# ilur98/DLMC-QUANT

Hardware: AMD Instinct MI355X
Metric: ResNet-50 W8A8 fake-quant fwd images/sec (higher is better)
Workload: dtype i8; 1 GPU; resnet50 W8A8 per-channel fake-quant forward (FSPTQ forms: W minmax_channel s8, A minmax_tensor u8), BN folded first as in FSPTQuant.py:67, fused int8 MFMA conv/linear, frozen execution plan (epilogue-fused ReLU / shortcut / next-layer codes; block end + next 1x1 as one launch; weight codes quantised once at plan build), 2 HIP streams per GPU, 224x224 relu(N(0,1)) pixels, batch 512 per GPU, scales; global_batch=512, parallelism=dp1 (batch-sharded replicas)

## Files before the change

dlmc-quant_amd/csrc/conv_chain_i8.hip:

```cpp
#include "conv_i8_common.h"

namespace dlmcq {

struct ChainArgs {
  const int8_t* x;
  const int8_t* w1;
  const float* s_w1;
  const int32_t* wsum1;
  const float* bias1;
  const float* s_in1;
  const float* zp_in1;
  int shift1;
  const float* residual;
  const int8_t* x2;
  const int8_t* w2;
  const float* s_w2;
  const int32_t* wsum2;
  const float* bias2;
  const float* s_in2;
  const float* zp_in2;
  int shift2, P, Q, H2, W2, stride2;
  FastDiv qdiv, pdiv;
  float* out;
  uint8_t* codes;
  const int8_t* w3;
  const float* s_w3;
  const int32_t* wsum3;
  const float* bias3;
  uint8_t* codes2;
  int w3_row, w3_chunk;
  int M, KD, rows_per_tile;
  int f_rowq, f_cstep, o_rowq, o_cstep;
  int lab;
  unsigned long long* trace;
};

template <int CTRL>
__device__ __forceinline__ float quad_dpp(float v) {
  return __builtin_bit_cast(float, __builtin_amdgcn_mov_dpp(__builtin_bit_cast(int, v), CTRL, 0xf, 0xf, true));
}
__device__ __forceinline__ void quad_transpose(float& x0, float& x1, float& x2, float& x3, bool b0, bool b1) {
  const float x0s = quad_dpp<0xB1>(x0), x1s = quad_dpp<0xB1>(x1), x2s = quad_dpp<0xB1>(x2), x3s = quad_dpp<0xB1>(x3);
  const float n0 = b0 ? x1s : x0, n1 = b0 ? x1 : x0s, n2 = b0 ? x3s : x2, n3 = b0 ? x3 : x2s;
  const float n0s = quad_dpp<0x4E>(n0), n1s = quad_dpp<0x4E>(n1), n2s = quad_dpp<0x4E>(n2), n3s = quad_dpp<0x4E>(n3);
  x0 = b1 ? n2s : n0;
  x2 = b1 ? n2 : n0s;
  x1 = b1 ? n3s : n1;
  x3 = b1 ? n3 : n1s;
}

constexpr int CHAIN_WGS(int c1, int kb) { return c1 + kb <= 256 ? 3 : 2; }
constexpr int CH_BIG = 0x7fff0000;

template <int C1, int KB, int C2 = 0, int FL = -1>
__global__ __launch_bounds__(256, CHAIN_WGS(C1 + C2, KB)) void conv_chain_i8_kernel(ChainArgs a, ConvEpi ep1, ConvEpi ep2) {
  constexpr bool DUALH = C2 > 0;
  const bool relu1 = FL < 0 ? ep1.relu != 0 : (FL & 1) != 0;
  const bool out1 = FL < 0 ? a.out != nullptr : (FL & 2) != 0;
  constexpr int S1 = C1 / 64;
  constexpr int S2 = C2 / 64;
  constexpr int U3 = KB / 64;
  constexpr int WCH = (S1 + S2 + U3) * 4096;
  constexpr int NPD = DUALH ? 2 : 1;
  constexpr int PAR = NPD * 4 * 256;
#ifndef DLMCQ_CHAIN_LDS_T
#define DLMCQ_CHAIN_LDS_T ((C1 == 128 && C2 == 256) ? 0 : 2)
#endif
  constexpr int TF = DLMCQ_CHAIN_LDS_T;
  constexpr bool LDST = TF != 0;
#ifdef DLMCQ_LAB
  constexpr int LABDMA = (C2 == 0 && C1 == 64) ? 16384 : 0;
#else
  constexpr int LABDMA = 0;
#endif
  __shared__ __attribute__((aligned(1024))) int8_t lds[2 * WCH + 2 * PAR + 4096 + 3 * KB * 4 + (LDST ? 4096 : 0) + LABDMA];
  int8_t* const par0 = lds + 2 * WCH;
  int8_t* const ctile = lds + 2 * WCH + 2 * PAR;
  int8_t* const par3 = ctile + 4096;
  float* const tstage = reinterpret_cast<float*>(par3 + 3 * KB * 4) + (threadIdx.x >> 6) * 256;

  const int tid = threadIdx.x, wave = tid >> 6, lane = tid & 63, l31 = lane & 31, hsel = lane >> 5;
  const int wr = wave >> 1, wc = wave & 1;
  constexpr bool LDST2 = TF == 2;
  const int q4 = LDST2 ? (lane & 7) : (l31 >> 2), b4 = l31 & 3;
  const int rsel = LDST2 ? (lane >> 3) : (4 * hsel + b4);
  const bool b0 = (lane & 1) != 0, b1 = (lane & 2) != 0;
  const int64_t row0 = (int64_t)blockIdx.x * a.rows_per_tile;
  const int rows_here = (int)((a.M - row0) < a.rows_per_tile ? (a.M - row0) : a.rows_per_tile);
  const int NC = a.KD >> 6;
#ifndef DLMCQ_CHAIN_ROT
#define DLMCQ_CHAIN_ROT 0
#endif
  const int rot = DLMCQ_CHAIN_ROT ? (int)(blockIdx.x % (unsigned)NC) : 0;
  auto cn = [&](int n) { const int m = n + rot; return m >= NC ? m - NC : m; };
#ifdef DLMCQ_LAB
  unsigned long long* const tr = (a.trace && tid == 0) ? a.trace + 64 * (size_t)blockIdx.x : nullptr;
  int trn = 0;
#define CHAIN_STAMP() do { if (tr && trn < 56) tr[trn++] = __builtin_readcyclecounter(); } while (0)
#define CHAIN_FINE(k) do { if (tr && nseq == 1) tr[56 + (k)] = __builtin_readcyclecounter(); } while (0)
#else
#define CHAIN_STAMP() do { } while (0)
#define CHAIN_FINE(k) do { } while (0)
#endif
  CHAIN_STAMP();
#ifdef DLMCQ_LAB
  if ((a.lab & 0x600) && blockIdx.x < 512) {
    const int unit = a.lab >> 16;
    const int d = (a.lab & 0x200) ? ((blockIdx.x >> 8) & 1) * unit : (int)(((blockIdx.x * 2654435761u) >> 28) * (uint32_t)unit) >> 4;
    for (int i = 0; i < d; ++i) __builtin_amdgcn_s_sleep(1);
  }
#endif

  {
    const int lrw = tid >> 2;
    const int sgw = ((tid & 3) ^ ((lrw >> 2) & 3)) * 16;
    const int8_t* xp = a.x + (row0 + (lrw < rows_here ? lrw : rows_here - 1)) * C1 + sgw;
#pragma unroll
    for (int s = 0; s < S1; ++s)
      __builtin_amdgcn_global_load_lds((gptr_t)(xp + s * 64), (lptr_t)(lds + WCH + s * 4096 + (tid >> 6) * 1024), 16, 0, 0);
    if constexpr (DUALH) {
      const uint32_t m = (uint32_t)(row0 + (lrw < rows_here ? lrw : rows_here - 1));
      const uint32_t t = fdiv(m, a.qdiv), nn = fdiv(t, a.pdiv);
      const int q = (int)(m - t * (uint32_t)a.Q), pp = (int)(t - nn * (uint32_t)a.P);
      const int8_t* xp2 = a.x2 + (((int64_t)nn * a.H2 + pp * a.stride2) * a.W2 + q * a.stride2) * C2 + sgw;
#pragma unroll
      for (int s = 0; s < S2; ++s)
        __builtin_amdgcn_global_load_lds((gptr_t)(xp2 + s * 64), (lptr_t)(lds + WCH + (S1 + s) * 4096 + (tid >> 6) * 1024), 16, 0, 0);
    }
  }
  const float sin2 = ep1.q_scale[0];
  const float zpf2 = ep1.q_zp ? ep1.q_zp[0] : 0.0f;
  const int dz2 = 128 - (int)__builtin_rintf(zpf2);
  if (tid < KB) {
    reinterpret_cast<float*>(par3)[tid] = sin2 * a.s_w3[tid];
    reinterpret_cast<int*>(par3)[KB + tid] = dz2 * a.wsum3[tid];
    reinterpret_cast<float*>(par3)[2 * KB + tid] = a.bias3 ? a.bias3[tid] : 0.0f;
  }
  asm volatile("s_waitcnt vmcnt(0) lgkmcnt(0)\n\ts_barrier" ::: "memory");
  i32x4 af[S1][2];
  i32x4 af2[DUALH ? S2 : 1][2];
  {
    const int r = wr * 32 + l31;
    const int8_t* ab = lds + WCH + r * 64;
    const uint32_t xw = a.shift1 ? 0x80808080u : 0u;
#pragma unroll
    for (int s = 0; s < S1; ++s)
#pragma unroll
      for (int ks = 0; ks < 2; ++ks) {
        const i32x4 t = *reinterpret_cast<const i32x4*>(ab + s * 4096 + (((ks * 2 + hsel) ^ ((r >> 2) & 3)) << 4));
        af[s][ks] = i32x4{(int)(t.x ^ xw), (int)(t.y ^ xw), (int)(t.z ^ xw), (int)(t.w ^ xw)};
      }
    if constexpr (DUALH) {
      const uint32_t xw2 = a.shift2 ? 0x80808080u : 0u;
#pragma unroll
      for (int s = 0; s < S2; ++s)
#pragma unroll
        for (int ks = 0; ks < 2; ++ks) {
          const i32x4 t = *reinterpret_cast<const i32x4*>(ab + (S1 + s) * 4096 + (((ks * 2 + hsel) ^ ((r >> 2) & 3)) << 4));
          af2[s][ks] = i32x4{(int)(t.x ^ xw2), (int)(t.y ^ xw2), (int)(t.z ^ xw2), (int)(t.w ^ xw2)};
        }
    }
  }
  asm volatile("s_waitcnt lgkmcnt(0)" ::: "memory");
  CHAIN_STAMP();

  const uint32_t fbytes = (uint32_t)((int64_t)a.M * a.KD * 4);
  const v4i r_res = make_rsrc(a.residual, fbytes);
  const v4i r_out = make_rsrc(a.out ? (const void*)a.out : (const void*)a.residual, a.out ? fbytes : 0u);
  const v4i r_cod = make_rsrc(a.codes ? (const void*)a.codes : (const void*)a.residual, a.codes ? fbytes / 4 : 0u);
  int fo[4];
#pragma unroll
  for (int g = 0; g < 4; ++g) {
    const int lr = wr * 32 + 8 * g + rsel;
    fo[g] = lr < rows_here ? (int)(((row0 + lr) * a.f_rowq + wc * 32 + q4 * 4) * 4) : CH_BIG;
#ifdef DLMCQ_LAB
    if (a.lab & 4) {
      const int lr2 = wr * 32 + 16 * (g >> 1) + 2 * (4 * hsel + b4) + (q4 >> 2);
      fo[g] = lr2 < rows_here ? (int)(((row0 + lr2) * a.KD + wc * 32 + 16 * (g & 1) + (q4 & 3) * 4) * 4) : CH_BIG;
    }
    if (a.lab & 8) {
      const int lr3 = wr * 32 + wc * 16 + 4 * g + (lane >> 4);
      fo[g] = lr3 < rows_here ? (int)(((row0 + lr3) * a.KD + (lane & 15) * 4) * 4) : CH_BIG;
    }
#endif
  }
  int cstep = a.f_cstep;
#ifdef DLMCQ_LAB
  if (a.lab & 64) {
    cstep = 64 * 256;
#pragma unroll
    for (int g = 0; g < 4; ++g) {
      const int lr = wr * 32 + 8 * g + rsel;
      fo[g] = lr < rows_here ? (int)(row0 * a.KD * 4 + lr * 256 + (wc * 32 + q4 * 4) * 4) : CH_BIG;
    }
  }
#endif
  constexpr bool MIXED_OK = !DUALH && !(C1 == 128 && KB == 128);
  int fo2[MIXED_OK ? 4 : 1];
  const int cstep2 = a.o_cstep;
  if constexpr (MIXED_OK) {
    const bool same = a.o_rowq == a.f_rowq;
#pragma unroll
    for (int g = 0; g < 4; ++g) {
      const int lr = wr * 32 + 8 * g + rsel;
      fo2[g] = same ? fo[g] : (lr < rows_here ? (int)(((row0 + lr) * a.o_rowq + wc * 32 + q4 * 4) * 4) : CH_BIG);
    }
  }
  auto out_off = [&](int g, int n) {
    if constexpr (MIXED_OK) return fo2[g] + n * cstep2;
    else return fo[g] + n * cstep;
  };
  int tw[4];
#pragma unroll
  for (int j = 0; j < 4; ++j) tw[j] = (4 * hsel + j) * 32 + (LDST2 ? l31 : ((l31 & 3) | ((l31 & ~3) ^ ((4 * hsel + j) * 4))));
  const int trd = LDST2 ? rsel * 32 + 4 * q4 : (4 * hsel + b4) * 32 + ((4 * q4) ^ ((4 * hsel + b4) * 4));
  const int nst = (out1 ? 4 : 0) + (a.codes ? 1 : 0);

  const int lrow = lane >> 2, pslot = lane & 3;
  const int drow = wave * 16 + lrow;
  const int dseg = (pslot ^ ((drow >> 2) & 3)) * 16;
  const int8_t* w1p = a.w1 + (int64_t)drow * C1 + dseg;
  const int d3 = drow & 31;
  const int prow3 = (drow & 32) + 16 * ((d3 >> 2) & 1) + 4 * (d3 >> 3) + (d3 & 3);
  const int8_t* w3p = a.w3 + (int64_t)prow3 * a.w3_row + dseg;
  const int cvo = drow < rows_here ? (int)((row0 + drow) * a.KD + dseg) : CH_BIG;
  const void* const pars[4] = {a.s_w1, a.wsum1, a.bias1 ? (const void*)a.bias1 : (const void*)a.s_w1, a.s_w1};
  const int32_t* parp = static_cast<const int32_t*>(wave == 0 ? pars[0] : wave == 1 ? pars[1] : wave == 2 ? pars[2] : pars[3]) + lane;
  const int8_t* w2p = DUALH ? a.w2 + (int64_t)drow * C2 + dseg : nullptr;
  const void* const pars2[4] = {a.s_w2, a.wsum2, a.bias2 ? (const void*)a.bias2 : (const void*)a.s_w2, a.s_w2};
  const int32_t* parp2 = static_cast<const int32_t*>(wave == 0 ? pars2[0] : wave == 1 ? pars2[1] : wave == 2 ? pars2[2] : pars2[3]) + lane;

  f32x4 res[2][4];
#ifdef DLMCQ_LAB
  if (a.lab & 0x801)
    for (auto& r2 : res)
      for (auto& r : r2) r = f32x4{1.0f, 2.0f, 3.0f, 4.0f};
#endif
  auto request = [&](int nseq, auto par_c) {
    constexpr int P = decltype(par_c)::value;
    const int n = cn(nseq);
    int8_t* wb = lds + P * WCH;
    bool wdma = true;
#ifdef DLMCQ_LAB
    wdma = !(((a.lab & 16) && (n & 1)) || (a.lab & 32));
#endif
#pragma unroll
    for (int s = 0; s < S1; ++s)
      if (wdma) __builtin_amdgcn_global_load_lds((gptr_t)(w1p + (int64_t)n * 64 * C1 + s * 64), (lptr_t)(wb + s * 4096 + wave * 1024), 16, 0, 0);
#pragma unroll
    for (int u = 0; u < U3; ++u)
      if (wdma) {
        const int8_t* src = w3p + (int64_t)u * 64 * a.w3_row + (int64_t)n * a.w3_chunk;
        __builtin_amdgcn_global_load_lds((gptr_t)src, (lptr_t)(wb + (S1 + S2 + u) * 4096 + wave * 1024), 16, 0, 0);
      }
    __builtin_amdgcn_global_load_lds((gptr_t)(parp + n * 64), (lptr_t)(par0 + P * PAR + wave * 256), 4, 0, 0);
    if constexpr (DUALH) {
#pragma unroll
      for (int s = 0; s < S2; ++s)
        if (wdma) __builtin_amdgcn_global_load_lds((gptr_t)(w2p + (int64_t)n * 64 * C2 + s * 64), (lptr_t)(wb + (S1 + s) * 4096 + wave * 1024), 16, 0, 0);
      __builtin_amdgcn_global_load_lds((gptr_t)(parp2 + n * 64), (lptr_t)(par0 + P * PAR + 1024 + wave * 256), 4, 0, 0);
      return;
    }
#pragma unroll
    for (int g = 0; g < 4; ++g) {
#ifdef DLMCQ_LAB
      if (a.lab & 1) continue;
      if constexpr (LABDMA > 0) {
        if (a.lab & 0x800) {
          const int lr = wr * 32 + 8 * g + rsel;
          const float* src = a.residual + (row0 + (lr < rows_here ? lr : rows_here - 1)) * a.KD + n * 64 + wc * 32 + q4 * 4;
          __builtin_amdgcn_global_load_lds((gptr_t)src, (lptr_t)(lds + sizeof(lds) - LABDMA + wave * 4096 + g * 1024), 16, 0, 2);
          continue;
        }
      }
#endif
      int lo = fo[g] + n * cstep;
#ifdef DLMCQ_LAB
      if (a.lab & 0x2000) lo &= 0xffff;
#endif
      bload16(res[P][g], lo, r_res);
    }
  };

  const float sin1 = a.s_in1[0];
  const float zpf1 = a.zp_in1 ? a.zp_in1[0] : 0.0f;
  const int dz1 = a.shift1 - (int)__builtin_rintf(zpf1);
  const float sin1b = DUALH ? a.s_in2[0] : 0.0f;
  const int dz1b = DUALH ? a.shift2 - (int)__builtin_rintf(a.zp_in2 ? a.zp_in2[0] : 0.0f) : 0;
  ConvEpi e1 = ep1;
  e1.codes = reinterpret_cast<uint8_t*>(uintptr_t(1));
  const EpiQuant eq1(e1, FL >= 0);
  __builtin_assume(!eq1.sgn);

  i32x16 acc2[U3];
#pragma unroll
  for (int j = 0; j < U3; ++j)
#pragma unroll
    for (int i = 0; i < 16; ++i) acc2[j][i] = 0;

  request(0, std::integral_constant<int, 0>{});

  auto chunk = [&](int nseq, auto par_c) {
    constexpr int P = decltype(par_c)::value;
    const int n = cn(nseq);
    if (nseq == 0 || nst == 0) asm volatile("s_waitcnt vmcnt(0)\n\ts_barrier" ::: "memory");
    else if (nst == 4) asm volatile("s_waitcnt vmcnt(4)\n\ts_barrier" ::: "memory");
    else if (nst == 5) asm volatile("s_waitcnt vmcnt(5)\n\ts_barrier" ::: "memory");
    else asm volatile("s_waitcnt vmcnt(1)\n\ts_barrier" ::: "memory");
    CHAIN_STAMP();
    if constexpr (!DUALH) asm volatile("" : "+v"(res[P][0]), "+v"(res[P][1]), "+v"(res[P][2]), "+v"(res[P][3]));
    if (nseq + 1 < NC) request(nseq + 1, std::integral_constant<int, 1 - P>{});

    const int8_t* wb = lds + P * WCH;
    const int8_t* pp = par0 + P * PAR + (wc * 32 + l31) * 4;
    i32x16 acc;
    f32x2 extra2[DUALH ? 8 : 1];
    if constexpr (DUALH) {
      const float corr2f = (float)(dz1b * *reinterpret_cast<const int*>(pp + 1024 + 256));
#pragma unroll
      for (int i = 0; i < 16; ++i) acc[i] = 0;
      const int r = wc * 32 + l31;
#pragma unroll
      for (int s = 0; s < S2; ++s)
#pragma unroll
        for (int ks = 0; ks < 2; ++ks) {
          const i32x4 bf = *reinterpret_cast<const i32x4*>(wb + (S1 + s) * 4096 + r * 64 + (((ks * 2 + hsel) ^ ((r >> 2) & 3)) << 4));
          acc = __builtin_amdgcn_mfma_i32_32x32x32_i8(af2[s][ks], bf, acc, 0, 0, 0);
        }
      const float mult2 = sin1b * *reinterpret_cast<const float*>(pp + 1024);
      const float bv2 = a.bias2 ? *reinterpret_cast<const float*>(pp + 1024 + 512) : 0.0f;
      const f32x2 c2{corr2f, corr2f}, m2{mult2, mult2}, b2{bv2, bv2};
#pragma unroll
      for (int i = 0; i < 8; ++i) extra2[i] = pk_fma(f32x2{(float)acc[2 * i], (float)acc[2 * i + 1]} + c2, m2, b2);
    }
    const float corrf = (float)(dz1 * *reinterpret_cast<const int*>(pp + 256));
#pragma unroll
    for (int i = 0; i < 16; ++i) acc[i] = 0;
    {
      const int r = wc * 32 + l31;
#pragma unroll
      for (int s = 0; s < S1; ++s)
#pragma unroll
        for (int ks = 0; ks < 2; ++ks) {
          const i32x4 bf = *reinterpret_cast<const i32x4*>(wb + s * 4096 + r * 64 + (((ks * 2 + hsel) ^ ((r >> 2) & 3)) << 4));
          acc = __builtin_amdgcn_mfma_i32_32x32x32_i8(af[s][ks], bf, acc, 0, 0, 0);
        }
    }
#ifdef DLMCQ_LAB
    if (tr && nseq == 1) asm volatile("s_nop 0" ::"v"(acc[0]), "v"(acc[15]));
#endif
    CHAIN_FINE(0);
    const float mult = sin1 * *reinterpret_cast<const float*>(pp);
    const float bv = a.bias1 ? *reinterpret_cast<const float*>(pp + 512) : 0.0f;
    float v[16];
    {
      const f32x2 c2{corrf, corrf}, m2{mult, mult}, b2{bv, bv};
#pragma unroll
      for (int i = 0; i < 8; ++i) {
        f32x2 f = pk_fma(f32x2{(float)acc[2 * i], (float)acc[2 * i + 1]} + c2, m2, b2);
        if constexpr (DUALH) f = f + extra2[DUALH ? i : 0];
        v[2 * i] = f.x;
        v[2 * i + 1] = f.y;
      }
    }
#ifndef DLMCQ_CHAIN_GP
#define DLMCQ_CHAIN_GP 4
#endif
    constexpr bool TIGHT = C2 == 0 && ((C1 == 64 && KB == 128) || (C1 == 128 && KB == 128));
    constexpr int GP = (FL < 0 || TIGHT) ? 1 : DLMCQ_CHAIN_GP;
#pragma unroll
    for (int g0 = 0; g0 < 4; g0 += GP) {
      f32x4 y[GP];
#pragma unroll
      for (int k = 0; k < GP; ++k) {
        const int g = g0 + k;
        if constexpr (LDST) {
#pragma unroll
          for (int j = 0; j < 4; ++j) tstage[tw[j]] = v[4 * g + j];
          asm volatile("" ::: "memory");
          y[k] = *reinterpret_cast<const f32x4*>(tstage + trd);
          asm volatile("" ::: "memory");
        } else {
          quad_transpose(v[4 * g], v[4 * g + 1], v[4 * g + 2], v[4 * g + 3], b0, b1);
          y[k] = f32x4{v[4 * g], v[4 * g + 1], v[4 * g + 2], v[4 * g + 3]};
        }
        if constexpr (!DUALH) y[k] = y[k] + res[P][g];
        if (relu1 && (FL < 0 || out1)) y[k] = relu4_nan(y[k]);
#ifdef DLMCQ_LAB
        if (out1) bstore16(y[k], (a.lab & 0x1000) ? (out_off(g, n) & 0xffff) : out_off(g, n), r_out);
#else
        if (out1) bstore16(y[k], out_off(g, n), r_out);
#endif
      }
      uint32_t c[GP];
      if constexpr (FL >= 0) {
        eq1.code4n_plain(y, c);
      } else if constexpr (GP == 1) {
        c[0] = eq1.code4(y[0]);
      } else {
        bool un[GP];
        eq1.code4n(y, c, un);
      }
#pragma unroll
      for (int k = 0; k < GP; ++k) {
        const int R = wr * 32 + 8 * (g0 + k) + rsel;
        *reinterpret_cast<uint32_t*>(ctile + R * 64 + (((wc * 2 + (q4 >> 2)) ^ ((R >> 2) & 3)) << 4) + (q4 & 3) * 4) = c[k];
        CHAIN_FINE(1 + g0 + k);
      }
    }
    CHAIN_STAMP();
    asm volatile("s_waitcnt lgkmcnt(0)\n\ts_barrier" ::: "memory");
    CHAIN_STAMP();
    if (a.codes)
      bstore16i(*reinterpret_cast<const i32x4*>(ctile + drow * 64 + pslot * 16), cvo == CH_BIG ? CH_BIG : cvo + n * 64, r_cod);
    {
      const int R = wr * 32 + l31;
#pragma unroll
      for (int ks = 0; ks < 2; ++ks) {
        const i32x4 t = *reinterpret_cast<const i32x4*>(ctile + R * 64 + (((ks * 2 + hsel) ^ ((R >> 2) & 3)) << 4));
        const i32x4 a2 = i32x4{(int)(t.x ^ 0x80808080u), (int)(t.y ^ 0x80808080u), (int)(t.z ^ 0x80808080u), (int)(t.w ^ 0x80808080u)};
#pragma unroll
        for (int j = 0; j < U3; ++j) {
          const int kb = wc * (KB / 2) + j * 32 + l31;
          const i32x4 bf = *reinterpret_cast<const i32x4*>(wb + (S1 + S2) * 4096 + kb * 64 + (((ks * 2 + hsel) ^ ((kb >> 2) & 3)) << 4));
          acc2[j] = __builtin_amdgcn_mfma_i32_32x32x32_i8(bf, a2, acc2[j], 0, 0, 0);
        }
      }
    }
  };
  for (int n = 0; n < NC; n += 2) {
    chunk(n, std::integral_constant<int, 0>{});
    if (n + 1 < NC) chunk(n + 1, std::integral_constant<int, 1>{});
  }

  CHAIN_STAMP();
  const EpiQuant eq2(ep2, ep2.relu != 0);
  const int lr2 = wr * 32 + l31;
#pragma unroll
  for (int j = 0; j < U3; ++j) {
    const int cb = wc * (KB / 2) + j * 32 + hsel * 16;
    f32x4 y[4];
#pragma unroll
    for (int q = 0; q < 4; ++q) {
      const f32x4 mu = *reinterpret_cast<const f32x4*>(par3 + (cb + 4 * q) * 4);
      const i32x4 co = *reinterpret_cast<const i32x4*>(par3 + (KB + cb + 4 * q) * 4);
      const f32x4 bs = *reinterpret_cast<const f32x4*>(par3 + (2 * KB + cb + 4 * q) * 4);
      y[q] = f32x4{dequant1(acc2[j][4 * q] + co.x, mu.x, bs.x), dequant1(acc2[j][4 * q + 1] + co.y, mu.y, bs.y),
                   dequant1(acc2[j][4 * q + 2] + co.z, mu.z, bs.z), dequant1(acc2[j][4 * q + 3] + co.w, mu.w, bs.w)};
    }
    uint32_t wq[4];
    if constexpr (FL >= 0) {
      eq2.code4n_plain(y, wq);
    } else {
      bool uq[4];
      eq2.code4n(y, wq, uq);
    }
    if (lr2 < rows_here)
      *reinterpret_cast<i32x4*>(ep2.codes + (row0 + lr2) * KB + cb) = i32x4{(int)wq[0], (int)wq[1], (int)wq[2], (int)wq[3]};
  }
#ifdef DLMCQ_LAB
  if (tr) {
    asm volatile("s_waitcnt vmcnt(0)" ::: "memory");
    CHAIN_STAMP();
    tr[63] = __builtin_amdgcn_s_getreg(4 | (31 << 11));
  }
#endif
}

}

using namespace dlmcq;

#ifdef DLMCQ_LAB
static unsigned long long* g_chain_trace = nullptr;
extern "C" void dlmcq_x_chain_trace(void* buf) { g_chain_trace = static_cast<unsigned long long*>(buf); }
static int g_chain_lab = 0;
extern "C" void dlmcq_x_chain_lab(int flags) { g_chain_lab = flags; }
#endif

static int chain_launch(ChainArgs& a, int64_t M, int64_t C, int64_t K, int64_t C2, int64_t K2, int32_t relu, void* codes,
                        const float* q_scale, const float* q_zero_point, int32_t q_lo, int32_t q_hi, int32_t q_form, float q_ste_g,
                        int32_t relu2, void* codes2, const float* q2_scale, const float* q2_zero_point, int32_t q2_lo, int32_t q2_hi,
                        int32_t q2_form, float q2_ste_g, int32_t rows_per_tile, dlmcq_stream_t stream) {
  if (relu == DLMCQ_ACT_RELU6 || relu2 == DLMCQ_ACT_RELU6) return DLMCQ_EINVAL;
  if (q_lo != 0 || q_hi != 255) return DLMCQ_EINVAL;
  if (q2_form & (DLMCQ_FORCE_TILED | DLMCQ_ROUTE_ONLY | DLMCQ_PIPELINED)) return DLMCQ_EINVAL;
  const bool w3cm = (q2_form & DLMCQ_W2_CHUNK_MAJOR) != 0, ocm = (q2_form & DLMCQ_FP32_OUT_CHUNK_MAJOR) != 0;
  const bool icm = (C2 == 0 && a.residual) ? (q2_form & DLMCQ_FP32_IN_CHUNK_MAJOR) != 0 : ocm;
  const bool ocm2 = a.out ? ocm : icm;
  q2_form &= ~(DLMCQ_W2_CHUNK_MAJOR | DLMCQ_FP32_IN_CHUNK_MAJOR | DLMCQ_FP32_OUT_CHUNK_MAJOR);
  if (icm != ocm2 && C2 == 0 && C == 128 && K2 == 128) return DLMCQ_EINVAL;
  a.w3_row = w3cm ? 64 : (int)K;
  a.w3_chunk = w3cm ? (int)K2 * 64 : 64;
  ConvEpi ep1{}, ep2{};
  if (q2_lo > q2_hi || q2_lo < -128 || q2_hi > 255 || q2_hi - q2_lo > 255 || q_form < DLMCQ_FORM_EMULATE ||
      q_form > DLMCQ_FORM_SYMMETRIC || !epi_set_form(ep2, q2_form, q2_lo, q2_hi))
    return DLMCQ_EINVAL;
  if (M * K * 4 > (int64_t)CH_BIG) return DLMCQ_ERANGE;
  a.M = (int)M; a.KD = (int)K;
  a.f_rowq = icm ? 64 : (int)K;
  a.f_cstep = icm ? (int)M * 256 : 256;
  a.o_rowq = ocm2 ? 64 : (int)K;
  a.o_cstep = ocm2 ? (int)M * 256 : 256;
#ifdef DLMCQ_LAB
  a.trace = g_chain_trace;
  a.lab = g_chain_lab;
#endif
  if (rows_per_tile <= 0) {
    const int64_t t64 = (M + 63) / 64, slots = 256 * CHAIN_WGS((int)(C + C2), (int)K2);
    const int64_t full = t64 / slots, left = t64 % slots;
    rows_per_tile = (full >= 2 && full <= 4 && left > 0 && left * 8 < slots) ? 56 : 64;
  }
  a.rows_per_tile = rows_per_tile;
  if (a.rows_per_tile > 64) return DLMCQ_EINVAL;
  ep1.relu = relu != 0; ep1.q_scale = q_scale; ep1.q_zp = q_zero_point; ep1.q_lo = (float)q_lo; ep1.q_hi = (float)q_hi;
  ep1.q_g = q_ste_g; ep1.q_form = q_form; ep1.codes = static_cast<uint8_t*>(codes);
  ep2.relu = relu2 != 0; ep2.q_scale = q2_scale; ep2.q_zp = q2_zero_point; ep2.q_lo = (float)q2_lo; ep2.q_hi = (float)q2_hi;
  ep2.q_g = q2_ste_g; ep2.codes = static_cast<uint8_t*>(codes2);
  const int64_t tiles = (M + a.rows_per_tile - 1) / a.rows_per_tile;
  if (tiles >= (1ll << 31)) return DLMCQ_ERANGE;
  hipStream_t st = reinterpret_cast<hipStream_t>(stream);
  const dim3 grid((uint32_t)tiles), block(256);
  size_t dyn = 0;
#ifdef DLMCQ_LAB
  dyn = (g_chain_lab & 128 ? 40960 : 0) + (g_chain_lab & 256 ? 81920 : 0);
#endif
  const int fl = (relu && epi_plain_q(ep1) && epi_plain_q(ep2)) ? (a.out ? 3 : 1) : -1;
#define DLMCQ_CHAIN_GO(...)                                                                                          \
  do {                                                                                                               \
    if (fl == 3) hipLaunchKernelGGL((conv_chain_i8_kernel<__VA_ARGS__, 3>), grid, block, dyn, st, a, ep1, ep2);       \
    else if (fl == 1) hipLaunchKernelGGL((conv_chain_i8_kernel<__VA_ARGS__, 1>), grid, block, dyn, st, a, ep1, ep2);  \
    else hipLaunchKernelGGL((conv_chain_i8_kernel<__VA_ARGS__, -1>), grid, block, dyn, st, a, ep1, ep2);              \
  } while (0)
  if (C2 == 0) {
    if (C == 64 && K2 == 64) DLMCQ_CHAIN_GO(64, 64, 0);
    else if (C == 64 && K2 == 128) DLMCQ_CHAIN_GO(64, 128, 0);
    else if (C == 128 && K2 == 128) DLMCQ_CHAIN_GO(128, 128, 0);
    else if (C == 128 && K2 == 256) DLMCQ_CHAIN_GO(128, 256, 0);
    else if (C == 256 && K2 == 256) DLMCQ_CHAIN_GO(256, 256, 0);
    else return DLMCQ_EINVAL;
  } else {
    if (C == 64 && C2 == 64 && K2 == 64) DLMCQ_CHAIN_GO(64, 64, 64);
    else if (C == 128 && C2 == 256 && K2 == 128) DLMCQ_CHAIN_GO(128, 128, 256);
    else return DLMCQ_EINVAL;
  }
#undef DLMCQ_CHAIN_GO
  return launch_status();
}

extern "C" int dlmcq_conv2d_i8_nhwc_chain(const void* x, const int8_t* w, float* out, const float* bias, const int32_t* wsum,
                                          const float* in_scale, const float* in_zero_point, const float* w_scale, int64_t M,
                                          int64_t C, int64_t K, int32_t x_is_unsigned, const float* residual, int32_t relu,
                                          void* codes, const float* q_scale, const float* q_zero_point, int32_t q_lo,
                                          int32_t q_hi, int32_t q_form, float q_ste_g, const int8_t* w2, const float* bias2,
                                          const int32_t* wsum2, const float* w_scale2, int64_t K2, int32_t relu2, void* codes2,
                                          const float* q2_scale, const float* q2_zero_point, int32_t q2_lo, int32_t q2_hi,
                                          int32_t q2_form, float q2_ste_g, int32_t rows_per_tile, dlmcq_stream_t stream) {
  if (M < 0 || C < 1 || K < 1 || K2 < 1 || K % 64 != 0) return DLMCQ_EINVAL;
  if (M == 0) return DLMCQ_OK;
  if (!x || !w || !wsum || !in_scale || !w_scale || !residual || !w2 || !wsum2 || !w_scale2 || !codes2 || !q_scale || !q2_scale)
    return DLMCQ_EINVAL;
  if (!aligned16(x) || !aligned16(w) || !aligned16(w2) || !aligned16(residual) || (out && !aligned16(out)) ||
      (codes && !aligned16(codes)) || !aligned16(codes2))
    return DLMCQ_EALIGN;
  ChainArgs a{};
  a.x = static_cast<const int8_t*>(x); a.w1 = w; a.s_w1 = w_scale; a.wsum1 = wsum; a.bias1 = bias;
  a.s_in1 = in_scale; a.zp_in1 = in_zero_point; a.shift1 = x_is_unsigned ? 128 : 0;
  a.residual = residual; a.out = out; a.codes = static_cast<uint8_t*>(codes);
  a.w3 = w2; a.s_w3 = w_scale2; a.wsum3 = wsum2; a.bias3 = bias2; a.codes2 = static_cast<uint8_t*>(codes2);
  return chain_launch(a, M, C, K, 0, K2, relu, codes, q_scale, q_zero_point, q_lo, q_hi, q_form, q_ste_g, relu2, codes2, q2_scale,
                      q2_zero_point, q2_lo, q2_hi, q2_form, q2_ste_g, rows_per_tile, stream);
}

extern "C" int dlmcq_conv2d_i8_nhwc_dual_chain(const void* x, const int8_t* w, float* out, const float* bias, const int32_t* wsum,
                                               const float* in_scale, const float* in_zero_point, const float* w_scale, int64_t N,
                                               int64_t H, int64_t W, int64_t C, int64_t K, int32_t x_is_unsigned, const void* x2,
                                               const int8_t* w2, const float* bias2, const int32_t* wsum2, const float* in_scale2,
                                               const float* in_zero_point2, const float* w_scale2, int64_t H2, int64_t W2,
                                               int64_t C2, int32_t stride2, int32_t x2_is_unsigned, int32_t relu, void* codes,
                                               const float* q_scale, const float* q_zero_point, int32_t q_lo, int32_t q_hi,
                                               int32_t q_form, float q_ste_g, const int8_t* w3, const float* bias3,
                                               const int32_t* wsum3, const float* w_scale3, int64_t K3, int32_t relu3, void* codes3,
                                               const float* q3_scale, const float* q3_zero_point, int32_t q3_lo, int32_t q3_hi,
                                               int32_t q3_form, float q3_ste_g, int32_t rows_per_tile, dlmcq_stream_t stream) {
  if (N < 0 || H < 1 || W < 1 || C < 1 || K < 1 || K3 < 1 || K % 64 != 0 || H2 < 1 || W2 < 1 || C2 < 1 || stride2 < 1)
    return DLMCQ_EINVAL;
  if ((H2 - 1) / stride2 + 1 != H || (W2 - 1) / stride2 + 1 != W) return DLMCQ_EINVAL;
  const int64_t M = N * H * W;
  if (M == 0) return DLMCQ_OK;
  if (!x || !w || !wsum || !in_scale || !w_scale || !x2 || !w2 || !wsum2 || !in_scale2 || !w_scale2 || !w3 || !wsum3 || !w_scale3 ||
      !codes3 || !q_scale || !q3_scale)
    return DLMCQ_EINVAL;
  if (!aligned16(x) || !aligned16(w) || !aligned16(x2) || !aligned16(w2) || !aligned16(w3) || (out && !aligned16(out)) ||
      (codes && !aligned16(codes)) || !aligned16(codes3))
    return DLMCQ_EALIGN;
  if (M >= (1ll << 31) || N * H2 * W2 * C2 >= (1ll << 40)) return DLMCQ_ERANGE;
  ChainArgs a{};
  a.x = static_cast<const int8_t*>(x); a.w1 = w; a.s_w1 = w_scale; a.wsum1 = wsum; a.bias1 = bias;
  a.s_in1 = in_scale; a.zp_in1 = in_zero_point; a.shift1 = x_is_unsigned ? 128 : 0;
  a.x2 = static_cast<const int8_t*>(x2); a.w2 = w2; a.s_w2 = w_scale2; a.wsum2 = wsum2; a.bias2 = bias2;
  a.s_in2 = in_scale2; a.zp_in2 = in_zero_point2; a.shift2 = x2_is_unsigned ? 128 : 0;
  a.P = (int)H; a.Q = (int)W; a.H2 = (int)H2; a.W2 = (int)W2; a.stride2 = stride2;
  a.qdiv = make_fastdiv((uint32_t)W);
  a.pdiv = make_fastdiv((uint32_t)H);
  a.residual = nullptr; a.out = out; a.codes = static_cast<uint8_t*>(codes);
  a.w3 = w3; a.s_w3 = w_scale3; a.wsum3 = wsum3; a.bias3 = bias3; a.codes2 = static_cast<uint8_t*>(codes3);
  return chain_launch(a, M, C, K, C2, K3, relu, codes, q_scale, q_zero_point, q_lo, q_hi, q_form, q_ste_g, relu3, codes3, q3_scale,
                      q3_zero_point, q3_lo, q3_hi, q3_form, q3_ste_g, rows_per_tile, stream);
}
```

dlmc-quant_amd/dlmc/_native.py:

```python
import ctypes
import os

import torch

_HERE = os.path.dirname(os.path.abspath(__file__))
import sys

_PRODUCT = os.path.join(os.path.dirname(_HERE), "libdlmcq.so")
_OVERRIDE = os.environ.get("DLMCQ_LIBRARY")
LAB_OVERRIDE = bool(_OVERRIDE) and os.environ.get("DLMCQ_LAB_TOOLS") == "1"
if _OVERRIDE and not LAB_OVERRIDE:
    print(f"[dlmc] DLMCQ_LIBRARY={_OVERRIDE} ignored (set DLMCQ_LAB_TOOLS=1 to load a lab / A-B build); loading {_PRODUCT}", file=sys.stderr)
LIB_PATH = _OVERRIDE if LAB_OVERRIDE else _PRODUCT
if LAB_OVERRIDE:
    print(f"[dlmc] lab override: loading {LIB_PATH} instead of the product library", file=sys.stderr)

FORM_EMULATE, FORM_QBASE, FORM_ZEROPOINT, FORM_SYMMETRIC, FORM_ROOTQ_ACT = range(5)
EMIT_SHIFT128 = 0x100
W2_CHUNK_MAJOR = 0x200
FORCE_TILED = 0x400
ROUTE_ONLY = 0x800
FP32_IN_CHUNK_MAJOR = 0x2000
FP32_OUT_CHUNK_MAJOR = 0x4000
PAD_CODE0 = 0x8000
PIPELINED = 0x1000
ROUTE_TILED, ROUTE_HALO3X3, ROUTE_PW, ROUTE_PWR, ROUTE_DW, ROUTE_DWM, ROUTE_HALO3X3_PIPE, ROUTE_GAP = 1, 2, 3, 4, 5, 6, 7, 8
ROUTE_TAG = {ROUTE_TILED: "conv_i8", ROUTE_HALO3X3: "conv3x3_halo", ROUTE_PW: "conv_pw", ROUTE_PWR: "conv_pwr", ROUTE_DW: "conv_dw",
             ROUTE_DWM: "conv_dwm", ROUTE_HALO3X3_PIPE: "conv3x3_pipe", ROUTE_GAP: "conv_gap"}
ACT_NONE, ACT_RELU, ACT_RELU6 = 0, 1, 2
Y_DEQUANT, Y_CODES = 0, 1
CODES_NONE, CODES_I8, CODES_P4 = 0, 1, 2
MINMAX_ABSMAX, MINMAX_MINMAX, MINMAX_NEGMIN = 0, 1, 2

_p, _i64, _i32, _f32, _sz = ctypes.c_void_p, ctypes.c_int64, ctypes.c_int32, ctypes.c_float, ctypes.c_size_t

SIGNATURES = {
    "dlmcq_version": (ctypes.c_int, []),
    "dlmcq_strerror": (ctypes.c_char_p, [ctypes.c_int]),
    "dlmcq_fake_quant_f32": (ctypes.c_int, [_p, _p, _p, _p, _p, _i64, _i64, _i64, _i32, _i32, _i32, _i32, _i32, _f32, _p]),
    "dlmcq_dequant_codes_f32": (ctypes.c_int, [_p, _p, _p, _p, _i64, _i64, _i64, _i32, _i32, _i32, _f32, _p]),
    "dlmcq_dequant_f32": (ctypes.c_int, [_p, _p, _p, _p, _i64, _i64, _i64, _p]),
    "dlmcq_minmax_scratch_bytes": (_sz, [_i64, _i64, _i64]),
    "dlmcq_minmax_f32": (ctypes.c_int, [_p, _p, _p, _i64, _i64, _i64, _i32, _p, _sz, _p]),
    "dlmcq_minmax_finalize_f32": (ctypes.c_int, [_p, _i64, _i64, _p, _p, _i32, _p]),
    "dlmcq_conv2d_i8_observed_partials": (_sz, [_i64, _i64]),
    "dlmcq_conv2d_i8_nhwc_fused_observed": (ctypes.c_int, [_p, _p, _p, _p, _p, _p, _p, _p, _i64, _i64, _i64, _i64, _i64, _i64, _i64, _i32, _i32,
                                                            _i32, _i32, _p, _i32, _p, _p, _p, _i32, _i32, _i32, _f32, _p, _i64, _p, _p]),
    "dlmcq_qparams_from_minmax": (ctypes.c_int, [_p, _p, _p, _p, _i64, _i32, _i32, _i32, _i32, _f32, _p]),
    "dlmcq_span_scale_f32": (ctypes.c_int, [_p, _p, _p, _i64, _f32, _i32, _p]),
    "dlmcq_lsq_init_scratch_bytes": (_sz, [_i64]),
    "dlmcq_lsq_init_f32": (ctypes.c_int, [_p, _p, _i64, _f32, _p, _sz, _p]),
    "dlmcq_observe_qparams_f32": (ctypes.c_int, [_p, _p, _p, _i64, _i64, _i64, _i32, _i32, _i32, _f32, _p, _sz, _p]),
    "dlmcq_pack_int4": (ctypes.c_int, [_p, _p, _i64, _p]),
    "dlmcq_unpack_int4": (ctypes.c_int, [_p, _p, _i64, _i32, _p]),
    "dlmcq_fq_bwd_scratch_bytes": (_sz, [_i64, _i64, _i64]),
    "dlmcq_fake_quant_bwd_f32": (ctypes.c_int, [_p, _p, _p, _p, _p, _p, _i64, _i64, _i64, _i32, _i32, _f32, _p, _sz, _p]),
    "dlmcq_rootq_bwd_scratch_bytes": (ctypes.c_size_t, [_i64]),
    "dlmcq_rootq_weight_bwd_f32": (ctypes.c_int, [_p, _p, _p, _p, _p, _p, _i64, _i32, _i32, _p, _sz, _p]),
    "dlmcq_fake_quant_bwd_form_f32": (ctypes.c_int, [_p, _p, _p, _p, _p, _p, _i64, _i64, _i64, _i32, _i32, _i32, _f32, _p, _sz, _p]),
    "dlmcq_fq_segment_bytes": (_sz, []),
    "dlmcq_fq_multi_prepare": (ctypes.c_int, [_p, _i64, _p, _p, _p, _p]),
    "dlmcq_fake_quant_multi_f32": (ctypes.c_int, [_p, _i64, _i64, _p]),
    "dlmcq_fake_quant_multi_bwd_f32": (ctypes.c_int, [_p, _i64, _i64, _i64, _p, _sz, _p]),
    "dlmcq_rootq_weight_f32": (ctypes.c_int, [_p, _p, _p, _i64, _i32, _i32, _p]),
    "dlmcq_l2norm_scratch_bytes": (_sz, [_i64, _i64, _i64]),
    "dlmcq_l2norm_step_f32": (ctypes.c_int, [_p, _p, _p, _p, _i64, _i64, _i64, _i32, _i32, _p, _sz, _p]),
    "dlmcq_l2norm_iterate_f32": (ctypes.c_int, [_p, _p, _p, _p, _i64, _i64, _i64, _i32, _i32, _i32, _f32, _p, _sz, _p]),
    "dlmcq_l2out_scratch_bytes": (_sz, [_i64, _i64, _i64]),
    "dlmcq_l2out_update_f32": (ctypes.c_int, [_p, _p, _p, _p, _p, _i64, _i64, _i64, _i32, _f32, _f32, _p, _sz, _p]),
    "dlmcq_l2loss_scratch_bytes": (_sz, [_i64]),
    "dlmcq_l2loss_tensor_f32": (ctypes.c_int, [_p, _p, _p, _p, _p, _i64, _i32, _f32, _p, _sz, _p]),
    "dlmcq_l2loss_rows_f32": (ctypes.c_int, [_p, _p, _p, _i64, _i64, _i32, _p]),
    "dlmcq_adaround_weight_f32": (ctypes.c_int, [_p, _p, _p, _p, _i64, _i64, _i32, _i32, _i32, _p]),
    "dlmcq_adaround_weight_bwd_f32": (ctypes.c_int, [_p, _p, _p, _p, _p, _p, _i64, _i64, _i32, _i32, _p]),
    "dlmcq_quantize_weight_krsc_i8": (ctypes.c_int, [_p, _p, _p, _p, _i64, _i64, _i64, _i64, _i32, _i32, _p]),
    "dlmcq_conv2d_i8_nhwc_f32": (ctypes.c_int, [_p, _p, _p, _p, _p, _p, _p, _p, _i64, _i64, _i64, _i64, _i64, _i64, _i64,
                                               _i32, _i32, _i32, _i32, _p]),
    "dlmcq_conv2d_i8_nhwc_fused": (ctypes.c_int, [_p, _p, _p, _p, _p, _p, _p, _p, _i64, _i64, _i64, _i64, _i64, _i64, _i64,
                                                 _i32, _i32, _i32, _i32, _p, _i32, _p, _p, _p, _i32, _i32, _i32, _f32, _p]),
    "dlmcq_conv2d_i8_nhwc_asym": (ctypes.c_int, [_p, _p, _p, _p, _p, _p, _p, _p, _p, _i64, _i64, _i64, _i64, _i64, _i64, _i64,
                                                _i32, _i32, _i32, _i32, _p, _i32, _p, _p, _p, _i32, _i32, _i32, _f32, _p]),
    "dlmcq_conv2d_i8_nhwc_narrow": (ctypes.c_int, [_p, _p, _p, _p, _p, _p, _p, _p, _p, _i64, _i64, _i64, _i64, _i64, _i64, _i64,
                                                  _i32, _i32, _i32, _i32, _p, _i32, _p, _p, _p, _i32, _i32, _i32, _f32, _i64, _p]),
    "dlmcq_conv2d_i8_nhwc_padres": (ctypes.c_int, [_p, _p, _p, _p, _p, _p, _p, _p, _p, _i64, _i64, _i64, _i64, _i64, _i64, _i64,
                                                  _i32, _i32, _i32, _i32, _p, _i64, _i64, _i64, _i32, _i64, _i32, _p, _p, _p, _i32, _i32, _i32,
                                                  _f32, _i64, _p]),
    "dlmcq_conv2d_dw_i8_nhwc": (ctypes.c_int, [_p, _p, _p, _p, _p, _p, _p, _p, _i64, _i64, _i64, _i64, _i64, _i64, _i32, _i32, _i32,
                                              _i32, _p, _p, _p, _i32, _i32, _i32, _f32, _p]),
    "dlmcq_conv2d_i8_nhwc_xoff": (ctypes.c_int, [_p, _p, _p, _p, _p, _p, _p, _p, _p, _i64, _i64, _i64, _i64, _i64, _i64, _i64,
                                                _i32, _i32, _i32, _i32, _p, _i32, _p, _p, _p, _i32, _i32, _i32, _f32, _p, _p, _p]),
    "dlmcq_conv2d_dw_i8_nhwc_xoff": (ctypes.c_int, [_p, _p, _p, _p, _p, _p, _p, _p, _i64, _i64, _i64, _i64, _i64, _i64, _i32, _i32, _i32,
                                                   _i32, _p, _p, _p, _i32, _i32, _i32, _f32, _p, _p, _p]),
    "dlmcq_conv2d_i8_stem_xoff": (ctypes.c_int, [_p, _p, _p, _p, _p, _p, _p, _p, _p, _i64, _i64, _i64, _i64, _i64, _i64, _i64, _i32, _i32,
                                                _i32, _i32, _p, _p, _p, _i32, _i32, _i32, _f32, _p, _p, _p]),
    "dlmcq_dwpw_pack_table": (ctypes.c_int, [_p, _p, _p, _p, _p, _p, _i64, _i32, _p, _p]),
    "dlmcq_conv2d_dwpw_i8_nhwc": (ctypes.c_int, [_p, _p, _i32, _i32, _i32, _p, _i64, _i64, _i64, _i64, _i32, _p, _p, _i32, _i32, _i32, _f32,
                                                _p, _p, _p, _p, _p, _p, _i64, _i32, _p, _p, _p, _i32, _i32, _i32, _f32, _p]),
    "dlmcq_conv2d_i8_nhwc_dual": (ctypes.c_int, [_p, _p, _p, _p, _p, _p, _p, _p, _i64, _i64, _i64, _i64, _i64, _i64, _i64,
                                                _i32, _i32, _i32, _i32,
                                                _p, _p, _p, _p, _p, _p, _p, _i64, _i64, _i64, _i64, _i64, _i32, _i32, _i32, _i32,
                                                _i32, _p, _p, _p, _i32, _i32, _i32, _f32, _p]),
    "dlmcq_conv2d_i8_nhwc_chain": (ctypes.c_int, [_p, _p, _p, _p, _p, _p, _p, _p, _i64, _i64, _i64, _i32, _p, _i32, _p, _p, _p, _i32,
                                                 _i32, _i32, _f32, _p, _p, _p, _p, _i64, _i32, _p, _p, _p, _i32, _i32, _i32, _f32,
                                                 _i32, _p]),
    "dlmcq_conv2d_i8_nhwc_dual_chain": (ctypes.c_int, [_p, _p, _p, _p, _p, _p, _p, _p, _i64, _i64, _i64, _i64, _i64, _i32,
                                                      _p, _p, _p, _p, _p, _p, _p, _i64, _i64, _i64, _i32, _i32,
                                                      _i32, _p, _p, _p, _i32, _i32, _i32, _f32,
                                                      _p, _p, _p, _p, _i64, _i32, _p, _p, _p, _i32, _i32, _i32, _f32, _i32, _p]),
    "dlmcq_quantize_pad_nhwc4": (ctypes.c_int, [_p, _p, _p, _p, _i64, _i64, _i64, _i64, _i64, _i64, _i64, _i64, _i32, _i32, _i32,
                                               _i32, _f32, _p]),
    "dlmcq_quantize_weight_stem_i8": (ctypes.c_int, [_p, _p, _p, _p, _i64, _i64, _i64, _i64, _i32, _i32, _p]),
    "dlmcq_conv2d_i8_stem_fused": (ctypes.c_int, [_p, _p, _p, _p, _p, _p, _p, _p, _i64, _i64, _i64, _i64, _i64, _i64, _i32, _i32,
                                                 _i32, _p, _p, _p, _i32, _i32, _i32, _f32, _p]),
    "dlmcq_conv2d_i8_stem_asym": (ctypes.c_int, [_p, _p, _p, _p, _p, _p, _p, _p, _p, _i64, _i64, _i64, _i64, _i64, _i64, _i64, _i32, _i32,
                                                _i32, _p, _p, _p, _i32, _i32, _i32, _f32, _p]),
    "dlmcq_conv2d_i8_stem_pool_fused": (ctypes.c_int, [_p, _p, _p, _p, _p, _p, _p, _p, _i64, _i64, _i64, _i64, _i64, _i64, _i32, _i32,
                                                      _i32, _p, _p, _p, _i32, _i32, _i32, _f32, _p]),
    "dlmcq_maxpool_codes_nhwc": (ctypes.c_int, [_p, _p, _i64, _i64, _i64, _i64, _i32, _i32, _i32, _i32, _p]),
    "dlmcq_gap_nhwc_f32": (ctypes.c_int, [_p, _p, _p, _i64, _i64, _i64, _p, _p, _i32, _i32, _i32, _f32, _p]),
    "dlmcq_avgpool_nhwc_f32": (ctypes.c_int, [_p, _p, _p, _i64, _i64, _i64, _i64, _i64, _i64, _i64, _i32, _p, _p, _i32, _i32, _i32, _f32, _p]),
    "dlmcq_conv2d_i8_nhwc_gap": (ctypes.c_int, [_p, _p, _p, _p, _p, _p, _p, _p, _i64, _i64, _i64, _i64, _i64, _i32, _p, _i32, _p, _p, _p,
                                               _i32, _i32, _i32, _f32, _p]),
    "dlmcq_fold_bn_f32": (ctypes.c_int, [_p, _p, _p, _p, _p, _p, _i64, _i64, _f32, _p]),
    "dlmcq_repvgg_fuse_f32": (ctypes.c_int, [_p, _p, _p, _p, _p, _p, _p, _f32, _f32, _f32, _i64, _i64, _p]),
}


class FqSegment(ctypes.Structure):
    _fields_ = [("x", _p), ("y", _p), ("gy", _p), ("gx", _p), ("scale", _p), ("offset", _p), ("gscale", _p),
                ("n", _i64), ("channels", _i64), ("inner", _i64), ("lo", _i64), ("hi", _i64), ("ste_g", ctypes.c_double),
                ("form", _i64), ("fwd_chunk0", _i64), ("bwd_wg0", _i64), ("part0", _i64)]


FQ_MULTI_MAX_ELEMENTS = 8192 * 1024


def _load():
    if not os.path.exists(LIB_PATH):
        raise ImportError(
            f"{LIB_PATH} not found: build it with `make -C dlmc-quant_amd/csrc` (or "
            "`python -c 'import __graft_entry__ as g; g.build()'`).  There is no CPU fallback.")
    tlib = os.path.join(os.path.dirname(torch.__file__), "lib", "libamdhip64.so")
    if os.path.exists(tlib):
        ctypes.CDLL(tlib, mode=ctypes.RTLD_GLOBAL)
    lib = ctypes.CDLL(LIB_PATH)
    for name, (res, args) in SIGNATURES.items():
        try:
            fn = getattr(lib, name)
        except AttributeError:
            if LAB_OVERRIDE:
                continue
            raise
        fn.restype, fn.argtypes = res, args
    if hasattr(lib, "dlmcq_fq_segment_bytes") and lib.dlmcq_fq_segment_bytes() != ctypes.sizeof(FqSegment):
        raise ImportError(f"{LIB_PATH}: dlmcq_fq_segment is {lib.dlmcq_fq_segment_bytes()} bytes, the ctypes mirror {ctypes.sizeof(FqSegment)}")
    return lib


lib = _load()


def experimental(name, argtypes):
    fn = getattr(lib, name)
    fn.restype, fn.argtypes = ctypes.c_int, argtypes
    return fn


class DlmcqError(RuntimeError):
    pass


def check(rc):
    if rc != 0:
        raise DlmcqError(f"{lib.dlmcq_strerror(rc).decode()} (code {rc})")


def route(rc):
    if rc <= 0:
        raise DlmcqError(f"{lib.dlmcq_strerror(rc).decode()} (code {rc})" if rc < 0 else "route query returned DLMCQ_OK (an empty problem)")
    return rc


def stream_ptr():
    return ctypes.c_void_p(torch.cuda.current_stream().cuda_stream)


def ptr(t):
    return None if t is None else ctypes.c_void_p(t.data_ptr())


def require_gpu(*tensors):
    for t in tensors:
        if t is not None and not t.is_cuda:
            raise DlmcqError(
                "dlmc (MI355X build) runs on the GPU only: got a tensor on "
                f"'{t.device}'.  There is no CPU fallback in this package.")
```

dlmc-quant_amd/dlmc/quantization/scalar/kernels.py:

```python
import collections
import ctypes
import math

import torch

from ... import _native as N
from ..._native import (CODES_I8, CODES_NONE, CODES_P4, FORM_EMULATE, FORM_QBASE, FORM_ROOTQ_ACT,
                        FORM_SYMMETRIC, FORM_ZEROPOINT, MINMAX_ABSMAX, MINMAX_MINMAX, MINMAX_NEGMIN,
                        Y_CODES, Y_DEQUANT)

__all__ = ["fake_quant", "dequant_codes", "dequant", "minmax", "observe_qparams", "qparams_from_minmax",
           "span_scale", "lsq_init", "l2norm_step", "adaround_weight", "adaround_weight_backward", "quantize_weight_krsc", "conv2d_i8", "global_avgpool", "avgpool_quant", "conv2d_i8_gap", "gap_head_supported", "gap_head_profitable", "pack_int4", "unpack_int4", "fake_quant_backward", "Segment", "FqMultiPlan", "fake_quant_multi", "fake_quant_multi_backward", "rootq_weight", "geometry", "channel_shape",
           "PROFILE"]


class _Profile:

    def __init__(self):
        self.enabled = False
        self.records = []

    def reset(self):
        self.records = []

# ... 543 lines not shown
    if not want_out and emit is None:
        raise ValueError("conv2d_dw_i8: nothing to produce (want_out=False without emit)")

    def alloc(dtype):
        return torch.empty((n, c, P, Q), dtype=dtype, device=codes.device, memory_format=torch.channels_last)
    q = _quantiser(emit, alloc, codes, False, "conv2d_dw_i8")
    out = alloc(torch.float32) if want_out else None
    small = (_bias_c(bias), _flat(in_scale, codes), _flat(in_zp, codes), _flat(w_scale, codes), _flat(w_offset, codes))
    fn, trailer = N.lib.dlmcq_conv2d_dw_i8_nhwc, ()
    if in_offset is not None:
        in_offset, tap_sums = _flat(in_offset, codes), _flat(tap_sums, codes)
        fn, trailer = N.lib.dlmcq_conv2d_dw_i8_nhwc_xoff, (N.ptr(in_offset), N.ptr(tap_sums))
    args = (N.ptr(codes), N.ptr(wq), N.ptr(out), *map(N.ptr, small), n, h, w_, c, R, S, int(stride), int(padding),
            int(codes.dtype == torch.uint8), _act(relu, act))
    flags = N.FORCE_TILED if force_tiled else 0

    def call(extra=0):
        return fn(*args, *_q_args(q, flags | extra), *trailer, N.stream_ptr())
    oe = n * c * P * Q
    tag = N.ROUTE_TAG[N.route(call(N.ROUTE_ONLY))] if PROFILE.enabled else "conv_dw"
    PROFILE.launch(tag, codes.numel() + wq.numel() + oe * (4 * want_out + (emit is not None)), lambda: N.check(call()), 2 * oe * R * S)
    return (out, q[0]) if emit is not None else out


DWPW_WIDTHS = (128, 192, 512)


def dwpw_supported(c, k, h, w, stride, padding, ksize):
    return ksize == 3 and stride == 1 and padding == 1 and c % 64 == 0 and k in DWPW_WIDTHS and w <= 61 and h >= 1


def dwpw_table(wq, bias, in_scale, in_zp, w_scale, w_offset, x_unsigned=True):
    N.require_gpu(wq)
    r, s_, c = wq.shape
    if (r, s_) != (3, 3) or c % 64:
        raise ValueError("dwpw_table: 3 x 3 weights [3, 3, C], C % 64 == 0")
    table = torch.empty((c // 64, 64, 8), dtype=torch.int32, device=wq.device)
    small = (_bias_c(bias), _flat(in_scale, wq), _flat(in_zp, wq), _flat(w_scale, wq), _flat(w_offset, wq))
    N.check(N.lib.dlmcq_dwpw_pack_table(N.ptr(wq), *map(N.ptr, small), c, int(bool(x_unsigned)), N.ptr(table), N.stream_ptr()))
    return table


def conv2d_dwpw_i8(codes, table, dw_asym, dw_bias, dw_relu, in_zp, emit, pw, relu=True, emit2=None):
    N.require_gpu(codes, table, pw["wq"])
    codes = _nhwc(codes)
    n, c, h, w_ = codes.shape
    k = pw["wq"].shape[0]
    if tuple(pw["wq"].shape[1:]) != (1, 1, c) or emit is None or emit2 is None or tuple(table.shape) != (c // 64, 64, 8):
        raise ValueError("conv2d_dwpw_i8: a pointwise layer [K, 1, 1, C] on the depthwise layer's codes, both quantisers given")
    q1 = _quantiser(emit, lambda dtype: None, codes, False, "conv2d_dwpw_i8")
    q2 = _quantiser(emit2, lambda dtype: torch.empty((n, k, h, w_), dtype=dtype, device=codes.device, memory_format=torch.channels_last),
                    codes, False, "conv2d_dwpw_i8")
    zx, b = _flat(in_zp, codes), _bias_c(pw["bias"])
    scales = (_flat(pw["in_scale"], codes), _flat(pw["w_scale"], codes, k), _flat(pw.get("w_offset"), codes, k))
    m = n * h * w_
    nbytes = codes.numel() + table.numel() * 4 + pw["wq"].numel() + m * k
    PROFILE.launch("conv_dwpw", nbytes, lambda: N.check(N.lib.dlmcq_conv2d_dwpw_i8_nhwc(
        N.ptr(codes), N.ptr(table), int(bool(dw_asym)), int(bool(dw_bias)), int(bool(dw_relu)), N.ptr(zx), n, h, w_, c,
        int(codes.dtype == torch.uint8), *_q_args(q1)[1:], N.ptr(pw["wq"]), N.ptr(b), N.ptr(pw["wsum"]), *map(N.ptr, scales), k,
        int(bool(relu)), *_q_args(q2), N.stream_ptr())), 2 * m * c * (9 + k))
    return q2[0]


def conv2d_i8_dual(a, b, relu=False, emit=None, want_out=True, force_tiled=False, out_chunk_major=False):
    for t in (a, b):
        if t["codes"].dim() != 4:
            raise ValueError("conv2d_i8_dual takes 4-D activation codes")
    oa, ob = _operand(a), _operand(b)
    if oa.shape != ob.shape:
        raise ValueError(f"conv2d_i8_dual: the two convolutions give {oa.shape} and {ob.shape}")
    if not want_out and emit is None:
        raise ValueError("conv2d_i8_dual: nothing to produce (want_out=False without emit)")
    shape = oa.shape
    n, K_ = shape[:2]

    def alloc(dtype):
        return torch.empty(shape, dtype=dtype, device=oa.codes.device, memory_format=torch.channels_last)
    out = alloc(torch.float32) if want_out else None
    q = _quantiser(emit, alloc, oa.codes, True, "conv2d_i8_dual")
    h, w_, ch, R, S, st, pd, dl, uns = oa.geom
    _, _, ch2, R2, S2, st2, _, _, _ = ob.geom
    oe = math.prod(shape)
    def touched(c, r, s_, stride):
        return c.numel() // (stride * stride) if r == 1 and s_ == 1 else c.numel()
    nbytes = touched(oa.codes, R, S, st) + touched(ob.codes, R2, S2, st2) + a["wq"].numel() + b["wq"].numel() + oe * (4 * want_out + (emit is not None))
    args = (*_head(oa, out), n, h, w_, ch, K_, R, S, st, pd, dl, uns, *ob.ptrs, *ob.geom, int(bool(relu)))
    flags = N.FORCE_TILED if force_tiled else 0

    def call(extra=0):
        return N.lib.dlmcq_conv2d_i8_nhwc_dual(*args, *_q_args(q, flags | extra), N.stream_ptr())
    ocm = bool(out_chunk_major) and out is not None and N.route(call(N.ROUTE_ONLY)) == N.ROUTE_PWR
    tag = N.ROUTE_TAG[N.route(call(N.ROUTE_ONLY))] if PROFILE.enabled else "conv_i8"
    PROFILE.launch(tag, nbytes, lambda: N.check(call(N.FP32_OUT_CHUNK_MAJOR if ocm else 0)), 2 * oe * (ch * R * S + ch2 * R2 * S2))
    if ocm:
        out = _as_chunk_major(out)
    return (out, q[0]) if emit is not None else out


CHAIN_SHAPES = {(64, 64), (64, 128), (128, 128), (128, 256), (256, 256)}
CHAIN_ONE_LAYOUT = {(128, 128)}


def chain_supported(c, k, k2, m):
    return (c, k2) in CHAIN_SHAPES and k % 64 == 0 and m * k * 4 <= 0x7fff0000


def chunk_major(wq):
    k2, r, s_, k = wq.shape
    if (r, s_) != (1, 1) or k % 64:
        raise ValueError("chunk_major: a 1x1 layer with K % 64 = 0")
    return wq.reshape(k2, k // 64, 64).permute(1, 0, 2).contiguous()


class ChunkMajor:

    def __init__(self, buf, shape):
        self.buf, self.shape = buf, tuple(shape)
        self.dtype, self.device = buf.dtype, buf.device

    @staticmethod
    def empty(n, k, h, w, device):
        if k % 64:
            raise ValueError("ChunkMajor: K % 64 = 0")
        return ChunkMajor(torch.empty((k // 64, n * h * w, 64), dtype=torch.float32, device=device), (n, k, h, w))

    @staticmethod
    def from_nhwc(t):
        n, k, h, w = t.shape
        if k % 64 or t.dtype != torch.float32:
            raise ValueError("ChunkMajor: an fp32 tensor with K % 64 = 0")
        rows = t.permute(0, 2, 3, 1).reshape(n * h * w, k // 64, 64)
        return ChunkMajor(rows.permute(1, 0, 2).contiguous(), (n, k, h, w))

    def to_nhwc(self):
        n, k, h, w = self.shape
        rows = self.buf.permute(1, 0, 2).reshape(n, h, w, k)
        return rows.permute(0, 3, 1, 2).contiguous(memory_format=torch.channels_last)

    def dim(self):
        return 4

    def numel(self):
        return self.buf.numel()

    def window(self, n, p0, p1, q0, q1):
        nn, k, h, w = self.shape
        rows = self.buf.view(k // 64, nn, h, w, 64)[:, n, p0:p1, q0:q1, :]
        return rows.permute(1, 2, 0, 3).reshape(1, p1 - p0, q1 - q0, k).permute(0, 3, 1, 2).contiguous()

    def record_stream(self, s):
        self.buf.record_stream(s)


class PadShortcut:

    def __init__(self, src, stride=1, lo=0):
        if not isinstance(src, torch.Tensor) or src.dim() != 4 or src.dtype != torch.float32:
            raise ValueError("PadShortcut: the source is an fp32 (N, C, H, W) tensor")
        if not src.permute(0, 2, 3, 1).is_contiguous():
            raise ValueError("PadShortcut: the source must be dense in channels_last memory (a slice or a view with gaps is not)")
        self.src, self.stride, self.lo = src, int(stride), int(lo)
        if self.stride < 1 or self.lo < 0 or self.lo % 4 or src.shape[1] % 4 or src.shape[1] < 4:
            raise ValueError("PadShortcut: stride >= 1, lo >= 0, lo % 4 == 0 and source channels % 4 == 0")
        self.dtype, self.device = src.dtype, src.device

    def shape_for(self, k):
        n, c, h, w = self.src.shape
        s = self.stride
        return (n, k, (h + s - 1) // s, (w + s - 1) // s) if self.lo + c <= k else None

    def materialise(self, k):
        sub = self.src[:, :, ::self.stride, ::self.stride]
        return torch.nn.functional.pad(sub, (0, 0, 0, 0, self.lo, k - self.lo - sub.shape[1])).contiguous(memory_format=torch.channels_last)

    def record_stream(self, s):
        self.src.record_stream(s)


def _second_weights(b):
    wc = b.get("wq_chunk")
    if wc is None:
        return b["wq"], 0
    k2, _, _, k = b["wq"].shape
    if tuple(wc.shape) != (k // 64, k2, 64) or wc.dtype != torch.int8 or not wc.is_contiguous():
        raise ValueError("wq_chunk must be chunk_major(wq)")
    return wc, N.W2_CHUNK_MAJOR


def conv2d_i8_chain(a, b, residual, relu=True, emit=None, want_out=True, want_codes=False, relu2=True, emit2=None,
                    rows_per_tile=0, out_chunk_major=False):
    c = a["codes"]
    icm, ocm = isinstance(residual, ChunkMajor), bool(out_chunk_major) and want_out
    if want_out and icm != ocm and (c.shape[1], b["wq"].shape[0]) in CHAIN_ONE_LAYOUT:
        residual = residual.to_nhwc() if icm else ChunkMajor.from_nhwc(residual)
        icm = ocm
    res_cm, residual = (residual, residual.buf) if icm else (None, residual)
    N.require_gpu(b["wq"], residual)
    o = _operand(a)
    c = o.codes
    (n, K_), (h, w_, ch, R, S, _, _, _, uns) = o.shape[:2], o.geom
    K2, R2, S2, C2 = b["wq"].shape
    if (R, S, R2, S2) != (1, 1, 1, 1) or C2 != K_ or emit is None or emit2 is None:
        raise ValueError("conv2d_i8_chain: two 1x1 convolutions, the second reading the first's codes")
    if tuple(res_cm.shape if icm else residual.shape) != (n, K_, h, w_) or residual.dtype != torch.float32:
        raise ValueError("conv2d_i8_chain: residual must be fp32 of the first output's shape")
    if not icm:
        residual = _nhwc(residual)
    m = n * h * w_

    def alloc(k, dtype):
        return torch.empty((n, k, h, w_), dtype=dtype, device=c.device, memory_format=torch.channels_last)
    out = (ChunkMajor.empty(n, K_, h, w_, c.device) if ocm else alloc(K_, torch.float32)) if want_out else None
    q = _quantiser(emit, lambda dtype: alloc(K_, dtype) if want_codes else None, c, False, "conv2d_i8_chain")
    q2 = _quantiser(emit2, lambda dtype: alloc(K2, dtype), c, True, "conv2d_i8_chain")
    b2, ws2 = _bias_c(b["bias"]), _flat(b["w_scale"], c, K2)
    nbytes = c.numel() + a["wq"].numel() + b["wq"].numel() + m * K_ * (4 + 4 * want_out + want_codes) + m * K2
    w2t, w2flag = _second_weights(b)
    flags = w2flag | (N.FP32_IN_CHUNK_MAJOR if icm else 0) | (N.FP32_OUT_CHUNK_MAJOR if ocm else 0)
    PROFILE.launch("conv_chain", nbytes, lambda: N.check(N.lib.dlmcq_conv2d_i8_nhwc_chain(
        *_head(o, out.buf if ocm else out), m, ch, K_, uns, N.ptr(residual), int(bool(relu)), *_q_args(q),
        N.ptr(w2t), N.ptr(b2), N.ptr(b["wsum"]), N.ptr(ws2), K2, int(bool(relu2)), *_q_args(q2, flags), int(rows_per_tile), N.stream_ptr())),
        2 * m * K_ * (ch + K2))
    return out, q[0], q2[0]


DUAL_CHAIN_SHAPES = {(64, 64, 64), (128, 256, 128)}


def dual_chain_supported(c, c2, k, k3, m):
    return (c, c2, k3) in DUAL_CHAIN_SHAPES and k % 64 == 0 and m * k * 4 <= 0x7fff0000


def conv2d_i8_dual_chain(a, b, c3, relu=True, emit=None, want_out=True, want_codes=False, relu3=True, emit3=None, rows_per_tile=0,
                         out_chunk_major=False):
    N.require_gpu(c3["wq"])
    oa, ob = _operand(a), _operand(b)
    (n, K_), (h, w_, ch, _, _, st, pd, _, uns) = oa.shape[:2], oa.geom
    h2, w2, ch2, _, _, st2, pd2, _, uns2 = ob.geom
    K3 = c3["wq"].shape[0]
    if (tuple(a["wq"].shape[1:3]), tuple(b["wq"].shape[1:3]), tuple(c3["wq"].shape[1:3])) != ((1, 1),) * 3 or st != 1 or pd or pd2 \
            or b["wq"].shape[0] != K_ or c3["wq"].shape[3] != K_ or emit is None or emit3 is None:
        raise ValueError("conv2d_i8_dual_chain: three unpadded 1x1 convolutions, the third reading the codes of the sum of the first two")

    def alloc(k, dtype):
        return torch.empty((n, k, h, w_), dtype=dtype, device=oa.codes.device, memory_format=torch.channels_last)
    fcm = bool(out_chunk_major) and want_out
    out = (ChunkMajor.empty(n, K_, h, w_, oa.codes.device) if fcm else alloc(K_, torch.float32)) if want_out else None
    q = _quantiser(emit, lambda dtype: alloc(K_, dtype) if want_codes else None, oa.codes, False, "conv2d_i8_dual_chain")
    q3 = _quantiser(emit3, lambda dtype: alloc(K3, dtype), oa.codes, True, "conv2d_i8_dual_chain")
    b3, ws3 = _bias_c(c3["bias"]), _flat(c3["w_scale"], oa.codes, K3)
    m = n * h * w_
    nbytes = oa.codes.numel() + ob.codes.numel() // (st2 * st2) + a["wq"].numel() + b["wq"].numel() + c3["wq"].numel() + \
        m * K_ * (4 * want_out + want_codes) + m * K3
    w3t, w3flag = _second_weights(c3)
    PROFILE.launch("conv_chain", nbytes, lambda: N.check(N.lib.dlmcq_conv2d_i8_nhwc_dual_chain(
        *_head(oa, out.buf if fcm else out), n, h, w_, ch, K_, uns, *ob.ptrs, h2, w2, ch2, st2, uns2, int(bool(relu)), *_q_args(q),
        N.ptr(w3t), N.ptr(b3), N.ptr(c3["wsum"]), N.ptr(ws3), K3, int(bool(relu3)),
        *_q_args(q3, w3flag | (N.FP32_OUT_CHUNK_MAJOR if fcm else 0)), int(rows_per_tile), N.stream_ptr())),
        2 * m * K_ * (ch + ch2 + K3))
    return out, q[0], q3[0]


def quantize_pad_nhwc4(x, scale, zero_point, lo, hi, form, pad, g=0.0, shift128=False, pad_code0=False):
    N.require_gpu(x)
    if x.dim() != 4 or x.shape[1] > 4 or x.dtype != torch.float32:
        raise ValueError("quantize_pad_nhwc4 takes an fp32 (N, C <= 4, H, W) tensor")
    n, c, h, w = x.shape
    hp, wp = h + 2 * pad, w + 2 * pad
    if shift128 and not (0 <= lo and hi <= 255):
        raise ValueError("quantize_pad_nhwc4: shift128 needs an unsigned byte range")
    flat = torch.empty(n * hp * wp * 4 + 32, dtype=torch.uint8 if lo >= 0 and not shift128 else torch.int8, device=x.device)
    scale = _f32c(scale.detach(), x).reshape(-1)
    zero_point = None if zero_point is None else _f32c(zero_point, x).reshape(-1)
    PROFILE.launch("fq_image", x.numel() * 4 + n * hp * wp * 4, lambda: N.check(N.lib.dlmcq_quantize_pad_nhwc4(
        N.ptr(x), N.ptr(flat), N.ptr(scale), N.ptr(zero_point), n, c, h, w, *x.stride(), int(pad), int(lo), int(hi),
        int(form) | (N.EMIT_SHIFT128 if shift128 else 0) | (N.PAD_CODE0 if pad_code0 else 0), float(g), N.stream_ptr())))
    return flat[:n * hp * wp * 4].view(n, hp, wp, 4)


def quantize_weight_stem(w, scale, lo, hi):
    N.require_gpu(w)
    w = w.detach().contiguous()
    K_, C, R, S = w.shape
    scale = _f32c(scale.detach(), w).reshape(-1)
    if scale.numel() == 1:
        scale = scale.expand(K_).contiguous()
    wq = torch.empty((K_, R, 8, 4), dtype=torch.int8, device=w.device)
    wsum = torch.empty(K_, dtype=torch.int32, device=w.device)
    N.check(N.lib.dlmcq_quantize_weight_stem_i8(N.ptr(w), N.ptr(wq), N.ptr(wsum), N.ptr(scale), K_, C, R, S, int(lo), int(hi),
                                                N.stream_ptr()))
    return wq, wsum


def conv2d_i8_stem(xpad, wq, wsum, bias, in_scale, in_zp, w_scale, S, stride=1, relu=False, emit=None, want_out=True, pool=False,
                   w_offset=None, channels=4, act=None, in_offset=None, tap_sums=None, pad=0):
    if (in_offset is None) != (tap_sums is None) or (in_offset is not None and pool):
        raise ValueError("conv2d_i8_stem: in_offset needs tap_sums and no pool")
    act = _act(relu, act)
    N.require_gpu(xpad, wq)
    n, hp, wp, _ = xpad.shape
    K_, R = wq.shape[0], wq.shape[1]
    P0, Q0 = P, Q = _out_hw(hp, wp, R, S, stride)
    if pool:
        if K_ > 64:
            raise ValueError("conv2d_i8_stem(pool=True) handles at most 64 output channels")
        P, Q = _out_hw(P, Q, 3, 3, 2, 1)
    if not want_out and emit is None:
        raise ValueError("conv2d_i8_stem: nothing to produce (want_out=False without emit)")

    def alloc(dtype):
        return torch.empty((n, K_, P, Q), dtype=dtype, device=xpad.device, memory_format=torch.channels_last)
    q = _quantiser(emit, alloc, xpad, False, "conv2d_i8_stem")
    out = alloc(torch.float32) if want_out else None
    bias, in_scale, in_zp, w_scale = _bias_c(bias), _flat(in_scale, xpad), _flat(in_zp, xpad), _flat(w_scale, xpad, K_)
    w_offset, in_offset, tap_sums = _flat(w_offset, xpad), _flat(in_offset, xpad), _flat(tap_sums, xpad)
    w_off, pad_arg, trailer, cin = (N.ptr(w_offset), int(channels)), (), (), int(channels)
    if in_offset is not None:
        fn, pad_arg, trailer = N.lib.dlmcq_conv2d_i8_stem_xoff, (int(pad),), (N.ptr(in_offset), N.ptr(tap_sums))
    elif w_offset is not None:
        if pool:
            raise ValueError("conv2d_i8_stem: the pooling kernel has no weight-offset term")
        fn = N.lib.dlmcq_conv2d_i8_stem_asym
    else:
        fn, w_off, cin = (N.lib.dlmcq_conv2d_i8_stem_pool_fused if pool else N.lib.dlmcq_conv2d_i8_stem_fused), (), 3
    args = (N.ptr(xpad), N.ptr(wq), N.ptr(out), N.ptr(bias), N.ptr(wsum), N.ptr(in_scale), N.ptr(in_zp), N.ptr(w_scale), *w_off,
            n, hp, wp, K_, R, int(S), int(stride), *pad_arg, int(xpad.dtype == torch.uint8), act, *_q_args(q), *trailer)
    PROFILE.launch("conv_stem", xpad.numel() + wq.numel() + n * K_ * P * Q * (4 * want_out + (emit is not None)),
                   lambda: N.check(fn(*args, N.stream_ptr())), 2 * n * K_ * P0 * Q0 * R * S * cin)
    return (out, q[0]) if emit is not None else out


def maxpool_codes(codes, kernel, stride, padding):
    N.require_gpu(codes)
    n, c, h, w = codes.shape
    if not codes.is_contiguous(memory_format=torch.channels_last):
        codes = codes.contiguous(memory_format=torch.channels_last)
    P, Q = (h + 2 * padding - kernel) // stride + 1, (w + 2 * padding - kernel) // stride + 1
    y = torch.empty((n, c, P, Q), dtype=codes.dtype, device=codes.device, memory_format=torch.channels_last)
    PROFILE.launch("pool_codes", codes.numel() + y.numel(), lambda: N.check(N.lib.dlmcq_maxpool_codes_nhwc(
        N.ptr(codes), N.ptr(y), n, h, w, c, int(kernel), int(stride), int(padding), int(codes.dtype == torch.uint8),
        N.stream_ptr())))
    return y


GAP_HEAD_MAX_HW, GAP_HEAD_MAX_C = 64, 2048


def gap_head_supported(c, k, h, w, ksize=1, stride=1, padding=0, asym=False):
    return (ksize == 1 and stride == 1 and padding == 0 and not asym and c >= 64 and c % 64 == 0 and c <= GAP_HEAD_MAX_C and k >= 64 and
            k % 64 == 0 and h >= 1 and w >= 1 and h * w <= GAP_HEAD_MAX_HW)


GAP_HEAD_MEASURED_SLOWER = {(512, 2048), (320, 1280), (512, 1280)}


def gap_head_profitable(c, k):
    return (c, k) not in GAP_HEAD_MEASURED_SLOWER


def global_avgpool(x, emit=None, want_out=True):
    N.require_gpu(x)
    if x.dim() != 4 or x.dtype != torch.float32:
        raise ValueError("global_avgpool: an fp32 (N, C, H, W) tensor")
    if not want_out and emit is None:
        raise ValueError("global_avgpool: nothing to produce (want_out=False without emit)")
    x = _nhwc(x)
    n, c, h, w_ = x.shape

    def alloc(dtype):
        return torch.empty((n, c), dtype=dtype, device=x.device)
    out = alloc(torch.float32) if want_out else None
    q = _quantiser(emit, alloc, x, True, "global_avgpool")
    PROFILE.launch("gap", x.numel() * 4 + n * c * (4 * want_out + (emit is not None)), lambda: N.check(N.lib.dlmcq_gap_nhwc_f32(
        N.ptr(x), N.ptr(out), *_q_args(q)[:1], n, h * w_, c, *_q_args(q)[1:], N.stream_ptr())))
    return (out, q[0]) if emit is not None else out


def _nhwc_rows(x):
    n, c, h, w = x.shape
    xs = x.stride(3)
    ok = (h > 1 and w > 1 and x.stride(1) == 1 and xs >= c and xs % 4 == 0 and x.stride(2) == w * xs and
          (n == 1 or x.stride(0) == h * w * xs) and x.data_ptr() % 16 == 0)
    return xs if ok else None


def avgpool_quant(x, window, emit=None, want_out=True, c_pad=None, pad_code=0):
    N.require_gpu(x)
    if x.dim() != 4 or x.dtype != torch.float32:
        raise ValueError("avgpool_quant: an fp32 (N, C, H, W) tensor")
    if not want_out and emit is None:
        raise ValueError("avgpool_quant: nothing to produce (want_out=False without emit)")
    n, c, h, w_ = x.shape
    c_pad = c if c_pad is None else int(c_pad)
    if c_pad != c and emit is None:
        raise ValueError("avgpool_quant: c_pad pads the code rows (emit=None writes none)")
    s = int(window)
    xs = _nhwc_rows(x)
    if xs is None:
        x = _nhwc(x)
        xs = c
    p, q_ = (h // s, w_ // s) if s > 0 else (0, 0)

    def alloc(dtype, ch=c_pad):
        return torch.empty((n, ch, p, q_), dtype=dtype, device=x.device, memory_format=torch.channels_last)
    out = alloc(torch.float32, c) if want_out else None
    q = _quantiser(emit, alloc, x, True, "avgpool_quant")
    m = n * p * q_
    PROFILE.launch("avgpool", m * (c * (4 * s * s + 4 * want_out) + c_pad * (emit is not None)), lambda: N.check(N.lib.dlmcq_avgpool_nhwc_f32(
        N.ptr(x), N.ptr(out), *_q_args(q)[:1], n, h, w_, c, xs, s, c_pad, int(pad_code), *_q_args(q)[1:], N.stream_ptr())))
    return out, q[0]


def conv2d_i8_gap(codes, wq, wsum, bias, in_scale, in_zp, w_scale, residual=None, act=None, emit=None, want_out=True):
# ... 243 lines not shown
```

dlmc-quant_amd/dlmc/utils/fuse.py:

```python
import math
import operator

import torch
import torch.fx as fx
import torch.nn.functional as F
from torch import nn

from .. import _native as N
from ..quantization.scalar import kernels as K
from ..quantization.scalar._wrapper import int8_kind, ste_scale_value
from ..quantization.scalar.FSPTQuant.base import FSPTQBase
from ..quantization.scalar.modules.base import QBase
from ..quantization.scalar.RootQ.base import RootQBase

__all__ = ["fuse_inference", "StreamedPlan", "Int8Layer", "DualInt8Layer", "StemLayer", "GapLayer", "GapHeadLayer", "AvgPoolLayer", "FusionReport"]


class _ActSpec:

    def __init__(self, scale, zp, lo, hi, form, needs_g, xoff=False):
        self.scale, self.zp, self.lo, self.hi, self.form, self.needs_g = scale, zp, int(lo), int(hi), form, needs_g
        self.xoff = bool(xoff)
        self.key = (form, self.lo, self.hi, float(scale.reshape(-1)[0]), 0.0 if zp is None else float(zp.reshape(-1)[0]),
                    needs_g)
        self.zp_emit = None if self.key[4] == 0.0 else zp

    def g(self, numel):
        return 1 / math.sqrt(numel * self.hi) if self.needs_g else 0.0

    def emit(self, numel):
        return K.EmitCodes(self.scale, self.zp_emit, self.lo, self.hi, self.form, self.g(numel))


def _byte_range(lo, hi):
    return (0 <= lo and hi <= 255) or (-128 <= lo and hi <= 127)


def _ceil64(n):
    return (n + 63) // 64 * 64


def plan_kind(mod):
    k = int8_kind(mod)
    if k is not None:
        return k
    w = mod.weight
    sq = lambda t: len(set(t)) == 1
    if w.dim() != 4 or mod.padding_mode != "zeros" or isinstance(mod.padding, str) or not (sq(mod.stride) and sq(mod.padding)):
        return None
    if tuple(mod.dilation) != (1, 1):
        return None
    if mod.groups == 1 and w.shape[1] % 4 == 0 and w.shape[1] > 4:
        return "gemm"
    if mod.groups == w.shape[0] and w.shape[1] == 1 and w.shape[0] % 4 == 0 and w.shape[2] <= 7 and w.shape[3] <= 7:
        return "dw"
    return None


def _frozen_spec(mod, act_offsets=False):
    kind = plan_kind(mod)
    if kind is None:
        return None
    spec = _frozen_spec_(mod, kind, act_offsets)
    if spec is None:
        return None
    if len(spec) == 4:
        spec = spec + (None, None)
    return spec[:4] + (kind,) + spec[4:]


def _xoff_kernel_exists(mod, kind):
    w = mod.weight
    if w.dim() != 4 or int(mod.padding[0]) == 0 or kind == "gemm":
        return True
    if kind == "dw":
        return tuple(w.shape[2:]) == (3, 3) and _ceil64(w.shape[0]) <= 2048
    return w.shape[2] in (3, 7)


def _frozen_spec_(mod, kind, act_offsets=False):
    if isinstance(mod, FSPTQBase):
        if not (mod.act_quant and mod.wt_quant) or mod.in_scale.numel() != 1:
            return None
        if mod.qconfig["weight"].get("recon_type") in ("adaround", "dist_recon"):
            return None
        if not (mod._init.ready(mod, "in_init_state") and mod._init.ready(mod, "wt_init_state")):
            raise RuntimeError("fuse_inference: run a calibration forward first (scales are not initialised)")
        if not (_byte_range(mod.in_min_val, mod.in_max_val) and -128 <= mod.wt_min_val and mod.wt_max_val <= 127):
            return None
        zp = mod.in_offset.detach().to(torch.float32).reshape(-1)[:1].clone()
        z = float(zp[0])
        if z != round(z) or not (mod.in_min_val <= z <= mod.in_max_val):
            return None
        act = _ActSpec(mod.in_scale.detach().reshape(-1)[:1].clone(), zp, mod.in_min_val, mod.in_max_val,
                       N.FORM_ZEROPOINT, False)
        return act, mod.wt_scale.detach().clone(), mod.wt_min_val, mod.wt_max_val
    if isinstance(mod, QBase):
        cfg = mod.qconfig
        if not (cfg["input"]["enable"] and cfg["weight"]["enable"]):
            return None
        k = mod.weight.shape[0]
        per_channel = mod.wt_scale.numel() != 1
        if mod.in_scale.numel() != 1 or (per_channel and (mod.wt_scale.numel() != k or mod.wt_scale.shape[0] != k)):
            return None
        if not (mod._init.ready(mod, "in_init_state") and mod._init.ready(mod, "wt_init_state")):
            raise RuntimeError("fuse_inference: run a calibration forward first (scales are not initialised)")
        lo, hi = mod.wt_min_val, mod.wt_max_val
        if not (_byte_range(mod.in_min_val, mod.in_max_val) and _byte_range(lo, hi)):
            return None
        xoff = float(mod.in_offset.abs().max()) != 0
        if xoff and not (act_offsets and mod.in_offset.numel() == 1 and _xoff_kernel_exists(mod, kind)):
            return None
        asym = mod.wt_offset is not None and float(mod.wt_offset.abs().max()) != 0
        act = _ActSpec(mod.in_scale.detach().reshape(-1)[:1].clone(),
                       mod.in_offset.detach().to(torch.float32).reshape(-1)[:1].clone() if xoff else None, mod.in_min_val, mod.in_max_val,
                       N.FORM_QBASE, True, xoff=xoff)
        g_w = 1 / math.sqrt(mod.weight.numel() * hi)
        s_hat = ste_scale_value(mod.wt_scale, g_w).clone()
        if not (per_channel or asym or hi > 127 or kind == "dw"):
            return act, s_hat, lo, hi
        w_off = mod.wt_offset.detach().to(torch.float32).reshape(-1).clone() if asym else None

        def codes(mod=mod, g_w=g_w, lo=lo, hi=hi):
            off = mod.wt_offset if mod.wt_offset is not None else None
            return K.fake_quant(mod.weight.detach(), mod.wt_scale.detach(), off, lo, hi, N.FORM_QBASE, g=g_w, codes="i8",
                                want_y=False)[1]
        return act, s_hat, lo, hi, w_off, codes
    return None


class _PlanLayer(nn.Module):

    def __init__(self, layer, spec, relu=False, emit=None, want_out=True, pool=None, relu6=False):
        super().__init__()
        self.layer = layer
        self.act, w_scale, self.w_lo, self.w_hi, self.kind, w_off, self._w_codes = spec
        self.relu, self.emit, self.want_out, self.pool = bool(relu), emit, bool(want_out), pool
        self.relu6 = bool(relu6)
        k = layer.weight.shape[0]
        self.k, self.k_pad = k, (_ceil64(k) if self.kind in ("gemm", "dw") and layer.weight.dim() == 4 else k)
        w_scale = w_scale.detach().to(torch.float32).reshape(-1)
        w_scale = w_scale.expand(k) if w_scale.numel() == 1 else w_scale
        self.register_buffer("w_scale", self._padk(w_scale, 1.0), persistent=False)
        if w_off is not None:
            w_off = w_off.expand(k) if w_off.numel() == 1 else w_off
        self.register_buffer("w_off", None if w_off is None else self._padk(w_off.to(w_scale.device), 0.0), persistent=False)
        self.register_buffer("bias_pad", None if layer.bias is None or self.k_pad == k else self._padk(layer.bias.detach().float(), 0.0),
                             persistent=False)
        self._kzp = None if self.act.xoff else self.act.zp
        self._zp_fill = int(0 if self._kzp is None else float(self._kzp.reshape(-1)[0]))
        self.emit_shift = False
        zs = None
        if self.act.lo >= 0:
# ... 86 lines not shown


class Int8Layer(_PlanLayer):

    def __init__(self, layer, spec, **kw):
        super().__init__(layer, spec, **kw)
        w = layer.weight.detach()
        c = w.shape[1]
        self.c, self.c_pad = c, (_ceil64(c) if w.dim() == 4 else c)
        if self._w_codes is None and self.c_pad == c and self.k_pad == self.k:
            wq, wsum = K.quantize_weight_krsc(w, self.w_scale, self.w_lo, self.w_hi)
        else:
            if self._w_codes is not None:
                q = _weight_codes(self)
            else:
                q4 = w if w.dim() == 4 else w[:, :, None, None]
                q = K.quantize_weight_krsc(q4, self.w_scale[:self.k], self.w_lo, self.w_hi)[0].permute(0, 3, 1, 2).to(torch.int16)
            full = torch.zeros((self.k_pad, self.c_pad) + tuple(q.shape[2:]), dtype=torch.int16, device=q.device)
            full[:self.k, :c] = q
            wq = full.permute(0, 2, 3, 1).contiguous().to(torch.int8)
            wsum = full.sum(dim=(1, 2, 3)).to(torch.int32).contiguous()
        self.register_buffer("wq", wq, persistent=False)
        self.register_buffer("wsum", wsum, persistent=False)
        if self.act.xoff:
            q = wq.reshape(self.k_pad, -1, self.c_pad)[:, :, :c].to(torch.float64)
            tap = q.sum(dim=2) * self.w_scale.to(torch.float64)[:, None]
            if self.w_off is not None:
                tap = tap + c * self.w_off.to(torch.float64)[:, None]
            r, s_ = (w.shape[2], w.shape[3]) if w.dim() == 4 else (1, 1)
            self._fold_offset(tap.reshape(self.k_pad, r, s_))

    def _codes(self, x):
        act = self.act
        if x.dtype not in (torch.uint8, torch.int8):
            N.require_gpu(x)
            if x.dim() == 4 and not x.is_contiguous(memory_format=torch.channels_last):
                x = x.contiguous(memory_format=torch.channels_last)
            x = K.fake_quant(x, act.scale, act.zp, act.lo, act.hi, act.form, g=act.g(x.numel()), codes="i8", want_y=False)[1]
        c_pad = getattr(self, "c_pad", x.shape[1])
        if x.dim() == 4 and x.shape[1] != c_pad:
            x = _pad_channels(x, c_pad, self._zp_fill)
        elif act.xoff and x.dim() == 4 and self.c != c_pad and self.w_off is not None:
            x[:, self.c:] = -128 if (x.dtype == torch.int8 and act.lo >= 0) else 0
        return x

    def _real_numel(self, codes):
        return codes.numel() // codes.shape[1] * self.c if codes.dim() == 4 else codes.numel()

    def _conv_kw(self):
        lay = self.layer
        return {} if lay.weight.dim() == 2 else dict(stride=lay.stride[0], padding=lay.padding[0], dilation=lay.dilation[0])

    def _out_hw(self, codes):
        lay = self.layer
        if lay.weight.dim() == 2:
            return 1, 1
        st, pd, dl = lay.stride[0], lay.padding[0], lay.dilation[0]
        r, s = lay.weight.shape[2], lay.weight.shape[3]
        return (codes.shape[2] + 2 * pd - dl * (r - 1) - 1) // st + 1, (codes.shape[3] + 2 * pd - dl * (s - 1) - 1) // st + 1

    def operand(self, x, codes=None):
        codes = self._codes(x) if codes is None else codes
        return dict(codes=codes, wq=self.wq, wsum=self.wsum, bias=self._bias(), in_scale=self._in_scale(self._real_numel(codes)),
                    in_zp=self._zp(codes), w_scale=self.w_scale, **self._conv_kw())

    def forward(self, x, residual=None):
        lay, act = self.layer, self.act
        linear = lay.weight.dim() == 2
        lead = None
        if linear and x.dim() != 2:
            lead = x.shape[:-1]
            x = x.reshape(-1, x.shape[-1])
            if residual is not None:
                residual = residual.reshape(-1, residual.shape[-1])
        codes = self._codes(x)
        numel = self._real_numel(codes)
        emit = self._emit_for(codes.shape[0], lay.weight.shape[0], *self._out_hw(codes))
        kw = self._conv_kw()
        if self.w_off is not None:
            kw["w_offset"] = self.w_off
        kw.update(self._xoff_kw())
        if self.narrow or self.pad_shortcut is not None:
            kw["out_channels"] = self.k
        if self.pad_shortcut is not None:
            residual = K.PadShortcut(K._nhwc(residual), *self.pad_shortcut)
        if self.relu or self.relu6 or residual is not None or emit is not None or self.w_off is not None or self.xoff_padded:
            res = K.conv2d_i8(codes, self.wq, self.wsum, self._bias(), self._in_scale(numel), self._zp(codes), self.w_scale,
                              residual=residual, act=self._act_arg(), emit=emit, want_out=self.want_out,
                              out_chunk_major=getattr(self, "out_cm", False), **kw)
            out, out_codes = res if emit is not None else (res, None)
        else:
            out, out_codes = K.conv2d_i8(codes, self.wq, self.wsum, self._bias(), self._in_scale(numel), self._zp(codes), self.w_scale, **kw), None
        if lead is not None:
            out = None if out is None else out.reshape(*lead, out.shape[-1])
            out_codes = None if out_codes is None else out_codes.reshape(*lead, out_codes.shape[-1])
        return self._finish(out, out_codes)


class DwInt8Layer(Int8Layer):

    def __init__(self, layer, spec, **kw):
        _PlanLayer.__init__(self, layer, spec, **kw)
        w = layer.weight.detach()
        self.c, self.c_pad = self.k, self.k_pad
        if self._w_codes is not None:
            q = _weight_codes(self)
        else:
            q = K.quantize_weight_krsc(w, self.w_scale[:self.k], self.w_lo, self.w_hi)[0].permute(0, 3, 1, 2).to(torch.int16)
        full = torch.zeros((self.k_pad,) + tuple(q.shape[2:]), dtype=torch.int16, device=q.device)
        full[:self.k] = q[:, 0]
        self.register_buffer("wq", full.permute(1, 2, 0).contiguous().to(torch.int8), persistent=False)
        if self.act.xoff:
            tap = full.to(torch.float64) * self.w_scale.to(torch.float64)[:, None, None]
            if self.w_off is not None:
                tap = tap + self.w_off.to(torch.float64)[:, None, None]
                tap[self.k:] = 0.0
            self._fold_offset(tap)

    def forward(self, x):
        lay, act = self.layer, self.act
        codes = self._codes(x)
        numel = self._real_numel(codes)
        emit = self._emit_for(codes.shape[0], self.k, *self._out_hw(codes))
        res = K.conv2d_dw_i8(codes, self.wq, self._bias(), self._in_scale(numel), self._zp(codes), self.w_scale, self.w_off,
                             stride=lay.stride[0], padding=lay.padding[0], act=self._act_arg(), emit=emit, want_out=self.want_out,
                             **self._xoff_kw())
        out, out_codes = res if emit is not None else (res, None)
        return self._finish(out, out_codes)


class DualInt8Layer(nn.Module):

    def __init__(self, a, b):
        super().__init__()
        self.a, self.b = a, b

    def forward(self, x, y):
        a = self.a
        oa, ob = a.operand(x), self.b.operand(y)
        emit = a._emit_for(oa["codes"].shape[0], a.layer.weight.shape[0], *a._out_hw(oa["codes"]))
        res = K.conv2d_i8_dual(oa, ob, relu=a.relu, emit=emit, want_out=a.want_out, out_chunk_major=getattr(self, "out_cm", False))
        out, out_codes = res if emit is not None else (res, None)
        return a._finish(out, out_codes)


class ChainInt8Layer(nn.Module):

    def __init__(self, a, b, want_codes, short=None, main=None):
        super().__init__()
        self.a, self.b, self.want_codes, self.short, self.main = a, b, bool(want_codes), short, (main if main is not None else a)
        self.swapped = short is not None and self.main is not a
        self._w2cm = None
        self.out_cm = False

    def forward(self, x, y):
        a, b, sc, mn = self.a, self.b, self.short, self.main
        if self.swapped:
            x, y = y, x
        codes = mn._codes(x)
        n, c, h, w = codes.shape
        nxt = dict(wq=b.wq, wsum=b.wsum, bias=b._bias(), w_scale=b.w_scale)
        if not getattr(b, "_packed4", False):
            if self._w2cm is None or self._w2cm.device != b.wq.device:
                self._w2cm = K.chunk_major(b.wq)
            nxt["wq_chunk"] = self._w2cm
        kw = dict(relu=a.relu, emit=a._emit_for(n, a.k, h, w), want_out=a.want_out, want_codes=self.want_codes, emit2=b._emit_for(n, b.k, h, w),
                  out_chunk_major=self.out_cm)
        if sc is None:
            if not K.chain_supported(c, a.k, b.k, n * h * w):
                if isinstance(y, K.ChunkMajor):
                    y = y.to_nhwc()
                out, mid = a(x, y)
                return out, (mid if self.want_codes else None), b(mid)[1]
            return K.conv2d_i8_chain(a.operand(x, codes), nxt, y, relu2=b.relu, **kw)
        if not K.dual_chain_supported(c, sc.c, a.k, b.k, n * h * w):
            out, mid = DualInt8Layer(a, sc if mn is a else mn)(*((x, y) if mn is a else (y, x)))
            return out, (mid if self.want_codes else None), b(mid)[1]
        kw["emit3"] = kw.pop("emit2")
        return K.conv2d_i8_dual_chain(mn.operand(x), sc.operand(y), nxt, relu3=b.relu, **kw)


class DwPwInt8Layer(nn.Module):

    def __init__(self, dw, pw):
        super().__init__()
        self.dw, self.pw = dw, pw
        self._tables = {}

    def forward(self, x):
        dw, pw = self.dw, self.pw
        codes = dw._codes(x)
        n, c, h, w = codes.shape
        lay = dw.layer
        if not K.dwpw_supported(c, pw.k_pad, h, w, lay.stride[0], lay.padding[0], lay.weight.shape[2]) or pw.c_pad != c:
            return pw(dw(x)[1])
        numel = dw._real_numel(codes)
        key = (numel, codes.dtype == torch.uint8, dw.wq.data_ptr())
        table = self._tables.get(key)
        if table is None:
            self._tables.clear()
            table = self._tables[key] = K.dwpw_table(dw.wq, dw._bias(), dw._in_scale(numel), dw._zp(codes), dw.w_scale, dw.w_off,
                                                     x_unsigned=codes.dtype == torch.uint8)
        emit = dw._emit_for(n, dw.k, h, w)
        emit2 = pw._emit_for(n, pw.layer.weight.shape[0], h, w)
        op = dict(wq=pw.wq, wsum=pw.wsum, bias=pw._bias(), w_scale=pw.w_scale, w_offset=pw.w_off, in_scale=pw._in_scale(n * h * w * pw.c))
        out = K.conv2d_dwpw_i8(codes, table, dw.w_off is not None, dw._bias() is not None, dw.relu, dw._zp(codes), emit, op, relu=pw.relu, emit2=emit2)
        return pw._finish(None, out)


def _dwpw_pass(gm, report):
    graph = gm.graph
    modules = dict(gm.named_modules())
    count = 0
    for nd in list(graph.nodes):
        dw = modules.get(nd.target) if nd.op == "call_module" else None
        if type(dw) is not DwInt8Layer or len(nd.args) != 1:
            continue
        lay = dw.layer
        if dw.relu6 or dw.act.xoff:
            continue
        if not (tuple(lay.weight.shape[2:]) == (3, 3) and lay.stride[0] == 1 and lay.padding[0] == 1 and lay.dilation[0] == 1 and dw.pool is None and
                dw.emit is not None and not dw.want_out and (dw.emit.lo, dw.emit.hi) == (0, 255) and not dw.emit_shift and dw.k_pad % 64 == 0):
            continue
        gets = {u.args[1]: u for u in nd.users if u.op == "call_function" and u.target is operator.getitem}
        if len(gets) != len(nd.users) or 1 not in gets or (0 in gets and gets[0].users):
            continue
        g1 = gets[1]
        if len(g1.users) != 1:
            continue
        npw = next(iter(g1.users))
        pw = modules.get(npw.target) if npw.op == "call_module" else None
        if type(pw) is not Int8Layer or npw.args != (g1,) or pw.relu6 or pw.act.xoff:
            continue
        pl = pw.layer
        if not (pl.weight.dim() == 4 and tuple(pl.weight.shape[2:]) == (1, 1) and pl.stride[0] == 1 and pl.padding[0] == 0 and pw.pool is None and
                pw.emit is not None and not pw.want_out and not pw.emit_shift and pw.c_pad == dw.k_pad and pw.k_pad in K.DWPW_WIDTHS):
            continue
        pgets = {u.args[1]: u for u in npw.users if u.op == "call_function" and u.target is operator.getitem}
        if len(pgets) != len(npw.users) or (0 in pgets and pgets[0].users):
            continue
        name = f"_int8_dwpw_{count}"
        count += 1
        gm.add_module(name, DwPwInt8Layer(dw, pw))
        with graph.inserting_after(npw):
            nc = graph.call_module(name, args=nd.args)
        with graph.inserting_after(nc):
            codes = graph.call_function(operator.getitem, (nc, 1))
        if 1 in pgets:
            pgets[1].replace_all_uses_with(codes)
        for n in list(pgets.values()) + [npw] + list(gets.values()) + [nd]:
            graph.erase_node(n)
    report.dwpw = count
    if count:
        graph.eliminate_dead_code()
        graph.lint()
        gm.recompile()


def _pointwise(plan):
    lay = plan.layer
    return (type(plan) is Int8Layer and lay.weight.dim() == 4 and tuple(lay.weight.shape[2:]) == (1, 1) and lay.stride[0] == 1 and
            lay.padding[0] == 0 and plan.w_off is None and plan.pool is None and plan.k_pad == plan.k and plan.c_pad == plan.c and
            not plan.act.needs_g and not plan.relu6 and
            plan.pad_shortcut is None)


def _chain_pass(gm, report):
    graph = gm.graph
    modules = dict(gm.named_modules())
    count = 0
    for na in list(graph.nodes):
        if na.op != "call_module" or len(na.args) != 2 or not isinstance(modules.get(na.target), (Int8Layer, DualInt8Layer)):
            continue
        a, main, short = modules[na.target], None, None
        if isinstance(a, DualInt8Layer):
            a, other = a.a, a.b
            main, short = (a, other) if _pointwise(a) else (other, a)
            lay = short.layer
            if not (_pointwise(main) and type(short) is Int8Layer and lay.weight.dim() == 4 and tuple(lay.weight.shape[2:]) == (1, 1) and
                    lay.padding[0] == 0 and short.w_off is None and short.pool is None and short.k_pad == short.k and
                    short.c_pad == short.c and not short.act.needs_g and a.pool is None and a.w_off is None):
                continue
        elif not _pointwise(a):
            continue
        if not (a.emit is not None and (a.emit.lo, a.emit.hi) == (0, 255) and not a.emit.needs_g):
            continue
        mc = (main if main is not None else a).c
        gets = {u.args[1]: u for u in na.users if u.op == "call_function" and u.target is operator.getitem}
        if len(gets) != len(na.users) or 1 not in gets:
            continue
        g1 = gets[1]
        nb = next((u for u in g1.users if u.op == "call_module" and u.args == (g1,) and isinstance(modules.get(u.target), Int8Layer) and
                   _pointwise(modules[u.target]) and modules[u.target].emit is not None and not modules[u.target].want_out and
                   not modules[u.target].emit.needs_g and modules[u.target].c == a.k and
                   ((mc, modules[u.target].k) in K.CHAIN_SHAPES if short is None else
                    (mc, short.c, modules[u.target].k) in K.DUAL_CHAIN_SHAPES)), None)
        if nb is None:
            continue
        b = modules[nb.target]
        bgets = {u.args[1]: u for u in nb.users if u.op == "call_function" and u.target is operator.getitem}
        if len(bgets) != len(nb.users) or (0 in bgets and bgets[0].users):
            continue
        name = f"_int8_chain_{count}"
        count += 1
        a.emit_shift = False
        gm.add_module(name, ChainInt8Layer(a, b, want_codes=len(g1.users) > 1, short=short, main=main))
        with graph.inserting_after(na):
            nc = graph.call_module(name, args=na.args)
        with graph.inserting_after(nc):
            outs = [graph.call_function(operator.getitem, (nc, i)) for i in (2, 1, 0)][::-1]
        if 0 in gets:
            gets[0].replace_all_uses_with(outs[0])
        for u in list(g1.users):
            if u is not nb:
                u.replace_input_with(g1, outs[1])
        if 1 in bgets:
            bgets[1].replace_all_uses_with(outs[2])
        for n in list(bgets.values()) + [nb] + list(gets.values()) + [na]:
            graph.erase_node(n)
    report.chained = count
    if count:
        graph.eliminate_dead_code()
        graph.lint()
        gm.recompile()


def _block_end_like(m):
    return (type(m) is Int8Layer and _pointwise(m) and m.c in (256, 512) and m.k % 128 == 0 and m.k_pad == m.k and m.c_pad == m.c and m.relu
            and m.w_off is None and m.pool is None and m.layer.stride[0] == 1 and not m.act.needs_g and
            (m.emit is None or ((m.emit.lo, m.emit.hi) == (0, 255) and not m.emit.needs_g)))


def _block_layout_pass(gm, report):
    graph = gm.graph
    modules = dict(gm.named_modules())

    def mod(node):
        return modules.get(node.target) if node.op == "call_module" else None

    def writer(m):
        if isinstance(m, ChainInt8Layer):
            return m.a.k % 64 == 0
        if isinstance(m, DualInt8Layer):
            one = lambda t: type(t) is Int8Layer and t.layer.weight.dim() == 4 and tuple(t.layer.weight.shape[2:]) == (1, 1)
            dense, other = (m.a, m.b) if m.a.c == 256 else (m.b, m.a)
            return (one(m.a) and one(m.b) and (dense.c, other.c) == (256, 512) and dense.layer.stride[0] == 1 and m.a.relu and m.a.k % 128 == 0
                    and m.a.k_pad == m.a.k and m.a.w_off is None and m.b.w_off is None and m.a.pool is None and m.a.emit is not None)
        return isinstance(m, Int8Layer) and _block_end_like(m)

    def reader(node, o):
        m = mod(node)
        if len(node.args) != 2 or node.args[1] is not o or node.args[0] is o:
            return False
        if isinstance(m, ChainInt8Layer):
            return m.short is None
        return isinstance(m, Int8Layer) and _block_end_like(m)

    def one_layout(m):
        if isinstance(m, ChainInt8Layer):
            return m.short is None and (m.main.c, m.b.k) in K.CHAIN_ONE_LAYOUT
        return True
    nodes = [n for n in graph.nodes if isinstance(mod(n), (ChainInt8Layer, DualInt8Layer, Int8Layer))]
    out_node, src, cm = {}, {}, {}
    for nd in nodes:
        for u in nd.users:
            if u.op == "call_function" and u.target is operator.getitem and u.args[1] == 0 and u.users:
                out_node[nd] = u
    for nd, o in out_node.items():
        cm[nd] = writer(mod(nd)) and all(reader(r, o) for r in o.users)
        if cm[nd]:
            for r in o.users:
                src[r] = nd
    changed = True
    while changed:
        changed = False
        for nd in nodes:
            m = mod(nd)
            has_shortcut = len(nd.args) == 2 and not isinstance(m, DualInt8Layer) and not (isinstance(m, ChainInt8Layer) and m.short is not None)
            if nd not in out_node or not has_shortcut or not one_layout(m):
                continue
            icm, ocm = cm.get(src.get(nd), False), cm.get(nd, False)
            if icm and not ocm:
                cm[src[nd]] = False
                changed = True
            elif ocm and not icm:
                cm[nd] = False
                changed = True
    count = 0
    for nd, flag in cm.items():
        mod(nd).out_cm = bool(flag)
        count += bool(flag)
    report.chunk_major = count


class GapLayer(nn.Module):

    def __init__(self, emit, want_out):
        super().__init__()
        self.emit, self.want_out = emit, bool(want_out)

    def forward(self, x):
        n, c = x.shape[0], x.shape[1]
        return K.global_avgpool(x, emit=self.emit.emit(n * c), want_out=self.want_out)


class GapHeadLayer(nn.Module):

    def __init__(self, a, emit, want_out):
        super().__init__()
        self.a, self.emit, self.want_out = a, emit, bool(want_out)

    def forward(self, x, residual=None):
        a = self.a
        codes = a._codes(x)
        n, c, h, w = codes.shape
        emit = self.emit.emit(n * a.k)
        if not K.gap_head_supported(c, a.k, h, w):
            return K.global_avgpool(a(codes, residual)[0], emit=emit, want_out=self.want_out)
        return K.conv2d_i8_gap(codes, a.wq, a.wsum, a._bias(), a._in_scale(a._real_numel(codes)), a._zp(codes), a.w_scale,
                               residual=residual, act=a._act_arg(), emit=emit, want_out=self.want_out)


class AvgPoolLayer(nn.Module):

    def __init__(self, window, emit, want_out, c, c_pad, pad_code, shift=False):
        super().__init__()
        self.window, self.emit, self.want_out = int(window), emit, bool(want_out)
        self.c, self.c_pad, self.pad_code, self.emit_shift = int(c), int(c_pad), int(pad_code), bool(shift)

    def forward(self, x):
        n, c, h, w = x.shape
        s = self.window
        e = self.emit.emit(n * c * (h // s) * (w // s))
        e.shift128 = self.emit_shift
        return K.avgpool_quant(x, s, emit=e, want_out=self.want_out, c_pad=self.c_pad, pad_code=self.pad_code)


_AVGPOOL_NAMES = ("input", "kernel_size", "stride", "padding", "ceil_mode", "count_include_pad", "divisor_override")


def _avgpool_window(node, modules):
    if node.op == "call_module":
        m = modules.get(node.target)
        if type(m) is not nn.AvgPool2d or len(node.args) != 1 or node.kwargs:
            return None
        given = dict(input=node.args[0], kernel_size=m.kernel_size, stride=m.stride, padding=m.padding, ceil_mode=m.ceil_mode,
                     divisor_override=m.divisor_override)
    elif node.op == "call_function" and node.target in (F.avg_pool2d, torch._C._nn.avg_pool2d):
        if len(node.args) > len(_AVGPOOL_NAMES) or not set(node.kwargs) <= set(_AVGPOOL_NAMES[len(node.args):]):
            return None
        given = dict(zip(_AVGPOOL_NAMES, node.args), **node.kwargs)
    else:
        return None

    def one(v):
        if isinstance(v, (tuple, list)) and len(v) in (1, 2) and len(set(v)) == 1:
            v = v[0]
        return v if isinstance(v, int) and not isinstance(v, bool) else None
    x, k = given.get("input"), one(given.get("kernel_size"))
    stride, pad = given.get("stride"), given.get("padding", 0)
    if not isinstance(x, fx.Node) or k is None or not 2 <= k <= 8:
        return None
    if not (stride is None or (isinstance(stride, (tuple, list)) and len(stride) == 0) or one(stride) == k):
        return None
    if one(pad) != 0 or given.get("ceil_mode", False) is not False or given.get("divisor_override") is not None:
        return None
    return x, k


def _avgpool_pass(gm, report, planned, dry_run):
    graph = gm.graph
    modules = dict(gm.named_modules())
    count = 0

    def reader(u, pool):
        info = planned.get(u)
        if info is None or info["kind"] != "gemm":
            return None
        if info["dual"]:
            ops = [(info["dual_inputs"][i], (info["mod"], info["dual_mod"])[i]) for i in (0, 1) if u.args[i] is pool]
            if not ops or len({a.key for a, _ in ops}) != 1:
                return None
        elif u.args[0] is pool and pool not in u.args[1:]:
            ops = [(info["spec"][0], info["mod"])]
        else:
            return None
        a, m = ops[0]
        return (a, m) if m.weight.dim() == 4 and m.groups == 1 and all(mm.weight.shape[1] == m.weight.shape[1] for _, mm in ops) else None

    for pool in list(graph.nodes):
        win = _avgpool_window(pool, modules)
        if win is None:
            continue
        x, s = win
        readers = {u: reader(u, pool) for u in pool.users}
        takers = [u for u, r in readers.items() if r is not None]
        if not takers or len({readers[u][0].key for u in takers}) != 1:
# ... 63 lines not shown
        given = dict(zip(("input", "start_dim", "end_dim"), node.args), **node.kwargs)
        return 2 if given.get("start_dim") == 1 and given.get("end_dim", -1) in (-1, rank - 1) and set(given) <= {"input", "start_dim", "end_dim"} else None
    if meth and node.target in ("view", "reshape") and not node.kwargs:
        shape = node.args[1:]
        if len(shape) == 1 and isinstance(shape[0], (tuple, list)):
            shape = tuple(shape[0])
        return 2 if len(shape) == 2 and shape[1] == -1 and _batch_size_of(shape[0]) else None
    if (fn and node.target is torch.squeeze) or (meth and node.target == "squeeze"):
        given = dict(zip(("input", "dim"), node.args), **node.kwargs)
        if set(given) == {"input"}:
            return 2
        d = given.get("dim")
        if set(given) != {"input", "dim"} or not isinstance(d, int) or isinstance(d, bool):
            return None
        d = d if d >= 0 else rank + d
        return rank - 1 if 2 <= d < rank else None
    return None


def _gap_pass(gm, report, mode, planned, dry_run):
    graph = gm.graph
    modules = dict(gm.named_modules())
    count = 0

    def aux(n, inside):
        if not ((n.op == "call_method" and n.target == "size") or (n.op == "call_function" and n.target in (getattr, operator.getitem))):
            return False
        return bool(n.users) and all(u in inside or aux(u, inside) for u in n.users)

    def real_users(n, inside):
        return [u for u in n.users if not aux(u, inside)]

    for pool in list(graph.nodes):
        rank = _pool_dims(pool, modules)
        if rank is None:
            continue
        x = pool.args[0] if pool.args else pool.kwargs["input"]
        chain, last = [pool], pool
        while True:
            nxt = [u for u in last.users if _flatten_rank(u, last, rank) is not None]
            if len(nxt) != 1 or len(real_users(last, set(chain) | set(nxt))) != 1:
                break
            rank = _flatten_rank(nxt[0], last, rank)
            chain.append(nxt[0])
            last = nxt[0]
        if rank != 2:
            continue
        inside = set(chain)
        if any(real_users(n, inside) != [c] for n, c in zip(chain[:-1], chain[1:])):
            continue
        def linear_act(u):
            info = planned.get(u)
            if info is None or info["dual"] or info["kind"] != "gemm" or u.args[0] is not last or last in u.args[1:]:
                return None
            w = info["mod"].weight
            return info["spec"][0] if w.dim() == 2 and w.shape[1] % 64 == 0 else None
        users = real_users(last, inside)
        acts = {u: linear_act(u) for u in users}
        keys = [a.key for a in acts.values() if a is not None]
        if not keys:
            continue
        key = max(set(keys), key=keys.count)
        takers = [u for u, a in acts.items() if a is not None and a.key == key]
        emit = acts[takers[0]]
        want_out = len(takers) != len(users)
        prod = x.args[0] if x.op == "call_function" and x.target is operator.getitem and x.args[1] == 0 else None
        info = planned.get(prod)
        fused = False
        if mode in (True, "fused") and info is not None and real_users(x, inside) == [pool]:
            w = info["mod"].weight
            gets = [u for u in prod.users if u.op == "call_function" and u.target is operator.getitem]
            fused = (info["kind"] == "gemm" and not info["dual"] and info["pool"] is None and info["emit"] is None and w.dim() == 4 and
                     info.get("pad_shortcut") is None and
                     len(gets) == len(prod.users) and all(g is x or not real_users(g, inside) for g in gets) and info["spec"][5] is None and
                     K.gap_head_supported(_ceil64(w.shape[1]), w.shape[0], 1, 1, w.shape[2], info["mod"].stride[0], info["mod"].padding[0]) and
                     w.shape[2] == w.shape[3] and (mode == "fused" or K.gap_head_profitable(_ceil64(w.shape[1]), w.shape[0])))
        name = f"_int8_gap_{count}"
        count += 1
        if dry_run:
            gm.add_module(name, _DryNode())
        elif fused:
            gm.add_module(name, GapHeadLayer(modules[prod.target], emit, want_out))
        else:
            gm.add_module(name, GapLayer(emit, want_out))
        with graph.inserting_after(last):
            node = graph.call_module(name, args=tuple(prod.args) if fused else (x,))
        with graph.inserting_after(node):
            out = graph.call_function(operator.getitem, (node, 0))
            codes = graph.call_function(operator.getitem, (node, 1))
        for u in users:
            u.replace_input_with(last, codes if u in takers else out)
        def erase_tree(n):
            for u in list(n.users):
                erase_tree(u)
            if n in live:
                live.discard(n)
                graph.erase_node(n)
        live = set(graph.nodes)
        erase_tree(pool)
        if fused:
            erase_tree(prod)
            report.fp32_outputs -= 1
        report.gap_heads.append((name, "fused" if fused else "separate"))
    if count:
        graph.eliminate_dead_code()
        graph.lint()
        gm.recompile()


class StemLayer(_PlanLayer):

    def __init__(self, layer, spec, **kw):
        super().__init__(layer, spec, **kw)
        self.c = layer.weight.shape[1]
        if self._w_codes is None:
            wq, wsum = K.quantize_weight_stem(layer.weight, self.w_scale, self.w_lo, self.w_hi)
        else:
            q = _weight_codes(self)
            k, c, r, s_ = q.shape
            full = torch.zeros((k, r, 8, 4), dtype=torch.int16, device=q.device)
            full[:, :, :s_, :c] = q.permute(0, 2, 3, 1)
            wq, wsum = full.to(torch.int8).contiguous(), q.sum(dim=(1, 2, 3)).to(torch.int32).contiguous()
        self.register_buffer("wq", wq, persistent=False)
        self.register_buffer("wsum", wsum, persistent=False)
        if self.act.xoff:
            _, _, r, s_ = layer.weight.shape
            tap = wq[:, :, :s_, :self.c].to(torch.float64).sum(dim=3) * self.w_scale.to(torch.float64)[:, None, None]
            if self.w_off is not None:
                tap = tap + self.c * self.w_off.to(torch.float64)[:, None, None]
            self._fold_offset(tap)

    def forward(self, x):
        lay, act = self.layer, self.act
        numel = x.numel()
        pad, st = lay.padding[0], lay.stride[0]
        k, _, r, s = lay.weight.shape
        emit = self._emit_for(x.shape[0], k, (x.shape[2] + 2 * pad - r) // st + 1, (x.shape[3] + 2 * pad - s) // st + 1)
        in_kernel = self.pool == (3, 2, 1) and k <= 64 and self.w_off is None and not self.relu6 and not act.xoff
        shifted = act.lo >= 0
        xpad = K.quantize_pad_nhwc4(x, act.scale, act.zp, act.lo, act.hi, act.form, pad, g=act.g(numel), shift128=shifted, pad_code0=act.xoff)
        xkw = dict(self._xoff_kw(), pad=pad) if self.xoff_padded else {}
        res = K.conv2d_i8_stem(xpad, self.wq, self.wsum, self._bias() if act.xoff else lay.bias, self._in_scale(numel),
                               self.zp_shift if shifted else self._kzp, self.w_scale, s, stride=st, act=self._act_arg(), emit=emit,
                               want_out=self.want_out, pool=in_kernel, w_offset=self.w_off, channels=self.c, **xkw)
        out, out_codes = res if emit is not None else (res, None)
        return (out, out_codes) if in_kernel else self._finish(out, out_codes)


class _DryNode(nn.Module):
    def forward(self, *args):
        raise RuntimeError("fuse_inference(dry_run=True) builds the plan's structure only")


class FusionReport:

    def __init__(self):
        self.layers = self.relu = self.residual = self.emit = self.fp32_outputs = self.stem = self.pooled = self.dual = 0
        self.relu6 = 0
        self.chained = 0
        self.chunk_major = 0
        self.dwpw = 0
        self.act_offset = 0
        self.narrow = 0
        self.pad_shortcuts = 0
        self.avg_pools = 0
        self.gap_heads = []
        self.skipped = []

    def __repr__(self):
        return (f"FusionReport(int8 layers={self.layers}, relu fused={self.relu}, relu6 fused={self.relu6}, residual fused={self.residual}, "
                f"code-emitting={self.emit}, fp32 outputs kept={self.fp32_outputs}, stem layers={self.stem}, "
                f"pools on codes={self.pooled}, dual (conv + shortcut conv) kernels={self.dual}, chained pairs={self.chained} (fp32 outputs chunk-major: {self.chunk_major}), "
                f"depthwise + pointwise units={self.dwpw}, " + (f"gap heads={self.gap_heads}, " if self.gap_heads else "") +
                (f"narrow fp32 rows={self.narrow}, " if self.narrow else "") +
                (f"pad shortcuts={self.pad_shortcuts}, " if self.pad_shortcuts else "") +
                (f"average pools on the plan={self.avg_pools}, " if self.avg_pools else "") +
                f"not eligible={self.skipped})")


class _Tracer(fx.Tracer):
    def is_leaf_module(self, m, qualname):
        return isinstance(m, (QBase, FSPTQBase, RootQBase)) or super().is_leaf_module(m, qualname)


_ADD_FNS = (operator.add, operator.iadd, torch.add)
_RELU_FNS = (F.relu, torch.relu, torch.relu_, F.relu_)


def _is_add(node):
    if node.kwargs:
        return False
    if node.op == "call_function" and node.target in _ADD_FNS:
        return len(node.args) == 2 and all(isinstance(a, fx.Node) for a in node.args)
    if node.op == "call_method" and node.target in ("add", "add_"):
        return len(node.args) == 2 and all(isinstance(a, fx.Node) for a in node.args)
    return False


def _inplace_add(node):
    return (node.op == "call_method" and node.target == "add_") or (node.op == "call_function" and node.target is operator.iadd)


def _is_relu(node, modules):
    if node.op == "call_module":
        return type(modules.get(node.target)) is nn.ReLU
    if node.op == "call_function":
        return node.target in _RELU_FNS
    return node.op == "call_method" and node.target in ("relu", "relu_")


def _is_relu6(node, modules):
    if node.op == "call_module":
        m = modules.get(node.target)
        return isinstance(m, nn.Hardtanh) and type(m) in (nn.ReLU6, nn.Hardtanh) and m.min_val == 0.0 and m.max_val == 6.0
    if node.op != "call_function":
        return False
    if node.target is F.relu6:
        return len(node.args) == 1 and set(node.kwargs) <= {"inplace"}
    if node.target in (F.hardtanh, F.hardtanh_):
        names = ("min_val", "max_val", "inplace") if node.target is F.hardtanh else ("min_val", "max_val")
        if len(node.args) > 1 + len(names) or not set(node.kwargs) <= set(names):
            return False
        given = dict(zip(names, node.args[1:]), **node.kwargs)
        lo, hi = given.get("min_val", -1.0), given.get("max_val", 1.0)
        return (isinstance(lo, (int, float)) and isinstance(hi, (int, float)) and not isinstance(lo, bool) and not isinstance(hi, bool)
                and float(lo) == 0.0 and float(hi) == 6.0)
    return False


_PAD_FNS = tuple({F.pad, torch._C._nn.pad})


def _pad_shortcut(node):
    if node.op != "call_function" or node.target not in _PAD_FNS or len(node.users) != 1:
        return None
    names = ("input", "pad", "mode", "value")
    if len(node.args) > len(names) or not set(node.kwargs) <= set(names[len(node.args):]):
        return None
    given = dict(zip(names, node.args), **node.kwargs)
    t, pad, mode, value = given.get("input"), given.get("pad"), given.get("mode", "constant"), given.get("value", None)
    if not isinstance(t, fx.Node) or not isinstance(pad, (tuple, list)) or len(pad) != 6 or mode != "constant":
        return None
    if not all(isinstance(v, int) and not isinstance(v, bool) for v in pad) or tuple(pad[:4]) != (0, 0, 0, 0) or pad[4] < 0 or pad[5] < 0:
        return None
    if not (value is None or (isinstance(value, (int, float)) and not isinstance(value, bool) and float(value) == 0.0)):
        return None
    if not (t.op == "call_function" and t.target is operator.getitem and len(t.args) == 2 and not isinstance(t.args[1], int)):
        return t, 1, int(pad[4]), int(pad[5]), [node]
    if len(t.users) != 1 or t.kwargs or not isinstance(t.args[0], fx.Node) or not isinstance(t.args[1], tuple):
        return None
    idx = t.args[1]
    full = slice(None, None, None)
    if len(idx) != 4 or idx[0] != full or idx[1] != full or not all(isinstance(i, slice) for i in idx):
        return None
    s = idx[2].step
    if (idx[2].start, idx[2].stop, idx[3].start, idx[3].stop) != (None,) * 4 or not isinstance(s, int) or isinstance(s, bool) or s < 1 or idx[3].step != s:
        return None
    return t.args[0], s, int(pad[4]), int(pad[5]), [node, t]


def _pool_params(node, modules):
    if node.op != "call_module" or type(modules.get(node.target)) is not nn.MaxPool2d:
        return None
    m = modules[node.target]
    one = lambda v: v[0] if isinstance(v, (tuple, list)) and len(set(v)) == 1 else (v if isinstance(v, int) else None)
    k, s, p, d = one(m.kernel_size), one(m.stride if m.stride is not None else m.kernel_size), one(m.padding), one(m.dilation)
    if None in (k, s, p, d) or d != 1 or m.ceil_mode or m.return_indices:
        return None
    return k, s, p


class PackedWeights4(nn.Module):

    def __init__(self, nodes, signed):
        super().__init__()
        self.signed = bool(signed)
        sizes = [n.wq.numel() for n in nodes]
        offs, total = [], 0
        for sz in sizes:
            offs.append(total)
            total += (sz + 31) // 32 * 32
        dev = nodes[0].wq.device
        flat = torch.zeros(total, dtype=torch.int8, device=dev)
        for n, o, sz in zip(nodes, offs, sizes):
            flat[o:o + sz] = n.wq.reshape(-1)
        self.register_buffer("packed", K.pack_int4(flat), persistent=False)
        self.register_buffer("scratch", torch.empty(total, dtype=torch.int8, device=dev), persistent=False)
        self.n = total
        for n, o, sz in zip(nodes, offs, sizes):
            n._buffers["wq"] = self.scratch[o:o + sz].view(n.wq.shape)
            n._packed4 = True
        self.expand()

    def expand(self):
        K.unpack_int4(self.packed, self.n, self.signed, out=self.scratch)


def _pack_plan_weights(gm):
    groups = {True: [], False: []}
    for m in gm.modules():
        if isinstance(m, _PlanLayer) and hasattr(m, "wq") and m.wq.dtype == torch.int8 and -8 <= m.w_lo and m.w_hi <= 15:
            lo, hi = int(m.wq.min()), int(m.wq.max())
            if 0 <= lo and hi <= 15:
                groups[False].append(m)
            elif -8 <= lo and hi <= 7:
                groups[True].append(m)
    holders = [PackedWeights4(nodes, signed) for signed, nodes in groups.items() if nodes]
    for i, h in enumerate(holders):
        gm.add_module(f"_packed_weights_{i}", h)
    if holders:
        gm.register_forward_pre_hook(lambda mod, args: [h.expand() for h in holders] and None)
    return holders


class EagerFused:

    def __init__(self, model):
        try:
            graph = _Tracer().trace(model)
        except Exception as e:
            raise RuntimeError(f"EagerFused reads the model's dataflow with torch.fx and could not trace it ({type(e).__name__}: {e})") from e
        self.gm = fx.GraphModule(model, graph)
        modules = dict(self.gm.named_modules())
        for node in list(graph.nodes):
            if node.op == "call_module" and isinstance(modules[node.target], (nn.Identity, nn.Dropout)) and len(node.args) == 1 and \
                    not (isinstance(modules[node.target], nn.Dropout) and model.training):
                node.replace_all_uses_with(node.args[0])
                graph.erase_node(node)
        self.gm.recompile()
        self.chains = {}
        taken = set()
        for node in graph.nodes:
            if node.op != "call_module" or len(node.args) != 1 or node.kwargs or not hasattr(modules[node.target], "forward_fused"):
                continue
            add = short = relu = None
            users = list(node.users)
            if len(users) == 1 and _is_add(users[0]) and users[0].args[0] is not users[0].args[1]:
                if users[0] in taken:
                    continue
                if _inplace_add(users[0]) and users[0].args[0] is not node:
                    continue
                add = users[0]
                taken.add(add)
                short = add.args[1] if add.args[0] is node else add.args[0]
                users = list(add.users)
            if len(users) == 1 and _is_relu(users[0], modules):
                relu = users[0]
            if add is not None or relu is not None:
                self.chains[node] = (add, short, relu)

    def __call__(self, *args):
        from ..quantization.scalar._wrapper import ZeroPointSpeculation
        with ZeroPointSpeculation() as sp:
            interp = _EagerInterp(self.gm, self.chains)
            out = interp.run(*args)
        self.speculation = {"layers": len(sp.pending), "held": True}
        if not sp.verify():
            sp.rearm()
            self.speculation["held"] = False
            interp = _EagerInterp(self.gm, self.chains)
            out = interp.run(*args)
        self.last_states = {n.target: ("fused" if st == "fused" else "plain") for n, st in interp.state.items()}
        return out


class _EagerInterp(fx.Interpreter):
    def __init__(self, gm, chains):
        super().__init__(gm)
        self.chains = chains
        self.add_of = {c[0]: n for n, c in chains.items() if c[0] is not None}
        self.relu_of = {c[2]: n for n, c in chains.items() if c[2] is not None}
        self.state = {}

    def _launch(self, node, layer, x, short):
        add, _, relu = self.chains[node]
        if add is not None and not self._fusable_shortcut(layer, x, short):
            self.state[node] = "plain"
            return None
        y = layer.forward_fused(x, residual=short, relu=relu is not None, observe_out=True)
        self.state[node] = "plain" if y is None else "fused"
        return y

    @staticmethod
    def _fusable_shortcut(layer, x, short):
        if not isinstance(short, torch.Tensor) or short.dtype != torch.float32 or short.device != x.device:
            return False
        w = layer.weight
        if w.dim() == 2:
            return tuple(short.shape) == (*x.shape[:-1], w.shape[0])
        if x.dim() != 4:
            return False
        def side(n, k, s, p, d):
            return (n + 2 * p - d * (k - 1) - 1) // s + 1
        p = layer.padding if not isinstance(layer.padding, str) else None
        if p is None:
            return False
        return tuple(short.shape) == (x.shape[0], w.shape[0], side(x.shape[2], w.shape[2], layer.stride[0], p[0], layer.dilation[0]),
                                      side(x.shape[3], w.shape[3], layer.stride[1], p[1], layer.dilation[1]))

    def run_node(self, n):
        if n in self.chains:
            add, short, _ = self.chains[n]
            layer = self.fetch_attr(n.target)
            (x,), _ = self.fetch_args_kwargs_from_env(n)
            if add is not None and short not in self.env:
                self.state[n] = ("pending", layer, x)
                return None
            y = self._launch(n, layer, x, self.env[short] if add is not None else None)
            return layer(x) if y is None else y
        if n in self.add_of:
            c = self.add_of[n]
            st = self.state.get(c)
            if st == "fused":
                return self.env[c]
            if isinstance(st, tuple):
                _, layer, x = st
                short = self.env[self.chains[c][1]]
                y = self._launch(c, layer, x, short)
                if y is not None:
                    return y
                self.env[c] = layer(x)
        elif n in self.relu_of:
            if self.state.get(self.relu_of[n]) == "fused":
                (v,), _ = self.fetch_args_kwargs_from_env(n)
                return v
        return super().run_node(n)


def _codes_from_blob(mod_name, blob, layer):
    rec = blob["layers"].get(mod_name)
    if rec is None:
        return None
    dev = layer.weight.device
    n = int(torch.tensor(rec["shape"]).prod())
    if rec["packed_int4"]:
        q = K.unpack_int4(rec["codes"].to(dev), n, rec["lo"] < 0)
    else:
        q = rec["codes"].to(dev)
    return q.reshape(rec["shape"]).to(torch.int16)


def fuse_inference(model, report=None, dry_run=False, chain_pairs=True, pack_int4=True, weight_blob=None, dwpw=False, block_layout=True,
                   relu6=True, act_offsets=False, gap_head=False, narrow_rows=False, pad_shortcuts=False, avg_pools=False):
    if not any(gap_head is v for v in (False, True)) and gap_head not in ("separate", "fused"):
        raise ValueError(f"fuse_inference: gap_head is False, True, 'separate' or 'fused', not {gap_head!r}")
    if model.training:
        raise RuntimeError("fuse_inference: the plan is for inference - call model.eval() first")
    report = report if report is not None else FusionReport()
    try:
        graph = _Tracer().trace(model)
    except Exception as e:
        raise RuntimeError(f"fuse_inference reads the model's dataflow with torch.fx and could not trace it ({type(e).__name__}: "
                           f"{e}); the module-by-module path (quantize_model(..., int8_gemm=True)) needs no tracing") from e
    gm = fx.GraphModule(model, graph)
    modules = dict(gm.named_modules())
    specs = {}

    def spec_of(node):
        if node.op != "call_module" or len(node.args) != 1 or node.kwargs:
            return None
        if node.target not in specs:
            mod = modules[node.target]
            specs[node.target] = _frozen_spec(mod, act_offsets) if isinstance(mod, (QBase, FSPTQBase)) else None
            if specs[node.target] is None and isinstance(mod, (QBase, FSPTQBase, RootQBase)):
                report.skipped.append(node.target)
        return specs[node.target]

    for node in list(graph.nodes):
        if node.op == "call_module" and isinstance(modules[node.target], (nn.Identity, nn.Dropout)) and len(node.args) == 1:
            node.replace_all_uses_with(node.args[0])
            graph.erase_node(node)

    dual_inputs = {}

    def accepts(u, t):
        if u in dual_inputs:
            acts = {dual_inputs[u][i].key: dual_inputs[u][i] for i in (0, 1) if u.args[i] is t}
            return next(iter(acts.values())) if len(acts) == 1 else None
        s = spec_of(u) if u.args and u.args[0] is t else None
        return s[0] if s is not None and s[4] in ("gemm", "dw") else None

    def source_channels(src):
        if src.op == "call_function" and src.target is operator.getitem and src.args[1] == 0 and src.args[0] in planned:
            info = planned[src.args[0]]
            w = info["mod"].weight
            ok = w.dim() == 4 and info["kind"] in ("gemm", "dw") and info["pool"] is None and (w.shape[0] % 64 == 0 or info["narrow"])
            return int(w.shape[0]) if ok else None
        if src.op == "placeholder":
            for u in src.users:
                info = planned.get(u)
                if info is not None and u.args[0] is src and info["mod"].weight.dim() == 4 and info["mod"].groups == 1:
                    return int(info["mod"].weight.shape[1])
        return None

    count = 0
    planned = {}
    live = set(graph.nodes)
    for node in list(graph.nodes):
        if node not in live:
            continue
        spec = spec_of(node)
        if spec is None:
            continue
        chain, last, residual, relu, act6 = [node], node, None, False, False
        users = list(last.users)
        wn = modules[node.target].weight
        unpadded = wn.dim() != 4 or wn.shape[0] % 64 == 0
        can_narrow = (narrow_rows and spec[4] == "gemm" and not unpadded and wn.shape[0] % 4 == 0 and
                      not (spec[0].xoff and int(modules[node.target].padding[0]) > 0))
        if spec[4] == "gemm" and (unpadded or can_narrow) and len(users) == 1 and _is_add(users[0]) and users[0].args[0] is not users[0].args[1]:
            add = users[0]
            residual = add.args[1] if add.args[0] is last else add.args[0]
            chain.append(add)
            last = add
            users = list(last.users)
        if len(users) == 1 and _is_relu(users[0], modules):
            relu = True
            chain.append(users[0])
            last = users[0]
            users = list(last.users)
        elif relu6 and len(users) == 1 and _is_relu6(users[0], modules):
            act6 = True
            chain.append(users[0])
            last = users[0]
            users = list(last.users)
        pool = None
        if len(users) == 1 and _pool_params(users[0], modules) is not None and modules[node.target].weight.shape[0] % 4 == 0:
            mp = users[0]
            cons = [accepts(u, mp) for u in mp.users]
            on_codes = cons and all(c is not None for c in cons) and len({c.key for c in cons}) == 1
            in_stem = (spec[4] == "stem" and _pool_params(mp, modules) == (3, 2, 1) and modules[node.target].weight.shape[0] <= 64 and
                       spec[5] is None and not act6 and not spec[0].xoff)
            if on_codes or in_stem:
                pool = _pool_params(mp, modules)
                chain.append(mp)
                last = mp
        pad_sc = None
        if (pad_shortcuts and residual is not None and residual.op == "call_function" and
                not (spec[0].xoff and int(modules[node.target].padding[0]) > 0)):
            m = _pad_shortcut(residual)
            cs = source_channels(m[0]) if m is not None else None
            if cs is not None and m[2] % 4 == 0 and cs % 4 == 0 and cs >= 4 and m[2] + cs + m[3] == wn.shape[0]:
                pad_sc = m
        consumers = {}
        fp32_needed = False
        for u in last.users:
            a = accepts(u, last)
            if a is None:
                fp32_needed = True
            else:
                consumers.setdefault(a.key, []).append((u, a))
        emit, takers = None, []
        if consumers:
            key = max(consumers, key=lambda k: len(consumers[k]))
            takers = [u for u, _ in consumers[key]]
            emit = consumers[key][0][1]
            fp32_needed = fp32_needed or len(consumers) > 1
        if not last.users:
            fp32_needed = True
        name = f"_int8_plan_{count}"
        count += 1
        specs[name] = None
        modules[name] = None
        cls = {"gemm": Int8Layer, "dw": DwInt8Layer}.get(spec[4], StemLayer)
        other = spec_of(residual) if residual is not None and residual.op == "call_module" else None
        dual = (other is not None and unpadded and other[4] == "gemm" and spec[5] is None and other[5] is None and list(residual.users) == [chain[1]] and
                modules[node.target].weight.dim() == 4 and modules[residual.target].weight.dim() == 4 and not act6 and
                not any(sp[0].xoff and int(modules[t].padding[0]) > 0 for sp, t in ((spec, node.target), (other, residual.target))))
        narrow = bool(can_narrow and (fp32_needed or emit is None or residual is not None))
        if dry_run:
            gm.add_module(name, _DryNode())
        else:
            def from_blob(name, sp):
                if weight_blob is None or name not in weight_blob["layers"]:
                    return sp
                return sp[:6] + ((lambda name=name: _codes_from_blob(name, weight_blob, modules[name])),)
            spec = from_blob(node.target, spec)
            if other is not None and dual:
                other = from_blob(residual.target, other)
            plan = cls(modules[node.target], spec, relu=relu, emit=emit, want_out=fp32_needed or emit is None, pool=pool, relu6=act6)
            plan.narrow = narrow
            if pad_sc is not None:
                plan.pad_shortcut = (pad_sc[1], pad_sc[2])
            def takes_shifted(u):
                sp = spec_of(u) if u.op == "call_module" else None
                m = modules.get(u.target) if u.op == "call_module" else None
                if sp is None or m is None or m.weight.dim() != 4:
                    return False
                if sp[4] == "dw":
                    return (not dwpw and m.kernel_size == (3, 3) and m.stride == (1, 1) and m.padding == (1, 1) and m.weight.shape[0] % 64 == 0)
                return sp[4] == "gemm" and m.groups == 1 and m.weight.shape[1] % 64 == 0
            plan.emit_shift = bool(cls is Int8Layer and emit is not None and 0 <= emit.lo and emit.hi <= 255 and pool is None and
                                   plan.k_pad == plan.k and takers and all(takes_shifted(u) for u in takers))
            gm.add_module(name, DualInt8Layer(plan, Int8Layer(modules[residual.target], other)) if dual else plan)
        if dual:
            args = (node.args[0], residual.args[0])
        else:
            args = (node.args[0],) if residual is None else (node.args[0], residual if pad_sc is None else pad_sc[0])
        with graph.inserting_after(last):
            fused = graph.call_module(name, args=args)
        planned[fused] = dict(spec=spec, kind=spec[4], mod=modules[node.target], dual=bool(dual), pool=pool, emit=emit, narrow=narrow,
                              pad_shortcut=pad_sc)
        if dual:
            dual_inputs[fused] = (spec[0], other[0])
            planned[fused].update(dual_inputs=dual_inputs[fused], dual_mod=modules[residual.target])
            chain.insert(0, residual)
            specs[residual.target] = None
            report.layers += 1
            report.dual += 1
        with graph.inserting_after(fused):
            out = graph.call_function(operator.getitem, (fused, 0))
            codes = graph.call_function(operator.getitem, (fused, 1))
        for u in list(last.users):
            if u in (out, codes):
                continue
            u.replace_input_with(last, codes if u in takers else out)
        for n in reversed(chain[1:] if dual else chain):
            graph.erase_node(n)
        if dual:
            graph.erase_node(residual)
            live.discard(residual)
        if pad_sc is not None:
            for n in pad_sc[4]:
                graph.erase_node(n)
                live.discard(n)
        report.pad_shortcuts += pad_sc is not None
        report.layers += 1
        report.stem += spec[4] == "stem"
        report.pooled += pool is not None
        report.relu += relu
        report.relu6 += act6
        report.act_offset += spec[0].xoff + (dual and other[0].xoff)
        report.residual += residual is not None
        report.narrow += narrow
        report.emit += emit is not None
        report.fp32_outputs += bool(fp32_needed or emit is None)
    graph.eliminate_dead_code()
    graph.lint()
    gm.recompile()
    if avg_pools:
        _avgpool_pass(gm, report, planned, dry_run)
    if gap_head:
        _gap_pass(gm, report, gap_head, planned, dry_run)
    if chain_pairs and not dry_run:
        _chain_pass(gm, report)
        if block_layout:
            _block_layout_pass(gm, report)
        if dwpw:
            _dwpw_pass(gm, report)
    gm.packed_weights = _pack_plan_weights(gm) if (pack_int4 and not dry_run) else []
    gm.fusion_report = report
    return gm


_STREAM_POOL = {}


def _plan_streams(device, n):
    device = torch.device(device)
    key = (device.type, device.index if device.index is not None else torch.cuda.current_device())
    pool = _STREAM_POOL.setdefault(key, [])
    while len(pool) < n:
        pool.append(torch.cuda.Stream(device=device))
    return pool[:n]


class StreamedPlan:

    def __init__(self, plan, n_streams=2):
        if n_streams < 1:
            raise ValueError("n_streams must be >= 1")
        for m in plan.modules():
            if isinstance(m, _PlanLayer) and (m.act.needs_g or (m.emit is not None and m.emit.needs_g)):
                raise ValueError("StreamedPlan: this plan holds QBase quantisers whose scale depends on the number of "
                                 "elements per call (grad_scale); splitting the batch would change the result")
        self.plan, self.n = plan, int(n_streams)
        self.streams = None

    def __call__(self, x):
        if self.n == 1 or x.shape[0] < self.n:
            return self.plan(x)
        if self.streams is None:
            self.streams = _plan_streams(x.device, self.n)
        cur = torch.cuda.current_stream(x.device)
        parts = x.chunk(self.n, dim=0)
        outs = [None] * len(parts)
        for i, part in enumerate(parts):
            s = self.streams[i]
            s.wait_stream(cur)
            with torch.cuda.stream(s):
                outs[i] = self.plan(part)
        for s in self.streams[:len(parts)]:
            cur.wait_stream(s)
        for o, s in zip(outs, self.streams):
            o.record_stream(cur)
        return torch.cat(outs, dim=0)
```

include/dlmcq.h:

```cpp
#ifndef DLMCQ_H
#define DLMCQ_H

#include <stddef.h>
#include <stdint.h>

#ifdef __cplusplus
extern "C" {
#endif

#define DLMCQ_VERSION 100

typedef void* dlmcq_stream_t;

#define DLMCQ_OK 0
#define DLMCQ_EINVAL (-1)
#define DLMCQ_ERANGE (-2)
#define DLMCQ_ESCRATCH (-3)
#define DLMCQ_EALIGN (-4)

#define DLMCQ_FORM_EMULATE 0
#define DLMCQ_FORM_QBASE 1
#define DLMCQ_FORM_ZEROPOINT 2
#define DLMCQ_FORM_SYMMETRIC 3
#define DLMCQ_FORM_ROOTQ_ACT 4
// ... 113 lines not shown
                               dlmcq_stream_t stream);
int dlmcq_fake_quant_multi_bwd_f32(const dlmcq_fq_segment* table, int64_t nseg, int64_t bwd_workgroups,
                                   int64_t finalize_workgroups, void* scratch, size_t scratch_bytes,
                                   dlmcq_stream_t stream);

int dlmcq_rootq_weight_f32(const float* w, float* y, const float* bounds, int64_t n, int32_t lo,
                           int32_t hi, dlmcq_stream_t stream);

size_t dlmcq_rootq_bwd_scratch_bytes(int64_t n);
int dlmcq_rootq_weight_bwd_f32(const float* w, const float* gy, float* gw, float* g_bounds_alpha,
                               const float* bounds, const float* alpha, int64_t n, int32_t lo, int32_t hi,
                               void* scratch, size_t scratch_bytes, dlmcq_stream_t stream);


int dlmcq_fold_bn_f32(float* weight, float* bias, const float* gamma, const float* beta,
                      const float* mean, const float* var, int64_t out_channels, int64_t inner,
                      float var_eps, dlmcq_stream_t stream);

int dlmcq_repvgg_fuse_f32(const float* k3, const float* k1, float* out_kernel, float* out_bias,
                          const float* const* bn3, const float* const* bn1, const float* const* bnid,
                          float eps3, float eps1, float epsid, int64_t out_channels,
                          int64_t cin_per_group, dlmcq_stream_t stream);


size_t dlmcq_l2norm_scratch_bytes(int64_t outer, int64_t channels, int64_t inner);
int dlmcq_l2norm_step_f32(const float* x, const float* scale, const float* offset, float* new_scale,
                          int64_t outer, int64_t channels, int64_t inner, int32_t lo, int32_t hi,
                          void* scratch, size_t scratch_bytes, dlmcq_stream_t stream);

int dlmcq_l2norm_iterate_f32(const float* x, float* scale, const float* offset, float* state, int64_t outer,
                             int64_t channels, int64_t inner, int32_t lo, int32_t hi, int32_t iterations, float eps,
                             void* scratch, size_t scratch_bytes, dlmcq_stream_t stream);

size_t dlmcq_l2out_scratch_bytes(int64_t outer, int64_t channels, int64_t inner);
int dlmcq_l2out_update_f32(const float* out, const float* out_q, float* scale, float* best_scale, float* state,
                           int64_t outer, int64_t channels, int64_t inner, int32_t per_channel, float mse_div, float eps,
                           void* scratch, size_t scratch_bytes, dlmcq_stream_t stream);

size_t dlmcq_l2loss_scratch_bytes(int64_t n);
int dlmcq_l2loss_tensor_f32(const float* x, const float* vmax, const float* vmin, float* scale, float* offset, int64_t n,
                            int32_t n_bits, float loss_div, void* scratch, size_t scratch_bytes, dlmcq_stream_t stream);

int dlmcq_l2loss_rows_f32(const float* x, float* scale, float* offset, int64_t rows, int64_t inner, int32_t n_bits,
                          dlmcq_stream_t stream);

int dlmcq_adaround_weight_f32(const float* w, const float* alpha, const float* scale, float* y,
                              int64_t out_channels, int64_t inner, int32_t lo, int32_t hi,
                              int32_t training, dlmcq_stream_t stream);
int dlmcq_adaround_weight_bwd_f32(const float* w, const float* alpha, const float* scale,
                                  const float* gy, float* g_alpha, float* g_scale,
                                  int64_t out_channels, int64_t inner, int32_t lo, int32_t hi,
                                  dlmcq_stream_t stream);


int dlmcq_quantize_weight_krsc_i8(const float* w, int8_t* wq, int32_t* wsum, const float* scale,
                                  int64_t K, int64_t C, int64_t R, int64_t S, int32_t lo, int32_t hi,
                                  dlmcq_stream_t stream);

int dlmcq_conv2d_i8_nhwc_f32(const void* x, const int8_t* w, float* out, const float* bias,
                             const int32_t* wsum, const float* in_scale, const float* in_zero_point,
                             const float* w_scale, int64_t N, int64_t H, int64_t W, int64_t C, int64_t K,
                             int64_t R, int64_t S, int32_t stride, int32_t pad, int32_t dilation,
                             int32_t x_is_unsigned, dlmcq_stream_t stream);

int dlmcq_conv2d_i8_nhwc_fused(const void* x, const int8_t* w, float* out, const float* bias,
                               const int32_t* wsum, const float* in_scale, const float* in_zero_point,
                               const float* w_scale, int64_t N, int64_t H, int64_t W, int64_t C, int64_t K,
                               int64_t R, int64_t S, int32_t stride, int32_t pad, int32_t dilation,
                               int32_t x_is_unsigned, const float* residual, int32_t relu, void* codes,
                               const float* q_scale, const float* q_zero_point, int32_t q_lo, int32_t q_hi,
                               int32_t q_form, float q_ste_g, dlmcq_stream_t stream);

size_t dlmcq_conv2d_i8_observed_partials(int64_t M, int64_t K);
int dlmcq_conv2d_i8_nhwc_fused_observed(const void* x, const int8_t* w, float* out, const float* bias, const int32_t* wsum,
                                        const float* in_scale, const float* in_zero_point, const float* w_scale, int64_t N,
                                        int64_t H, int64_t W, int64_t C, int64_t K, int64_t R, int64_t S, int32_t stride,
                                        int32_t pad, int32_t dilation, int32_t x_is_unsigned, const float* residual,
                                        int32_t relu, void* codes, const float* q_scale, const float* q_zero_point,
                                        int32_t q_lo, int32_t q_hi, int32_t q_form, float q_ste_g, float* partials,
                                        int64_t partials_capacity, int64_t* partials_count, dlmcq_stream_t stream);

int dlmcq_conv2d_i8_nhwc_asym(const void* x, const int8_t* w, float* out, const float* bias, const int32_t* wsum,
                              const float* in_scale, const float* in_zero_point, const float* w_scale, const float* w_offset,
                              int64_t N, int64_t H, int64_t W, int64_t C, int64_t K, int64_t R, int64_t S, int32_t stride,
                              int32_t pad, int32_t dilation, int32_t x_is_unsigned, const float* residual, int32_t relu,
                              void* codes, const float* q_scale, const float* q_zero_point, int32_t q_lo, int32_t q_hi,
                              int32_t q_form, float q_ste_g, dlmcq_stream_t stream);

int dlmcq_conv2d_i8_nhwc_narrow(const void* x, const int8_t* w, float* out, const float* bias, const int32_t* wsum,
                                const float* in_scale, const float* in_zero_point, const float* w_scale, const float* w_offset,
                                int64_t N, int64_t H, int64_t W, int64_t C, int64_t K, int64_t R, int64_t S, int32_t stride,
                                int32_t pad, int32_t dilation, int32_t x_is_unsigned, const float* residual, int32_t relu,
                                void* codes, const float* q_scale, const float* q_zero_point, int32_t q_lo, int32_t q_hi,
                                int32_t q_form, float q_ste_g, int64_t Kf, dlmcq_stream_t stream);

int dlmcq_conv2d_i8_nhwc_padres(const void* x, const int8_t* w, float* out, const float* bias, const int32_t* wsum,
                                const float* in_scale, const float* in_zero_point, const float* w_scale, const float* w_offset,
                                int64_t N, int64_t H, int64_t W, int64_t C, int64_t K, int64_t R, int64_t S, int32_t stride,
                                int32_t pad, int32_t dilation, int32_t x_is_unsigned, const float* res_src, int64_t res_h,
                                int64_t res_w, int64_t res_c, int32_t res_stride, int64_t res_clo, int32_t relu, void* codes,
                                const float* q_scale, const float* q_zero_point, int32_t q_lo, int32_t q_hi, int32_t q_form,
                                float q_ste_g, int64_t Kf, dlmcq_stream_t stream);

int dlmcq_conv2d_dw_i8_nhwc(const void* x, const int8_t* w, float* out, const float* bias, const float* in_scale,
                            const float* in_zero_point, const float* w_scale, const float* w_offset, int64_t N, int64_t H,
                            int64_t W, int64_t C, int64_t R, int64_t S, int32_t stride, int32_t pad, int32_t x_is_unsigned,
                            int32_t relu, void* codes, const float* q_scale, const float* q_zero_point, int32_t q_lo,
                            int32_t q_hi, int32_t q_form, float q_ste_g, dlmcq_stream_t stream);

int dlmcq_dwpw_pack_table(const int8_t* w, const float* bias, const float* in_scale, const float* in_zero_point,
                          const float* w_scale, const float* w_offset, int64_t C, int32_t x_is_unsigned, void* table,
                          dlmcq_stream_t stream);
int dlmcq_conv2d_dwpw_i8_nhwc(const void* x, const void* dw_table, int32_t dw_asym, int32_t dw_bias, int32_t dw_relu,
                              const float* in_zero_point, int64_t N, int64_t H, int64_t W, int64_t C, int32_t x_is_unsigned,
                              const float* q_scale, const float* q_zero_point, int32_t q_lo, int32_t q_hi, int32_t q_form,
                              float q_ste_g, const int8_t* w, const float* bias, const int32_t* wsum, const float* pw_in_scale,
                              const float* w_scale, const float* w_offset, int64_t K, int32_t relu, void* codes,
                              const float* q2_scale, const float* q2_zero_point, int32_t q2_lo, int32_t q2_hi, int32_t q2_form,
                              float q2_ste_g, dlmcq_stream_t stream);

int dlmcq_conv2d_i8_nhwc_dual(const void* x, const int8_t* w, float* out, const float* bias,
                              const int32_t* wsum, const float* in_scale, const float* in_zero_point,
                              const float* w_scale, int64_t N, int64_t H, int64_t W, int64_t C, int64_t K,
                              int64_t R, int64_t S, int32_t stride, int32_t pad, int32_t dilation,
                              int32_t x_is_unsigned, const void* x2, const int8_t* w2, const float* bias2,
                              const int32_t* wsum2, const float* in_scale2, const float* in_zero_point2,
                              const float* w_scale2, int64_t H2, int64_t W2, int64_t C2, int64_t R2,
                              int64_t S2, int32_t stride2, int32_t pad2, int32_t dilation2,
                              int32_t x2_is_unsigned, int32_t relu, void* codes, const float* q_scale,
                              const float* q_zero_point, int32_t q_lo, int32_t q_hi, int32_t q_form,
                              float q_ste_g, dlmcq_stream_t stream);

int dlmcq_conv2d_i8_nhwc_chain(const void* x, const int8_t* w, float* out, const float* bias, const int32_t* wsum,
                               const float* in_scale, const float* in_zero_point, const float* w_scale, int64_t M,
                               int64_t C, int64_t K, int32_t x_is_unsigned, const float* residual, int32_t relu,
                               void* codes, const float* q_scale, const float* q_zero_point, int32_t q_lo,
                               int32_t q_hi, int32_t q_form, float q_ste_g, const int8_t* w2, const float* bias2,
                               const int32_t* wsum2, const float* w_scale2, int64_t K2, int32_t relu2, void* codes2,
                               const float* q2_scale, const float* q2_zero_point, int32_t q2_lo, int32_t q2_hi,
                               int32_t q2_form, float q2_ste_g, int32_t rows_per_tile, dlmcq_stream_t stream);

int dlmcq_conv2d_i8_nhwc_dual_chain(const void* x, const int8_t* w, float* out, const float* bias, const int32_t* wsum,
                                    const float* in_scale, const float* in_zero_point, const float* w_scale, int64_t N,
                                    int64_t H, int64_t W, int64_t C, int64_t K, int32_t x_is_unsigned, const void* x2,
                                    const int8_t* w2, const float* bias2, const int32_t* wsum2, const float* in_scale2,
                                    const float* in_zero_point2, const float* w_scale2, int64_t H2, int64_t W2, int64_t C2,
                                    int32_t stride2, int32_t x2_is_unsigned, int32_t relu, void* codes, const float* q_scale,
                                    const float* q_zero_point, int32_t q_lo, int32_t q_hi, int32_t q_form, float q_ste_g,
                                    const int8_t* w3, const float* bias3, const int32_t* wsum3, const float* w_scale3,
                                    int64_t K3, int32_t relu3, void* codes3, const float* q3_scale, const float* q3_zero_point,
                                    int32_t q3_lo, int32_t q3_hi, int32_t q3_form, float q3_ste_g, int32_t rows_per_tile,
                                    dlmcq_stream_t stream);


int dlmcq_quantize_pad_nhwc4(const float* x, void* out, const float* scale, const float* zero_point, int64_t N,
                             int64_t C, int64_t H, int64_t W, int64_t stride_n, int64_t stride_c, int64_t stride_h,
                             int64_t stride_w, int32_t pad, int32_t lo, int32_t hi, int32_t form, float ste_g,
                             dlmcq_stream_t stream);

int dlmcq_quantize_weight_stem_i8(const float* w, int8_t* wq, int32_t* wsum, const float* scale, int64_t K,
                                  int64_t C, int64_t R, int64_t S, int32_t lo, int32_t hi, dlmcq_stream_t stream);

int dlmcq_conv2d_i8_stem_fused(const void* xpad, const int8_t* w, float* out, const float* bias,
                               const int32_t* wsum, const float* in_scale, const float* in_zero_point,
                               const float* w_scale, int64_t N, int64_t Hp, int64_t Wp, int64_t K, int64_t R,
                               int64_t S, int32_t stride, int32_t x_is_unsigned, int32_t relu, void* codes,
                               const float* q_scale, const float* q_zero_point, int32_t q_lo, int32_t q_hi,
                               int32_t q_form, float q_ste_g, dlmcq_stream_t stream);

int dlmcq_conv2d_i8_stem_asym(const void* xpad, const int8_t* w, float* out, const float* bias, const int32_t* wsum,
                              const float* in_scale, const float* in_zero_point, const float* w_scale, const float* w_offset,
                              int64_t C, int64_t N, int64_t Hp, int64_t Wp, int64_t K, int64_t R, int64_t S, int32_t stride,
                              int32_t x_is_unsigned, int32_t relu, void* codes, const float* q_scale, const float* q_zero_point,
                              int32_t q_lo, int32_t q_hi, int32_t q_form, float q_ste_g, dlmcq_stream_t stream);

int dlmcq_conv2d_i8_stem_pool_fused(const void* xpad, const int8_t* w, float* out, const float* bias,
                                    const int32_t* wsum, const float* in_scale, const float* in_zero_point,
                                    const float* w_scale, int64_t N, int64_t Hp, int64_t Wp, int64_t K, int64_t R,
                                    int64_t S, int32_t stride, int32_t x_is_unsigned, int32_t relu, void* codes,
                                    const float* q_scale, const float* q_zero_point, int32_t q_lo, int32_t q_hi,
                                    int32_t q_form, float q_ste_g, dlmcq_stream_t stream);

int dlmcq_maxpool_codes_nhwc(const void* x, void* y, int64_t N, int64_t H, int64_t W, int64_t C, int32_t kernel,
                             int32_t stride, int32_t pad, int32_t x_is_unsigned, dlmcq_stream_t stream);

int dlmcq_conv2d_i8_nhwc_xoff(const void* x, const int8_t* w, float* out, const float* bias, const int32_t* wsum,
                              const float* in_scale, const float* in_zero_point, const float* w_scale, const float* w_offset,
                              int64_t N, int64_t H, int64_t W, int64_t C, int64_t K, int64_t R, int64_t S, int32_t stride,
                              int32_t pad, int32_t dilation, int32_t x_is_unsigned, const float* residual, int32_t relu, void* codes,
                              const float* q_scale, const float* q_zero_point, int32_t q_lo, int32_t q_hi, int32_t q_form,
                              float q_ste_g, const float* in_offset, const float* tap_sums, dlmcq_stream_t stream);
int dlmcq_conv2d_dw_i8_nhwc_xoff(const void* x, const int8_t* w, float* out, const float* bias, const float* in_scale,
                                 const float* in_zero_point, const float* w_scale, const float* w_offset, int64_t N, int64_t H,
                                 int64_t W, int64_t C, int64_t R, int64_t S, int32_t stride, int32_t pad, int32_t x_is_unsigned,
                                 int32_t relu, void* codes, const float* q_scale, const float* q_zero_point, int32_t q_lo,
                                 int32_t q_hi, int32_t q_form, float q_ste_g, const float* in_offset, const float* tap_sums,
                                 dlmcq_stream_t stream);
int dlmcq_conv2d_i8_stem_xoff(const void* xpad, const int8_t* w, float* out, const float* bias, const int32_t* wsum,
                              const float* in_scale, const float* in_zero_point, const float* w_scale, const float* w_offset,
                              int64_t C, int64_t N, int64_t Hp, int64_t Wp, int64_t K, int64_t R, int64_t S, int32_t stride,
                              int32_t pad, int32_t x_is_unsigned, int32_t relu, void* codes, const float* q_scale,
                              const float* q_zero_point, int32_t q_lo, int32_t q_hi, int32_t q_form, float q_ste_g,
                              const float* in_offset, const float* tap_sums, dlmcq_stream_t stream);

#define DLMCQ_GAP_MAX_C 2048
int dlmcq_gap_nhwc_f32(const float* x, float* pooled, void* codes, int64_t N, int64_t HW, int64_t C, const float* q_scale,
                       const float* q_zero_point, int32_t q_lo, int32_t q_hi, int32_t q_form, float q_ste_g, dlmcq_stream_t stream);
int dlmcq_conv2d_i8_nhwc_gap(const void* x, const int8_t* w, float* pooled, const float* bias, const int32_t* wsum,
                             const float* in_scale, const float* in_zero_point, const float* w_scale, int64_t N, int64_t H,
                             int64_t W, int64_t C, int64_t K, int32_t x_is_unsigned, const float* residual, int32_t act,
                             void* codes, const float* q_scale, const float* q_zero_point, int32_t q_lo, int32_t q_hi,
                             int32_t q_form, float q_ste_g, dlmcq_stream_t stream);

int dlmcq_avgpool_nhwc_f32(const float* x, float* pooled, void* codes, int64_t N, int64_t H, int64_t W, int64_t C, int64_t x_stride,
                           int64_t window, int64_t c_pad, int32_t pad_code, const float* q_scale, const float* q_zero_point,
                           int32_t q_lo, int32_t q_hi, int32_t q_form, float q_ste_g, dlmcq_stream_t stream);

#ifdef __cplusplus
}
#endif
#endif
```

Before: 92360 images/s.

## Recompute block-end shortcut inside next chain kernel instead of storing fp32

Adds a recomputing form of the chain kernel that, instead of reading a stored fp32 residual, recomputes the previous block's output (main 1x1 conv plus shortcut conv) from their int8 inputs and adds it in the epilogue. A plan pass marks pairs where the producer defers its fp32 output and the consumer recomputes it, removing an fp32 residual write and read through memory. In exchange it spends extra MFMA work and LDS for two more operand sets, which can lower occupancy. The pass is gated by an environment default and a whitelist of channel shapes.

New measurement: 93910 images/s, median of 6. +1.7%, better.

```diff
diff --git a/dlmc-quant_amd/csrc/conv_chain_i8.hip b/dlmc-quant_amd/csrc/conv_chain_i8.hip
--- a/dlmc-quant_amd/csrc/conv_chain_i8.hip
+++ b/dlmc-quant_amd/csrc/conv_chain_i8.hip
@@ -21,6 +21,14 @@
   const float* zp_in2;
   int shift2, P, Q, H2, W2, stride2;
   FastDiv qdiv, pdiv;
+  const int8_t* xa;
+  const int8_t* wa;
+  const float* s_wa;
+  const int32_t* wsuma;
+  const float* biasa;
+  const float* s_ina;
+  const float* zp_ina;
+  int shifta, relu_sc;
   float* out;
   uint8_t* codes;
   const int8_t* w3;
@@ -52,16 +60,20 @@
 constexpr int CHAIN_WGS(int c1, int kb) { return c1 + kb <= 256 ? 3 : 2; }
 constexpr int CH_BIG = 0x7fff0000;
 
-template <int C1, int KB, int C2 = 0, int FL = -1>
-__global__ __launch_bounds__(256, CHAIN_WGS(C1 + C2, KB)) void conv_chain_i8_kernel(ChainArgs a, ConvEpi ep1, ConvEpi ep2) {
+template <int C1, int KB, int C2 = 0, int FL = -1, int CA = 0, int CB = 0>
+__global__ __launch_bounds__(256, CHAIN_WGS(C1 + C2 + CA + CB, KB)) void conv_chain_i8_kernel(ChainArgs a, ConvEpi ep1, ConvEpi ep2) {
   constexpr bool DUALH = C2 > 0;
+  constexpr bool RC = CA > 0;
+  static_assert(!RC || (C2 == 0 && CB > 0 && FL >= 0), "the recomputing form: two operands, no convolution shortcut of its own, flags known");
+  constexpr int SA = CA / 64, SB = CB / 64;
+  constexpr int W3U = C1 / 64 + C2 / 64 + SA + SB;
   const bool relu1 = FL < 0 ? ep1.relu != 0 : (FL & 1) != 0;
   const bool out1 = FL < 0 ? a.out != nullptr : (FL & 2) != 0;
   constexpr int S1 = C1 / 64;
   constexpr int S2 = C2 / 64;
   constexpr int U3 = KB / 64;
-  constexpr int WCH = (S1 + S2 + U3) * 4096;
-  constexpr int NPD = DUALH ? 2 : 1;
+  constexpr int WCH = (W3U + U3) * 4096;
+  constexpr int NPD = DUALH ? 2 : RC ? 3 : 1;
   constexpr int PAR = NPD * 4 * 256;
 #ifndef DLMCQ_CHAIN_LDS_T
 #define DLMCQ_CHAIN_LDS_T ((C1 == 128 && C2 == 256) ? 0 : 2)
@@ -127,6 +139,19 @@
       for (int s = 0; s < S2; ++s)
         __builtin_amdgcn_global_load_lds((gptr_t)(xp2 + s * 64), (lptr_t)(lds + WCH + (S1 + s) * 4096 + (tid >> 6) * 1024), 16, 0, 0);
     }
+    if constexpr (RC) {
+      const int8_t* xpa = a.xa + (row0 + (lrw < rows_here ? lrw : rows_here - 1)) * CA + sgw;
+#pragma unroll
+      for (int s = 0; s < SA; ++s)
+        __builtin_amdgcn_global_load_lds((gptr_t)(xpa + s * 64), (lptr_t)(lds + WCH + (S1 + s) * 4096 + (tid >> 6) * 1024), 16, 0, 0);
+      const uint32_t m = (uint32_t)(row0 + (lrw < rows_here ? lrw : rows_here - 1));
+      const uint32_t t = fdiv(m, a.qdiv), nn = fdiv(t, a.pdiv);
+      const int q = (int)(m - t * (uint32_t)a.Q), pp = (int)(t - nn * (uint32_t)a.P);
+      const int8_t* xpb = a.x2 + (((int64_t)nn * a.H2 + pp * a.stride2) * a.W2 + q * a.stride2) * CB + sgw;
+#pragma unroll
+      for (int s = 0; s < SB; ++s)
+        __builtin_amdgcn_global_load_lds((gptr_t)(xpb + s * 64), (lptr_t)(lds + WCH + (S1 + SA + s) * 4096 + (tid >> 6) * 1024), 16, 0, 0);
+    }
   }
   const float sin2 = ep1.q_scale[0];
   const float zpf2 = ep1.q_zp ? ep1.q_zp[0] : 0.0f;
@@ -139,6 +164,7 @@
   asm volatile("s_waitcnt vmcnt(0) lgkmcnt(0)\n\ts_barrier" ::: "memory");
   i32x4 af[S1][2];
   i32x4 af2[DUALH ? S2 : 1][2];
+  i32x4 afa[RC ? SA : 1][2], afb[RC ? SB : 1][2];
   {
     const int r = wr * 32 + l31;
     const int8_t* ab = lds + WCH + r * 64;
@@ -158,6 +184,23 @@
         for (int ks = 0; ks < 2; ++ks) {
           const i32x4 t = *reinterpret_cast<const i32x4*>(ab + (S1 + s) * 4096 + (((ks * 2 + hsel) ^ ((r >> 2) & 3)) << 4));
           af2[s][ks] = i32x4{(int)(t.x ^ xw2), (int)(t.y ^ xw2), (int)(t.z ^ xw2), (int)(t.w ^ xw2)};
+        }
+    }
+    if constexpr (RC) {
+      const uint32_t xwa = a.shifta ? 0x80808080u : 0u, xwb = a.shift2 ? 0x80808080u : 0u;
+#pragma unroll
+      for (int s = 0; s < SA; ++s)
+#pragma unroll
+        for (int ks = 0; ks < 2; ++ks) {
+          const i32x4 t = *reinterpret_cast<const i32x4*>(ab + (S1 + s) * 4096 + (((ks * 2 + hsel) ^ ((r >> 2) & 3)) << 4));
+          afa[s][ks] = i32x4{(int)(t.x ^ xwa), (int)(t.y ^ xwa), (int)(t.z ^ xwa), (int)(t.w ^ xwa)};
+        }
+#pragma unroll
+      for (int s = 0; s < SB; ++s)
+#pragma unroll
+        for (int ks = 0; ks < 2; ++ks) {
+          const i32x4 t = *reinterpret_cast<const i32x4*>(ab + (S1 + SA + s) * 4096 + (((ks * 2 + hsel) ^ ((r >> 2) & 3)) << 4));
+          afb[s][ks] = i32x4{(int)(t.x ^ xwb), (int)(t.y ^ xwb), (int)(t.z ^ xwb), (int)(t.w ^ xwb)};
         }
     }
   }
@@ -195,7 +238,7 @@
     }
   }
 #endif
-  constexpr bool MIXED_OK = !DUALH && !(C1 == 128 && KB == 128);
+  constexpr bool MIXED_OK = !DUALH && !RC && !(C1 == 128 && KB == 128);
   int fo2[MIXED_OK ? 4 : 1];
   const int cstep2 = a.o_cstep;
   if constexpr (MIXED_OK) {
@@ -229,6 +272,10 @@
   const int8_t* w2p = DUALH ? a.w2 + (int64_t)drow * C2 + dseg : nullptr;
   const void* const pars2[4] = {a.s_w2, a.wsum2, a.bias2 ? (const void*)a.bias2 : (const void*)a.s_w2, a.s_w2};
   const int32_t* parp2 = static_cast<const int32_t*>(wave == 0 ? pars2[0] : wave == 1 ? pars2[1] : wave == 2 ? pars2[2] : pars2[3]) + lane;
+  const int8_t* wap = RC ? a.wa + (int64_t)drow * CA + dseg : nullptr;
+  const int8_t* wbp = RC ? a.w2 + (int64_t)drow * CB + dseg : nullptr;
+  const void* const parsa[4] = {a.s_wa, a.wsuma, a.biasa ? (const void*)a.biasa : (const void*)a.s_wa, a.s_wa};
+  const int32_t* parpa = static_cast<const int32_t*>(wave == 0 ? parsa[0] : wave == 1 ? parsa[1] : wave == 2 ? parsa[2] : parsa[3]) + lane;
 
   f32x4 res[2][4];
 #ifdef DLMCQ_LAB
@@ -251,7 +298,7 @@
     for (int u = 0; u < U3; ++u)
       if (wdma) {
         const int8_t* src = w3p + (int64_t)u * 64 * a.w3_row + (int64_t)n * a.w3_chunk;
-        __builtin_amdgcn_global_load_lds((gptr_t)src, (lptr_t)(wb + (S1 + S2 + u) * 4096 + wave * 1024), 16, 0, 0);
+        __builtin_amdgcn_global_load_lds((gptr_t)src, (lptr_t)(wb + (W3U + u) * 4096 + wave * 1024), 16, 0, 0);
       }
     __builtin_amdgcn_global_load_lds((gptr_t)(parp + n * 64), (lptr_t)(par0 + P * PAR + wave * 256), 4, 0, 0);
     if constexpr (DUALH) {
@@ -259,6 +306,17 @@
       for (int s = 0; s < S2; ++s)
         if (wdma) __builtin_amdgcn_global_load_lds((gptr_t)(w2p + (int64_t)n * 64 * C2 + s * 64), (lptr_t)(wb + (S1 + s) * 4096 + wave * 1024), 16, 0, 0);
       __builtin_amdgcn_global_load_lds((gptr_t)(parp2 + n * 64), (lptr_t)(par0 + P * PAR + 1024 + wave * 256), 4, 0, 0);
+      return;
+    }
+    if constexpr (RC) {
+#pragma unroll
+      for (int s = 0; s < SA; ++s)
+        if (wdma) __builtin_amdgcn_global_load_lds((gptr_t)(wap + (int64_t)n * 64 * CA + s * 64), (lptr_t)(wb + (S1 + s) * 4096 + wave * 1024), 16, 0, 0);
+#pragma unroll
+      for (int s = 0; s < SB; ++s)
+        if (wdma) __builtin_amdgcn_global_load_lds((gptr_t)(wbp + (int64_t)n * 64 * CB + s * 64), (lptr_t)(wb + (S1 + SA + s) * 4096 + wave * 1024), 16, 0, 0);
+      __builtin_amdgcn_global_load_lds((gptr_t)(parpa + n * 64), (lptr_t)(par0 + P * PAR + 1024 + wave * 256), 4, 0, 0);
+      __builtin_amdgcn_global_load_lds((gptr_t)(parp2 + n * 64), (lptr_t)(par0 + P * PAR + 2048 + wave * 256), 4, 0, 0);
       return;
     }
 #pragma unroll
@@ -285,8 +343,10 @@
   const float sin1 = a.s_in1[0];
   const float zpf1 = a.zp_in1 ? a.zp_in1[0] : 0.0f;
   const int dz1 = a.shift1 - (int)__builtin_rintf(zpf1);
-  const float sin1b = DUALH ? a.s_in2[0] : 0.0f;
-  const int dz1b = DUALH ? a.shift2 - (int)__builtin_rintf(a.zp_in2 ? a.zp_in2[0] : 0.0f) : 0;
+  const float sin1b = (DUALH || RC) ? a.s_in2[0] : 0.0f;
+  const int dz1b = (DUALH || RC) ? a.shift2 - (int)__builtin_rintf(a.zp_in2 ? a.zp_in2[0] : 0.0f) : 0;
+  const float sin1a = RC ? a.s_ina[0] : 0.0f;
+  const int dz1a = RC ? a.shifta - (int)__builtin_rintf(a.zp_ina ? a.zp_ina[0] : 0.0f) : 0;
   ConvEpi e1 = ep1;
   e1.codes = reinterpret_cast<uint8_t*>(uintptr_t(1));
   const EpiQuant eq1(e1, FL >= 0);
@@ -308,7 +368,7 @@
     else if (nst == 5) asm volatile("s_waitcnt vmcnt(5)\n\ts_barrier" ::: "memory");
     else asm volatile("s_waitcnt vmcnt(1)\n\ts_barrier" ::: "memory");
     CHAIN_STAMP();
-    if constexpr (!DUALH) asm volatile("" : "+v"(res[P][0]), "+v"(res[P][1]), "+v"(res[P][2]), "+v"(res[P][3]));
+    if constexpr (!DUALH && !RC) asm volatile("" : "+v"(res[P][0]), "+v"(res[P][1]), "+v"(res[P][2]), "+v"(res[P][3]));
     if (nseq + 1 < NC) request(nseq + 1, std::integral_constant<int, 1 - P>{});
 
     const int8_t* wb = lds + P * WCH;
@@ -333,6 +393,56 @@
 #pragma unroll
       for (int i = 0; i < 8; ++i) extra2[i] = pk_fma(f32x2{(float)acc[2 * i], (float)acc[2 * i + 1]} + c2, m2, b2);
     }
+    f32x2 sc2[RC ? 8 : 1];
+    if constexpr (RC) {
+      f32x2 eb[8];
+      const int r = wc * 32 + l31;
+      {
+        const float corrbf = (float)(dz1b * *reinterpret_cast<const int*>(pp + 2048 + 256));
+#pragma unroll
+        for (int i = 0; i < 16; ++i) acc[i] = 0;
+#pragma unroll
+        for (int s = 0; s < SB; ++s)
+#pragma unroll
+          for (int ks = 0; ks < 2; ++ks) {
+            const i32x4 bf = *reinterpret_cast<const i32x4*>(wb + (S1 + SA + s) * 4096 + r * 64 + (((ks * 2 + hsel) ^ ((r >> 2) & 3)) << 4));
+            acc = __builtin_amdgcn_mfma_i32_32x32x32_i8(afb[s][ks], bf, acc, 0, 0, 0);
+          }
+        const float multb = sin1b * *reinterpret_cast<const float*>(pp + 2048);
+        const float bvb = a.bias2 ? *reinterpret_cast<const float*>(pp + 2048 + 512) : 0.0f;
+        const f32x2 c2{corrbf, corrbf}, m2{multb, multb}, b2{bvb, bvb};
+#pragma unroll
+        for (int i = 0; i < 8; ++i) eb[i] = pk_fma(f32x2{(float)acc[2 * i], (float)acc[2 * i + 1]} + c2, m2, b2);
+      }
+      {
+        const float corraf = (float)(dz1a * *reinterpret_cast<const int*>(pp + 1024 + 256));
+#pragma unroll
+        for (int i = 0; i < 16; ++i) acc[i] = 0;
+#pragma unroll
+        for (int s = 0; s < SA; ++s)
+#pragma unroll
+          for (int ks = 0; ks < 2; ++ks) {
+            const i32x4 bf = *reinterpret_cast<const i32x4*>(wb + (S1 + s) * 4096 + r * 64 + (((ks * 2 + hsel) ^ ((r >> 2) & 3)) << 4));
+            acc = __builtin_amdgcn_mfma_i32_32x32x32_i8(afa[s][ks], bf, acc, 0, 0, 0);
+          }
+        const float multa = sin1a * *reinterpret_cast<const float*>(pp + 1024);
+        const float bva = a.biasa ? *reinterpret_cast<const float*>(pp + 1024 + 512) : 0.0f;
+        const f32x2 c2{corraf, corraf}, m2{multa, multa}, b2{bva, bva};
+#pragma unroll
+        for (int i = 0; i < 8; ++i) {
+          f32x2 f = pk_fma(f32x2{(float)acc[2 * i], (float)acc[2 * i + 1]} + c2, m2, b2);
+          sc2[i] = f + eb[i];
+        }
+      }
+      if (a.relu_sc) {
+#pragma unroll
+        for (int i = 0; i < 8; i += 2) {
+          const f32x4 t = relu4_nan(f32x4{sc2[i].x, sc2[i].y, sc2[i + 1].x, sc2[i + 1].y});
+          sc2[i] = f32x2{t.x, t.y};
+          sc2[i + 1] = f32x2{t.z, t.w};
+        }
+      }
+    }
     const float corrf = (float)(dz1 * *reinterpret_cast<const int*>(pp + 256));
 #pragma unroll
     for (int i = 0; i < 16; ++i) acc[i] = 0;
@@ -359,6 +469,7 @@
       for (int i = 0; i < 8; ++i) {
         f32x2 f = pk_fma(f32x2{(float)acc[2 * i], (float)acc[2 * i + 1]} + c2, m2, b2);
         if constexpr (DUALH) f = f + extra2[DUALH ? i : 0];
+        if constexpr (RC) f = f + sc2[RC ? i : 0];
         v[2 * i] = f.x;
         v[2 * i + 1] = f.y;
       }
@@ -384,7 +495,7 @@
           quad_transpose(v[4 * g], v[4 * g + 1], v[4 * g + 2], v[4 * g + 3], b0, b1);
           y[k] = f32x4{v[4 * g], v[4 * g + 1], v[4 * g + 2], v[4 * g + 3]};
         }
-        if constexpr (!DUALH) y[k] = y[k] + res[P][g];
+        if constexpr (!DUALH && !RC) y[k] = y[k] + res[P][g];
         if (relu1 && (FL < 0 || out1)) y[k] = relu4_nan(y[k]);
 #ifdef DLMCQ_LAB
         if (out1) bstore16(y[k], (a.lab & 0x1000) ? (out_off(g, n) & 0xffff) : out_off(g, n), r_out);
@@ -422,7 +533,7 @@
 #pragma unroll
         for (int j = 0; j < U3; ++j) {
           const int kb = wc * (KB / 2) + j * 32 + l31;
-          const i32x4 bf = *reinterpret_cast<const i32x4*>(wb + (S1 + S2) * 4096 + kb * 64 + (((ks * 2 + hsel) ^ ((kb >> 2) & 3)) << 4));
+          const i32x4 bf = *reinterpret_cast<const i32x4*>(wb + W3U * 4096 + kb * 64 + (((ks * 2 + hsel) ^ ((kb >> 2) & 3)) << 4));
           acc2[j] = __builtin_amdgcn_mfma_i32_32x32x32_i8(bf, a2, acc2[j], 0, 0, 0);
         }
       }
@@ -481,7 +592,7 @@
 static int chain_launch(ChainArgs& a, int64_t M, int64_t C, int64_t K, int64_t C2, int64_t K2, int32_t relu, void* codes,
                         const float* q_scale, const float* q_zero_point, int32_t q_lo, int32_t q_hi, int32_t q_form, float q_ste_g,
                         int32_t relu2, void* codes2, const float* q2_scale, const float* q2_zero_point, int32_t q2_lo, int32_t q2_hi,
-                        int32_t q2_form, float q2_ste_g, int32_t rows_per_tile, dlmcq_stream_t stream) {
+                        int32_t q2_form, float q2_ste_g, int32_t rows_per_tile, dlmcq_stream_t stream, int64_t CA = 0, int64_t CB = 0) {
   if (relu == DLMCQ_ACT_RELU6 || relu2 == DLMCQ_ACT_RELU6) return DLMCQ_EINVAL;
   if (q_lo != 0 || q_hi != 255) return DLMCQ_EINVAL;
   if (q2_form & (DLMCQ_FORCE_TILED | DLMCQ_ROUTE_ONLY | DLMCQ_PIPELINED)) return DLMCQ_EINVAL;
@@ -507,7 +618,7 @@
   a.lab = g_chain_lab;
 #endif
   if (rows_per_tile <= 0) {
-    const int64_t t64 = (M + 63) / 64, slots = 256 * CHAIN_WGS((int)(C + C2), (int)K2);
+    const int64_t t64 = (M + 63) / 64, slots = 256 * CHAIN_WGS((int)(C + C2 + CA + CB), (int)K2);
     const int64_t full = t64 / slots, left = t64 % slots;
     rows_per_tile = (full >= 2 && full <= 4 && left > 0 && left * 8 < slots) ? 56 : 64;
   }
@@ -532,7 +643,11 @@
     else if (fl == 1) hipLaunchKernelGGL((conv_chain_i8_kernel<__VA_ARGS__, 1>), grid, block, dyn, st, a, ep1, ep2);  \
     else hipLaunchKernelGGL((conv_chain_i8_kernel<__VA_ARGS__, -1>), grid, block, dyn, st, a, ep1, ep2);              \
   } while (0)
-  if (C2 == 0) {
+  if (CA > 0) {
+    if (!(C == 64 && K2 == 64 && CA == 64 && CB == 64) || fl < 0) return DLMCQ_EINVAL;
+    if (fl == 3) hipLaunchKernelGGL((conv_chain_i8_kernel<64, 64, 0, 3, 64, 64>), grid, block, dyn, st, a, ep1, ep2);
+    else hipLaunchKernelGGL((conv_chain_i8_kernel<64, 64, 0, 1, 64, 64>), grid, block, dyn, st, a, ep1, ep2);
+  } else if (C2 == 0) {
     if (C == 64 && K2 == 64) DLMCQ_CHAIN_GO(64, 64, 0);
     else if (C == 64 && K2 == 128) DLMCQ_CHAIN_GO(64, 128, 0);
     else if (C == 128 && K2 == 128) DLMCQ_CHAIN_GO(128, 128, 0);
@@ -608,3 +723,42 @@
   return chain_launch(a, M, C, K, C2, K3, relu, codes, q_scale, q_zero_point, q_lo, q_hi, q_form, q_ste_g, relu3, codes3, q3_scale,
                       q3_zero_point, q3_lo, q3_hi, q3_form, q3_ste_g, rows_per_tile, stream);
 }
+
+extern "C" int dlmcq_conv2d_i8_nhwc_recompute_chain(
+    const void* x, const int8_t* w, float* out, const float* bias, const int32_t* wsum, const float* in_scale, const float* in_zero_point,
+    const float* w_scale, int64_t N, int64_t H, int64_t W, int64_t C, int64_t K, int32_t x_is_unsigned, const void* xa, const int8_t* wa,
+    const float* biasa, const int32_t* wsuma, const float* in_scalea, const float* in_zero_pointa, const float* w_scalea, int64_t Ca,
+    int32_t xa_is_unsigned, const void* xb, const int8_t* wb, const float* biasb, const int32_t* wsumb, const float* in_scaleb,
+    const float* in_zero_pointb, const float* w_scaleb, int64_t Hb, int64_t Wb, int64_t Cb, int32_t strideb, int32_t xb_is_unsigned,
+    int32_t relu_shortcut, int32_t relu, void* codes, const float* q_scale, const float* q_zero_point, int32_t q_lo, int32_t q_hi,
+    int32_t q_form, float q_ste_g, const int8_t* w2, const float* bias2, const int32_t* wsum2, const float* w_scale2, int64_t K2,
+    int32_t relu2, void* codes2, const float* q2_scale, const float* q2_zero_point, int32_t q2_lo, int32_t q2_hi, int32_t q2_form,
+    float q2_ste_g, int32_t rows_per_tile, dlmcq_stream_t stream) {
+  if (N < 0 || H < 1 || W < 1 || C < 1 || K < 1 || K2 < 1 || K % 64 != 0 || Ca < 1 || Hb < 1 || Wb < 1 || Cb < 1 || strideb < 1)
+    return DLMCQ_EINVAL;
+  if ((Hb - 1) / strideb + 1 != H || (Wb - 1) / strideb + 1 != W) return DLMCQ_EINVAL;
+  if (relu_shortcut == DLMCQ_ACT_RELU6) return DLMCQ_EINVAL;
+  const int64_t M = N * H * W;
+  if (M == 0) return DLMCQ_OK;
+  if (!x || !w || !wsum || !in_scale || !w_scale || !xa || !wa || !wsuma || !in_scalea || !w_scalea || !xb || !wb || !wsumb ||
+      !in_scaleb || !w_scaleb || !w2 || !wsum2 || !w_scale2 || !codes2 || !q_scale || !q2_scale)
+    return DLMCQ_EINVAL;
+  if (!aligned16(x) || !aligned16(w) || !aligned16(xa) || !aligned16(wa) || !aligned16(xb) || !aligned16(wb) || !aligned16(w2) ||
+      (out && !aligned16(out)) || (codes && !aligned16(codes)) || !aligned16(codes2))
+    return DLMCQ_EALIGN;
+  if (M >= (1ll << 31) || N * Hb * Wb * Cb >= (1ll << 40)) return DLMCQ_ERANGE;
+  ChainArgs a{};
+  a.x = static_cast<const int8_t*>(x); a.w1 = w; a.s_w1 = w_scale; a.wsum1 = wsum; a.bias1 = bias;
+  a.s_in1 = in_scale; a.zp_in1 = in_zero_point; a.shift1 = x_is_unsigned ? 128 : 0;
+  a.xa = static_cast<const int8_t*>(xa); a.wa = wa; a.s_wa = w_scalea; a.wsuma = wsuma; a.biasa = biasa;
+  a.s_ina = in_scalea; a.zp_ina = in_zero_pointa; a.shifta = xa_is_unsigned ? 128 : 0; a.relu_sc = relu_shortcut != 0;
+  a.x2 = static_cast<const int8_t*>(xb); a.w2 = wb; a.s_w2 = w_scaleb; a.wsum2 = wsumb; a.bias2 = biasb;
+  a.s_in2 = in_scaleb; a.zp_in2 = in_zero_pointb; a.shift2 = xb_is_unsigned ? 128 : 0;
+  a.P = (int)H; a.Q = (int)W; a.H2 = (int)Hb; a.W2 = (int)Wb; a.stride2 = strideb;
+  a.qdiv = make_fastdiv((uint32_t)W);
+  a.pdiv = make_fastdiv((uint32_t)H);
+  a.residual = nullptr; a.out = out; a.codes = static_cast<uint8_t*>(codes);
+  a.w3 = w2; a.s_w3 = w_scale2; a.wsum3 = wsum2; a.bias3 = bias2; a.codes2 = static_cast<uint8_t*>(codes2);
+  return chain_launch(a, M, C, K, 0, K2, relu, codes, q_scale, q_zero_point, q_lo, q_hi, q_form, q_ste_g, relu2, codes2, q2_scale,
+                      q2_zero_point, q2_lo, q2_hi, q2_form, q2_ste_g, rows_per_tile, stream, Ca, Cb);
+}
diff --git a/dlmc-quant_amd/dlmc/_native.py b/dlmc-quant_amd/dlmc/_native.py
--- a/dlmc-quant_amd/dlmc/_native.py
+++ b/dlmc-quant_amd/dlmc/_native.py
@@ -107,6 +107,11 @@
                                                       _p, _p, _p, _p, _p, _p, _p, _i64, _i64, _i64, _i32, _i32,
                                                       _i32, _p, _p, _p, _i32, _i32, _i32, _f32,
                                                       _p, _p, _p, _p, _i64, _i32, _p, _p, _p, _i32, _i32, _i32, _f32, _i32, _p]),
+    "dlmcq_conv2d_i8_nhwc_recompute_chain": (ctypes.c_int, [_p, _p, _p, _p, _p, _p, _p, _p, _i64, _i64, _i64, _i64, _i64, _i32,
+                                                           _p, _p, _p, _p, _p, _p, _p, _i64, _i32,
+                                                           _p, _p, _p, _p, _p, _p, _p, _i64, _i64, _i64, _i32, _i32,
+                                                           _i32, _i32, _p, _p, _p, _i32, _i32, _i32, _f32,
+                                                           _p, _p, _p, _p, _i64, _i32, _p, _p, _p, _i32, _i32, _i32, _f32, _i32, _p]),
     "dlmcq_quantize_pad_nhwc4": (ctypes.c_int, [_p, _p, _p, _p, _i64, _i64, _i64, _i64, _i64, _i64, _i64, _i64, _i32, _i32, _i32,
                                                _i32, _f32, _p]),
     "dlmcq_quantize_weight_stem_i8": (ctypes.c_int, [_p, _p, _p, _p, _i64, _i64, _i64, _i64, _i32, _i32, _p]),
diff --git a/dlmc-quant_amd/dlmc/quantization/scalar/kernels.py b/dlmc-quant_amd/dlmc/quantization/scalar/kernels.py
--- a/dlmc-quant_amd/dlmc/quantization/scalar/kernels.py
+++ b/dlmc-quant_amd/dlmc/quantization/scalar/kernels.py
@@ -719,6 +719,27 @@
         self.buf.record_stream(s)
 
 
+class DeferredBlock(ChunkMajor):
+
+    def __init__(self, pa, pb, relu, shape):
+        self.pa, self.pb, self.relu, self.shape = pa, pb, bool(relu), tuple(shape)
+        self.dtype, self.device, self._buf = torch.float32, pa["codes"].device, None
+
+    @property
+    def buf(self):
+        if self._buf is None:
+            self._buf = ChunkMajor.from_nhwc(conv2d_i8_dual(self.pa, self.pb, relu=self.relu, emit=None, want_out=True)).buf
+        return self._buf
+
+    def numel(self):
+        return math.prod(self.shape)
+
+    def record_stream(self, s):
+        for t in (self.pa["codes"], self.pb["codes"], self._buf):
+            if t is not None:
+                t.record_stream(s)
+
+
 class PadShortcut:
 
     def __init__(self, src, stride=1, lo=0):
@@ -826,6 +847,46 @@
         *_q_args(q3, w3flag | (N.FP32_OUT_CHUNK_MAJOR if fcm else 0)), int(rows_per_tile), N.stream_ptr())),
         2 * m * K_ * (ch + ch2 + K3))
     return out, q[0], q3[0]
+
+
+RECOMPUTE_CHAIN_SHAPES = {(64, 64, 64, 64)}
+
+
+def recompute_chain_supported(c, ca, cb, k, k2, m):
+    return (c, ca, cb, k2) in RECOMPUTE_CHAIN_SHAPES and k % 64 == 0 and m * k * 4 <= 0x7fff0000
+
+
+def conv2d_i8_recompute_chain(a, b, pa, pb, relu_shortcut=True, relu=True, emit=None, want_out=True, want_codes=False, relu2=True,
+                              emit2=None, rows_per_tile=0, out_chunk_major=False):
+    N.require_gpu(b["wq"])
+    o, oa, ob = _operand(a), _operand(pa), _operand(pb)
+    c = o.codes
+    (n, K_), (h, w_, ch, R, S, st, pd, _, uns) = o.shape[:2], o.geom
+    _, _, cha, Ra, Sa, sta, pda, _, unsa = oa.geom
+    hb, wb_, chb, Rb, Sb, stb, pdb, _, unsb = ob.geom
+    K2, R2, S2, C2 = b["wq"].shape
+    if (R, S, R2, S2, Ra, Sa, Rb, Sb) != (1,) * 8 or (st, sta) != (1, 1) or pd or pda or pdb or C2 != K_ or emit is None or emit2 is None:
+        raise ValueError("conv2d_i8_recompute_chain: unpadded 1x1 convolutions, the second reading the first's codes")
+    if oa.shape != o.shape or ob.shape != o.shape:
+        raise ValueError(f"conv2d_i8_recompute_chain: the block gives {o.shape}, its recomputed shortcut {oa.shape} and {ob.shape}")
+    m = n * h * w_
+
+    def alloc(k, dtype):
+        return torch.empty((n, k, h, w_), dtype=dtype, device=c.device, memory_format=torch.channels_last)
+    ocm = bool(out_chunk_major) and want_out
+    out = (ChunkMajor.empty(n, K_, h, w_, c.device) if ocm else alloc(K_, torch.float32)) if want_out else None
+    q = _quantiser(emit, lambda dtype: alloc(K_, dtype) if want_codes else None, c, False, "conv2d_i8_recompute_chain")
+    q2 = _quantiser(emit2, lambda dtype: alloc(K2, dtype), c, True, "conv2d_i8_recompute_chain")
+    b2, ws2 = _bias_c(b["bias"]), _flat(b["w_scale"], c, K2)
+    nbytes = c.numel() + oa.codes.numel() + ob.codes.numel() // (stb * stb) + a["wq"].numel() + pa["wq"].numel() + pb["wq"].numel() + \
+        b["wq"].numel() + m * K_ * (4 * want_out + want_codes) + m * K2
+    w2t, w2flag = _second_weights(b)
+    PROFILE.launch("conv_chain", nbytes, lambda: N.check(N.lib.dlmcq_conv2d_i8_nhwc_recompute_chain(
+        *_head(o, out.buf if ocm else out), n, h, w_, ch, K_, uns, *oa.ptrs, cha, unsa, *ob.ptrs, hb, wb_, chb, stb, unsb,
+        int(bool(relu_shortcut)), int(bool(relu)), *_q_args(q), N.ptr(w2t), N.ptr(b2), N.ptr(b["wsum"]), N.ptr(ws2), K2, int(bool(relu2)),
+        *_q_args(q2, w2flag | (N.FP32_OUT_CHUNK_MAJOR if ocm else 0)), int(rows_per_tile), N.stream_ptr())),
+        2 * m * K_ * (ch + cha + chb + K2))
+    return out, q[0], q2[0]
 
 
 def quantize_pad_nhwc4(x, scale, zero_point, lo, hi, form, pad, g=0.0, shift128=False, pad_code0=False):
diff --git a/dlmc-quant_amd/dlmc/utils/fuse.py b/dlmc-quant_amd/dlmc/utils/fuse.py
--- a/dlmc-quant_amd/dlmc/utils/fuse.py
+++ b/dlmc-quant_amd/dlmc/utils/fuse.py
@@ -1,4 +1,5 @@
 import math
+import os
 import operator
 
 import torch
@@ -391,6 +392,8 @@
         self.swapped = short is not None and self.main is not a
         self._w2cm = None
         self.out_cm = False
+        self.defer_out = False
+        self.recompute = False
 
     def forward(self, x, y):
         a, b, sc, mn = self.a, self.b, self.short, self.main
@@ -406,6 +409,9 @@
         kw = dict(relu=a.relu, emit=a._emit_for(n, a.k, h, w), want_out=a.want_out, want_codes=self.want_codes, emit2=b._emit_for(n, b.k, h, w),
                   out_chunk_major=self.out_cm)
         if sc is None:
+            if (self.recompute and isinstance(y, K.DeferredBlock) and y._buf is None and
+                    K.recompute_chain_supported(c, y.pa["codes"].shape[1], y.pb["codes"].shape[1], a.k, b.k, n * h * w)):
+                return K.conv2d_i8_recompute_chain(a.operand(x, codes), nxt, y.pa, y.pb, relu_shortcut=y.relu, relu2=b.relu, **kw)
             if not K.chain_supported(c, a.k, b.k, n * h * w):
                 if isinstance(y, K.ChunkMajor):
                     y = y.to_nhwc()
@@ -416,7 +422,11 @@
             out, mid = DualInt8Layer(a, sc if mn is a else mn)(*((x, y) if mn is a else (y, x)))
             return out, (mid if self.want_codes else None), b(mid)[1]
         kw["emit3"] = kw.pop("emit2")
-        return K.conv2d_i8_dual_chain(mn.operand(x), sc.operand(y), nxt, relu3=b.relu, **kw)
+        oa, ob = mn.operand(x), sc.operand(y)
+        if self.defer_out and a.want_out:
+            _, mid, codes3 = K.conv2d_i8_dual_chain(oa, ob, nxt, relu3=b.relu, **dict(kw, want_out=False))
+            return K.DeferredBlock(oa, ob, a.relu, (n, a.k, h, w)), mid, codes3
+        return K.conv2d_i8_dual_chain(oa, ob, nxt, relu3=b.relu, **kw)
 
 
 class DwPwInt8Layer(nn.Module):
@@ -498,7 +508,7 @@
 
 def _pointwise(plan):
     lay = plan.layer
-    return (type(plan) is Int8Layer and lay.weight.dim() == 4 and tuple(lay.weight.shape[2:]) == (1, 1) and lay.stride[0] == 1 and
+    return (_is_int8(plan) and lay.weight.dim() == 4 and tuple(lay.weight.shape[2:]) == (1, 1) and lay.stride[0] == 1 and
             lay.padding[0] == 0 and plan.w_off is None and plan.pool is None and plan.k_pad == plan.k and plan.c_pad == plan.c and
             not plan.act.needs_g and not plan.relu6 and
             plan.pad_shortcut is None)
@@ -516,7 +526,7 @@
             a, other = a.a, a.b
             main, short = (a, other) if _pointwise(a) else (other, a)
             lay = short.layer
-            if not (_pointwise(main) and type(short) is Int8Layer and lay.weight.dim() == 4 and tuple(lay.weight.shape[2:]) == (1, 1) and
+            if not (_pointwise(main) and _is_int8(short) and lay.weight.dim() == 4 and tuple(lay.weight.shape[2:]) == (1, 1) and
                     lay.padding[0] == 0 and short.w_off is None and short.pool is None and short.k_pad == short.k and
                     short.c_pad == short.c and not short.act.needs_g and a.pool is None and a.w_off is None):
                 continue
@@ -564,8 +574,42 @@
         gm.recompile()
 
 
+RECOMPUTE_ENABLED = {(64, 64, 64, 64)}
+RECOMPUTE_DEFAULT = os.environ.get("DLMCQ_RECOMPUTE_SHORTCUTS", "1") not in ("0", "", "off", "false")
+
+
+def _plain_emit(e):
+    return e is not None and (e.lo, e.hi) == (0, 255) and not e.needs_g and e.zp_emit is None
+
+
+def _recompute_pass(gm, report, enabled):
+    graph = gm.graph
+    modules = dict(gm.named_modules())
+    count = 0
+    for n0 in list(graph.nodes):
+        m0 = modules.get(n0.target) if n0.op == "call_module" else None
+        if not isinstance(m0, ChainInt8Layer) or m0.short is None or m0.defer_out or len(n0.args) != 2:
+            continue
+        outs = [u for u in n0.users if u.op == "call_function" and u.target is operator.getitem and u.args[1] == 0]
+        if len(outs) != 1 or len(outs[0].users) != 1:
+            continue
+        o = outs[0]
+        n1 = next(iter(o.users))
+        m1 = modules.get(n1.target) if n1.op == "call_module" else None
+        if not (isinstance(m1, ChainInt8Layer) and m1.short is None and not m1.recompute and len(n1.args) == 2 and not n1.kwargs and
+                n1.args[1] is o and n1.args[0] is not o):
+            continue
+        if (m1.main.c, m0.main.c, m0.short.c, m1.b.k) not in enabled or m0.a.k != m1.a.k:
+            continue
+        if not (m1.a.relu and _plain_emit(m1.a.emit) and _plain_emit(m1.b.emit) and m0.a.pool is None and m1.a.pool is None):
+            continue
+        m0.defer_out = m1.recompute = True
+        count += 1
+    report.recomputed = count
+
+
 def _block_end_like(m):
-    return (type(m) is Int8Layer and _pointwise(m) and m.c in (256, 512) and m.k % 128 == 0 and m.k_pad == m.k and m.c_pad == m.c and m.relu
+    return (_is_int8(m) and _pointwise(m) and m.c in (256, 512) and m.k % 128 == 0 and m.k_pad == m.k and m.c_pad == m.c and m.relu
             and m.w_off is None and m.pool is None and m.layer.stride[0] == 1 and not m.act.needs_g and
             (m.emit is None or ((m.emit.lo, m.emit.hi) == (0, 255) and not m.emit.needs_g)))
 
@@ -581,7 +625,7 @@
         if isinstance(m, ChainInt8Layer):
             return m.a.k % 64 == 0
         if isinstance(m, DualInt8Layer):
-            one = lambda t: type(t) is Int8Layer and t.layer.weight.dim() == 4 and tuple(t.layer.weight.shape[2:]) == (1, 1)
+            one = lambda t: _is_int8(t) and t.layer.weight.dim() == 4 and tuple(t.layer.weight.shape[2:]) == (1, 1)
             dense, other = (m.a, m.b) if m.a.c == 256 else (m.b, m.a)
             return (one(m.a) and one(m.b) and (dense.c, other.c) == (256, 512) and dense.layer.stride[0] == 1 and m.a.relu and m.a.k % 128 == 0
                     and m.a.k_pad == m.a.k and m.a.w_off is None and m.b.w_off is None and m.a.pool is None and m.a.emit is not None)
@@ -951,12 +995,32 @@
         raise RuntimeError("fuse_inference(dry_run=True) builds the plan's structure only")
 
 
+class _DryInt8Layer(Int8Layer):
+
+    def __init__(self, layer, spec, relu=False, emit=None, want_out=True, pool=None, relu6=False):
+        nn.Module.__init__(self)
+        self.layer, self.act, self.kind, self.w_off = layer, spec[0], spec[4], spec[5]
+        self.relu, self.emit, self.want_out, self.pool, self.relu6 = bool(relu), emit, bool(want_out), pool, bool(relu6)
+        w = layer.weight
+        self.k, self.c = int(w.shape[0]), int(w.shape[1])
+        self.k_pad, self.c_pad = (_ceil64(self.k), _ceil64(self.c)) if w.dim() == 4 else (self.k, self.c)
+        self.narrow, self.pad_shortcut, self.emit_shift = False, None, False
+
+    def forward(self, *args):
+        raise RuntimeError("fuse_inference(dry_run=...) builds the plan's structure only")
+
+
+def _is_int8(m):
+    return type(m) in (Int8Layer, _DryInt8Layer)
+
+
 class FusionReport:
 
     def __init__(self):
         self.layers = self.relu = self.residual = self.emit = self.fp32_outputs = self.stem = self.pooled = self.dual = 0
         self.relu6 = 0
         self.chained = 0
+        self.recomputed = 0
         self.chunk_major = 0
         self.dwpw = 0
         self.act_offset = 0
@@ -971,6 +1035,7 @@
                 f"code-emitting={self.emit}, fp32 outputs kept={self.fp32_outputs}, stem layers={self.stem}, "
                 f"pools on codes={self.pooled}, dual (conv + shortcut conv) kernels={self.dual}, chained pairs={self.chained} (fp32 outputs chunk-major: {self.chunk_major}), "
                 f"depthwise + pointwise units={self.dwpw}, " + (f"gap heads={self.gap_heads}, " if self.gap_heads else "") +
+                (f"recomputed shortcuts={self.recomputed}, " if self.recomputed else "") +
                 (f"narrow fp32 rows={self.narrow}, " if self.narrow else "") +
                 (f"pad shortcuts={self.pad_shortcuts}, " if self.pad_shortcuts else "") +
                 (f"average pools on the plan={self.avg_pools}, " if self.avg_pools else "") +
@@ -1240,7 +1305,8 @@
 
 
 def fuse_inference(model, report=None, dry_run=False, chain_pairs=True, pack_int4=True, weight_blob=None, dwpw=False, block_layout=True,
-                   relu6=True, act_offsets=False, gap_head=False, narrow_rows=False, pad_shortcuts=False, avg_pools=False):
+                   relu6=True, act_offsets=False, gap_head=False, narrow_rows=False, pad_shortcuts=False, avg_pools=False,
+                   recompute_shortcuts=None):
     if not any(gap_head is v for v in (False, True)) and gap_head not in ("separate", "fused"):
         raise ValueError(f"fuse_inference: gap_head is False, True, 'separate' or 'fused', not {gap_head!r}")
     if model.training:
@@ -1367,7 +1433,11 @@
                 modules[node.target].weight.dim() == 4 and modules[residual.target].weight.dim() == 4 and not act6 and
                 not any(sp[0].xoff and int(modules[t].padding[0]) > 0 for sp, t in ((spec, node.target), (other, residual.target))))
         narrow = bool(can_narrow and (fp32_needed or emit is None or residual is not None))
-        if dry_run:
+        if dry_run == "chains" and cls is Int8Layer:
+            opts = dict(relu=relu, emit=emit, want_out=fp32_needed or emit is None, pool=pool, relu6=act6)
+            plan = _DryInt8Layer(modules[node.target], spec, **opts)
+            gm.add_module(name, DualInt8Layer(plan, _DryInt8Layer(modules[residual.target], other)) if dual else plan)
+        elif dry_run:
             gm.add_module(name, _DryNode())
         else:
             def from_blob(name, sp):
@@ -1441,10 +1511,12 @@
         _avgpool_pass(gm, report, planned, dry_run)
     if gap_head:
         _gap_pass(gm, report, gap_head, planned, dry_run)
-    if chain_pairs and not dry_run:
+    if chain_pairs and (not dry_run or dry_run == "chains"):
         _chain_pass(gm, report)
         if block_layout:
             _block_layout_pass(gm, report)
+        if RECOMPUTE_DEFAULT if recompute_shortcuts is None else recompute_shortcuts:
+            _recompute_pass(gm, report, RECOMPUTE_ENABLED)
         if dwpw:
             _dwpw_pass(gm, report)
     gm.packed_weights = _pack_plan_weights(gm) if (pack_int4 and not dry_run) else []
diff --git a/include/dlmcq.h b/include/dlmcq.h
--- a/include/dlmcq.h
+++ b/include/dlmcq.h
@@ -289,6 +289,17 @@
                                     int32_t q3_lo, int32_t q3_hi, int32_t q3_form, float q3_ste_g, int32_t rows_per_tile,
                                     dlmcq_stream_t stream);
 
+int dlmcq_conv2d_i8_nhwc_recompute_chain(
+    const void* x, const int8_t* w, float* out, const float* bias, const int32_t* wsum, const float* in_scale, const float* in_zero_point,
+    const float* w_scale, int64_t N, int64_t H, int64_t W, int64_t C, int64_t K, int32_t x_is_unsigned, const void* xa, const int8_t* wa,
+    const float* biasa, const int32_t* wsuma, const float* in_scalea, const float* in_zero_pointa, const float* w_scalea, int64_t Ca,
+    int32_t xa_is_unsigned, const void* xb, const int8_t* wb, const float* biasb, const int32_t* wsumb, const float* in_scaleb,
+    const float* in_zero_pointb, const float* w_scaleb, int64_t Hb, int64_t Wb, int64_t Cb, int32_t strideb, int32_t xb_is_unsigned,
+    int32_t relu_shortcut, int32_t relu, void* codes, const float* q_scale, const float* q_zero_point, int32_t q_lo, int32_t q_hi,
+    int32_t q_form, float q_ste_g, const int8_t* w2, const float* bias2, const int32_t* wsum2, const float* w_scale2, int64_t K2,
+    int32_t relu2, void* codes2, const float* q2_scale, const float* q2_zero_point, int32_t q2_lo, int32_t q2_hi, int32_t q2_form,
+    float q2_ste_g, int32_t rows_per_tile, dlmcq_stream_t stream);
+
 
 int dlmcq_quantize_pad_nhwc4(const float* x, void* out, const float* scale, const float* zero_point, int64_t N,
                              int64_t C, int64_t H, int64_t W, int64_t stride_n, int64_t stride_c, int64_t stride_h,
```
